# zijinxuxu/PDFNet

Hardware: AMD Instinct MI355X
Metric: train-step images/sec @256x256 RGB-D B=32 (higher is better)
Workload: dtype f32

## Files before the change

include/pdfnet_hip.h:

```cpp
#ifndef PDFNET_HIP_H
#define PDFNET_HIP_H
#ifdef __cplusplus
extern "C" {
#endif

#define PDF_E_BADARG (-1)
#define PDF_E_WORKSPACE (-2)
#define PDF_ACT_NONE 0
#define PDF_ACT_RELU 1
#define PDF_ACT_LRELU01 2


int pdf_linear_fwd(const float* x, const float* w, const float* bias, float* y,
                   int M, int N, int K, int ldx, int ldw, int ldy, int act, void* stream);
int pdf_linear_bwd_weight(const float* x, const float* dy, float* dw, float* db, float* ws, long ws_floats,
                          int M, int N, int K, int ldx, int lddy, int accumulate, void* stream);
long pdf_wgrad_workspace_floats(int M, int NI, int NJ);
int pdf_init(void);
int pdf_debug_init_device(void);
int pdf_debug_kernel_timing(int on);
int pdf_set_stats_output(float* part, long cap_floats);
long pdf_stats_result_tiles(void);
long pdf_stats_result_rows(void);
int pdf_set_bn_tile_stats(const float* part, long tiles, long rows_per_tile);
int pdf_debug_kernel_record_count(void);
int pdf_debug_kernel_record(int i, char* name, int cap, double* flops, double* bytes, float* ms);
int pdf_stream_wait(void* waiter, void* signaler);
int pdf_set_gemm_precision(int bf16);
int pdf_debug_gemm_precision(void);
int pdf_debug_last_tile(void);
int pdf_debug_igemm_launches(void);
int pdf_linear_bwd_data(const float* dy, const float* w, float* dx, int M, int N, int K, int lddy, int ldw, int lddx, void* stream);
int pdf_linear_fwd_pair(const float* x, const float* w0, const float* w1, const float* b0, const float* b1, float* y,
                        int M, int N, int K, int ldx, int ldw, int ldy, int act, void* stream);
int pdf_linear_bwd_data_pair(const float* dy, const float* w0, const float* w1, float* dx, int M, int N, int K,
                             int lddy, int ldw, int lddx, void* stream);
int pdf_linear_bwd_weight_pair(const float* x, const float* dy, float* dw0, float* dw1, float* db0, float* db1,
                               float* ws, long ws_floats, int M, int N, int K, int ldx, int lddy, int accumulate, void* stream);

int pdf_conv2d_fwd(const float* x, const float* w, const float* bias, float* y,
                   int N, int H, int W, int Cin, int ldx, int Cout, int KH, int KW,
                   int stride, int pad, int OH, int OW, int ldy, int act, void* stream);
int pdf_conv2d_bwd_data(const float* dy, const float* w, float* dx,
                        int N, int H, int W, int Cin, int lddx, int Cout, int KH, int KW,
                        int stride, int pad, int OH, int OW, int lddy, void* stream);
int pdf_conv2d_bwd_data_add(const float* dy, const float* w, float* dx,
                        int N, int H, int W, int Cin, int lddx, int Cout, int KH, int KW,
                        int stride, int pad, int OH, int OW, int lddy, void* stream);
int pdf_conv2d_bwd_weight(const float* x, const float* dy, float* dw, float* db, float* ws, long ws_floats,
                          int N, int H, int W, int Cin, int ldx, int Cout, int KH, int KW,
                          int stride, int pad, int OH, int OW, int lddy, int accumulate, void* stream);

int pdf_deconv2d_fwd(const float* x, const float* w, const float* bias, float* y,
                     int N, int H, int W, int Cin, int ldx, int Cout, int KH, int KW,
                     int stride, int pad, int OH, int OW, int ldy, void* stream);
int pdf_deconv2d_bwd_data(const float* dy, const float* w, float* dx,
                          int N, int H, int W, int Cin, int lddx, int Cout, int KH, int KW,
                          int stride, int pad, int OH, int OW, int lddy, void* stream);
int pdf_deconv2d_bwd_weight(const float* x, const float* dy, float* dw, float* ws, long ws_floats,
                            int N, int H, int W, int Cin, int ldx, int Cout, int KH, int KW,
                            int stride, int pad, int OH, int OW, int lddy, int accumulate, void* stream);
int pdf_bmm_strided(const float* A, const float* B, float* C, int batch, int M, int N, int K, int RB,
                    long sab, long sar, long sam, long sak, long sbb, long sbr, long sbk, long sbn,
                    long scb, long scm, long scn, int beta, void* stream);


int pdf_knn_ball_group(const float* pts, int ldp, int C, int Bc, int N, int S, int K, float r2,
                       int* idx, float* grouped, int ldg, void* stream);
int pdf_group_bwd(const float* dg, int ldg, const int* idx, float* dpts, int ldd, int C,
                  int Bc, int N, int S, int K, void* stream);
int pdf_gather_sub_fwd(const float* u, int ldu, const float* v, int ldv, const int* idx, int Bc, int N, int S, int K, int C,
                       float* y, int ldy, void* stream);
int pdf_gather_sub_bwd(const float* dy, int lddy, const int* idx, float* du, int ldu, float* dv, int ldv,
                       int Bc, int N, int S, int K, int C, void* stream);
int pdf_invert_index(const int* idx, int Bc, int N, int E, int* start, int* list, int* tmp, void* stream);
int pdf_gather_sub_bwd_sorted(const float* dy, int lddy, const int* start, const int* list, float* du, int ldu, float* dv, int ldv,
                              int Bc, int N, int S, int K, int C, void* stream);
int pdf_gather_rows(const float* feat, int ldf, int C, long HW, const long* ind, long ind_bstride,
                    int B, int M, int R, int shift, float* out, int ldo, void* stream);
int pdf_scatter_rows_add(const float* dout, int ldo, int C, long HW, const long* ind, long ind_bstride,
                         int B, int M, int R, int shift, float* dfeat, int ldf, void* stream);
int pdf_window_op(float* feat, int ldf, int C, int H, int W, const long* ind, long ind_bstride,
                  int B, int M, int r, float* buf, const float* src, int mode, void* stream);
int pdf_nms_top1(const float* hm, int BC, int H, int W, long* ind, float* score, void* stream);
int pdf_maxk_fwd(const float* x, int ldx, int C, long R, int K, float* y, int ldy, int* arg, void* stream);
int pdf_maxk_bwd(const float* dy, int ldy, const int* arg, int C, long R, int K, float* dx, int ldx, void* stream);
int pdf_bn_relu_maxk_fwd(const float* y, int ldy, int C, long R, int K, const float* gamma, const float* beta,
                         float* running_mean, float* running_var, float momentum, float eps, int training,
                         float* out, int ldo, int* arg, float* save_mean, float* save_rstd, float* scale, float* shift,
                         float* ws, void* stream);
int pdf_bn_relu_maxk_bwd(const float* dout, int lddo, const int* arg, const float* y, int ldy, const float* save_mean, const float* save_rstd,
                         const float* gamma, const float* scale, const float* shift, int C, long R, int K,
                         float* dy, int lddy, float* dgamma, float* dbeta, int accumulate, float* ws, void* stream);
long pdf_sa_fused_workspace_floats(int Bc, int S, int K, int C1, int C2, int C3);
int pdf_sa_fused_fwd(const float* u, const float* v, const int* idx, int Bc, int N, int S, int K, int C1, int C2, int C3,
                     const float* w2, const float* b2, const float* w3, const float* b3,
                     const float* gamma1, const float* beta1, const float* gamma2, const float* beta2, const float* gamma3, const float* beta3,
                     float* rmean1, float* rvar1, float* rmean2, float* rvar2, float* rmean3, float* rvar3, float momentum, float eps, int training,
                     float* out, int* arg, float* zsel, float* saved, float* ws, long ws_floats, void* stream);
int pdf_sa_fused_bwd(const float* dout, const float* u, const float* v, const int* idx, int Bc, int N, int S, int K, int C1, int C2, int C3,
                     const float* w2, const float* b2, const float* w3, const float* b3,
                     const float* out, const int* arg, const float* zsel, const float* saved,
                     float* dz1, float* dw2, float* db2, float* dw3, float* db3,
                     float* dgamma1, float* dbeta1, float* dgamma2, float* dbeta2, float* dgamma3, float* dbeta3,
                     float* ws, long ws_floats, void* stream);


long pdf_bn_workspace_floats(int C, long R);
int pdf_bn_train_fwd(const float* x, int ldx, int C, long R, const float* gamma, const float* beta,
                     float* running_mean, float* running_var, float momentum, float eps,
                     const float* res, int ldr, int relu, float* y, int ldy,
                     float* save_mean, float* save_rstd, float* scale, float* shift, float* ws, void* stream);
int pdf_bn_eval_fwd(const float* x, int ldx, int C, long R, const float* gamma, const float* beta,
                    const float* running_mean, const float* running_var, float eps,
                    const float* res, int ldr, int relu, float* y, int ldy, float* scale, float* shift, void* stream);
int pdf_bn_train_bwd(const float* dy, int lddy, const float* y, int ldy, int relu, const float* x, int ldx,
                     const float* save_mean, const float* save_rstd, const float* gamma,
                     const float* scale, const float* shift, int C, long R,
                     float* dx, int lddx, float* dres, int lddr, float* dgamma, float* dbeta, int accumulate,
                     float* ws, void* stream);
int pdf_bn_eval_bwd(const float* dy, int lddy, const float* y, int ldy, int relu, const float* x, int ldx,
                    const float* running_mean, const float* running_var, float eps, const float* scale, const float* shift,
                    int C, long R, float* dx, int lddx, float* dres, int lddr,
                    float* dgamma, float* dbeta, int accumulate, float* ws, void* stream);
int pdf_bn_relu_maxk_eval_bwd(const float* dout, int lddo, const int* arg, const float* y, int ldy,
                              const float* running_mean, const float* running_var, float eps, const float* scale, const float* shift,
                              int C, long R, int K, float* dy, int lddy, float* dgamma, float* dbeta, int accumulate, float* ws, void* stream);
int pdf_colsum(const float* g, int ldg, int C, long R, float* out, int accumulate, float* ws, void* stream);
int pdf_colsum_pair(const float* g, int ldg, int C, long R, float* out0, float* out1, int accumulate, float* ws, void* stream);
int pdf_layernorm_fwd(const float* x, int ldx, int F, long R, const float* gamma, const float* beta, float eps,
                      float* y, int ldy, float* mean, float* rstd, void* stream);
int pdf_layernorm_bwd(const float* dy, int lddy, const float* x, int ldx, int F, long R, const float* gamma,
                      const float* mean, const float* rstd, float* dx, int lddx, float* dgamma, float* dbeta, void* stream);
int pdf_layernorm_fused_fwd(const float* x, int ldx, const float* add, int ldadd, float p, unsigned long long seed,
                            const unsigned long long* step, int F, long R, long R_split,
                            const float* gamma0, const float* beta0, const float* gamma1, const float* beta1, float eps, int act,
                            float* z, int ldz, float* y, int ldy, float* mean, float* rstd, void* stream);
int pdf_layernorm_fused_bwd(const float* dy, int lddy, const float* y, int ldy, int act, const float* z, int ldz, int F, long R, long R_split,
                            const float* gamma0, const float* gamma1, const float* mean, const float* rstd,
                            const float* dz_in, int lddzin, float* dz, int lddz, float* dadd, int lddadd,
                            float p, unsigned long long seed, const unsigned long long* step,
                            float* dgamma0, float* dbeta0, float* dgamma1, float* dbeta1, void* stream);
int pdf_l2norm_fwd(const float* x, int ldx, int C, long R, const float* w, float eps, float* y, int ldy, float* norm, void* stream);
int pdf_l2norm_bwd(const float* dy, int lddy, const float* x, int ldx, int C, long R, const float* w, float eps,
                   const float* norm, float* dx, int lddx, float* dw, void* stream);
int pdf_l2norm_cat_fwd(int nparts, const float* const* x, const int* C, const float* const* w, float eps, long R,
                       float* y, int ldy, float* const* norm, void* stream);
int pdf_l2norm_cat_bwd(int nparts, const float* dy, int lddy, const float* const* x, const int* C, const float* const* w, float eps, long R,
                       float* const* norm, float* const* dx, float* const* dw, void* const* dx16_or_null, void* stream);

int pdf_act_fwd(const float* x, int ldx, float* y, int ldy, int C, long R, int act, void* stream);
int pdf_act_bwd(const float* dy, int lddy, const float* y, int ldy, float* dx, int lddx, int C, long R, int act, void* stream);
int pdf_sft_fwd(const float* fea, int ldf, const float* scale, int lds, const float* shift, int ldh,
                float* out, int ldo, int C, long R, void* stream);
int pdf_sft_bwd(const float* g, int ldg, const float* fea, int ldf, const float* scale, int lds,
                float* dfea, int lddf, float* dscale, int ldds, int C, long R, void* stream);
int pdf_sft3_fwd(const float* fea, int ldf, const float* cond, int ldc, const float* w_scale0, const float* b_scale0,
                 const float* w_scale1, const float* b_scale1, const float* w_shift0, const float* b_shift0,
                 const float* w_shift1, const float* b_shift1, float* out, int ldo, long R, void* stream);
int pdf_sft3_bwd(const float* g, int ldg, const float* fea, int ldf, const float* cond, int ldc,
                 const float* w_scale0, const float* b_scale0, const float* w_scale1, const float* b_scale1,
                 const float* w_shift0, const float* b_shift0, const float* w_shift1, const float* b_shift1,
                 float* dfea, int lddf, float* dcond, int lddc,
                 float* dw_scale0, float* db_scale0, float* dw_scale1, float* db_scale1,
                 float* dw_shift0, float* db_shift0, float* dw_shift1, float* db_shift1, int accumulate,
                 float* ws, long R, void* stream);
int pdf_set_bf16_operands(const void* op0_bf16, const void* op1_bf16);
int pdf_set_bf16_output(void* out_bf16);
int pdf_set_bn_input_bf16(const void* x16);
int pdf_set_input_affine_relu(const float* scale, const float* shift);
int pdf_cast_bf16(const float* src, void* dst, long n, void* stream);
int pdf_cast_bf16_transposed(const float* src, void* dst, const void* table, int nlayers, long total_tiles, void* stream);
int pdf_debug_shadow_operands(void);
int pdf_dropout(const float* x, float* y, long n, float p, unsigned long long seed, const unsigned long long* step, void* stream);
int pdf_dropout_add(const float* x, const float* res, float* y, long n, float p, unsigned long long seed,
                    const unsigned long long* step, void* stream);
int pdf_maxpool3s2_fwd(const float* x, int N, int H, int W, int C, float* y, unsigned char* arg, void* stream);
int pdf_maxpool3s2_bwd(const float* dy, const unsigned char* arg, int N, int H, int W, int C, float* dx, void* stream);
int pdf_maxpool3s2_bwd_add(const float* dy, const unsigned char* arg, int N, int H, int W, int C, float* dx, void* stream);
int pdf_upsample2x_fwd(const float* x, int N, int H, int W, int C, float* y, void* stream);
int pdf_upsample2x_bwd(const float* dy, int N, int H, int W, int C, float* dx, void* stream);
int pdf_pad2d(const float* src, int lds, long R, int C, float* dst, int ldd, long R2, int C2, void* stream);
int pdf_adam_step(float* p, const float* g, float* m, float* v, long n, float lr, float b1, float b2, float eps,
                  const float* corr, float grad_scale, void* stream);

int pdf_cheby2_fwd(const float* x, int ldx, int B, int V, int F, const int* col, const float* val, int Wd,
                   float* out, int ldo, void* stream);
int pdf_cheby2_bwd(const float* d, int ldd, int B, int V, int F, const int* colT, const float* valT, int Wd,
                   float* dx, int lddx, void* stream);
int pdf_cheby2_fwd_pair(const float* x, int ldx, int B, int V, int F, const int* col0, const float* val0,
                        const int* col1, const float* val1, int Wd, float* out, int ldo, void* stream);
int pdf_cheby2_bwd_pair(const float* d, int ldd, int B, int V, int F, const int* colT0, const float* valT0,
                        const int* colT1, const float* valT1, int Wd, float* dx, int lddx, void* stream);
int pdf_attn_fwd(const float* q, const float* k, const float* v, int ld, int B, int V, int H, int dh, int kv_shift,
                 float pdrop, unsigned long long seed, const unsigned long long* step, float* out, int ldo, float* stat, void* stream);
int pdf_attn_bwd(const float* q, const float* k, const float* v, int ld, const float* o, const float* dout, int ldo,
                 const float* stat, int B, int V, int H, int dh, int kv_shift, float pdrop, unsigned long long seed, const unsigned long long* step,
                 float* dq, float* dk, float* dv, int lddq, float* dvec, void* stream);

int pdf_fps(const float* xyz, int ld, int Bc, int N, int S, const int* start, int* idx, void* stream);

int pdf_rowloss_fwd(const float* pred, const float* tgt, long rows, long n, int mode, float* out, void* stream);
int pdf_rowloss_bwd(const float* pred, const float* tgt, const float* gout, long rows, long n, int mode, float* dpred, void* stream);
int pdf_face_loss_fwd(const float* pred, const float* gt, const long long* faces, int G, int B, int V, int Fc, float* part, void* stream);
int pdf_face_loss_bwd(const float* pred, const float* gt, const long long* faces, int G, int B, int V, int Fc,
                      const float* wn, const float* we, float* dpred, void* stream);

long pdf_dense_loss_workspace_floats(int B);
int pdf_dense_loss_fwd(const float* mask, const float* mask_gt, int mask_c, int mask_hw,
                       const float* hms, const float* hms_gt, int hms_c, int hms_hw,
                       const float* hm, const float* hm_gt, int hm_c, int hm_hw, int B, float* ws, float* out, void* stream);
int pdf_dense_loss_bwd(const float* mask, const float* mask_gt, float* dmask, int mask_c, int mask_hw,
                       const float* hms, const float* hms_gt, float* dhms, int hms_c, int hms_hw,
                       const float* hm, const float* hm_gt, float* dhm, int hm_c, int hm_hw, int B,
                       const float* g_mask, const float* g_hms, const float* g_hm, const float* stat, void* stream);
int pdf_point_dist_sum(const float* pred, const float* gt, int rows, int n, int dim, float* out, void* stream);

int pdf_procrustes_dist(const float* pred, const float* gt, int rows, int n, float* sum, float* dist, float* aligned, void* stream);
int pdf_mesh_nn_counts(const float* pred, const float* gt, int rows, int n, const float* thr, int T, int* counts, float* d_gt, float* d_pred,
                       void* stream);

int pdf_depth2pcl(const float* depth, const float* mask, const float* K, const float* valid, int B, int H, int W,
                  unsigned long long seed, long* choose, float* cloud, int* count, void* stream);

int pdf_mano_lbs_fwd(const float* root_aa, const float* pose_aa, const float* shape, const float* trans,
                     const float* v_template, const float* shapedirs, const float* posedirs, const float* J_reg,
                     const float* weights, int B, int left_side, int center_idx, float* verts, float* joints, void* stream);
int pdf_mano_lbs_bwd(const float* root_aa, const float* pose_aa, const float* shape,
                     const float* v_template, const float* shapedirs, const float* posedirs, const float* J_reg,
                     const float* weights, int B, int left_side, int center_idx, const float* dverts, const float* djoints,
                     float* droot, float* dpose, float* dshape, float* dtrans, void* stream);
int pdf_mano_split_coeff(const float* params, int ldp, long HW, const long* ind, const float* K, int B, int input_res, int down,
                         float* orient, float* pose, float* shape, float* trans, void* stream);
int pdf_mano_split_coeff_bwd(const float* params, float* dparams, int ldp, long HW, const long* ind, const float* K, int B, int input_res, int down,
                             const float* dorient, const float* dpose, const float* dtrans, void* stream);


typedef struct PdfCallOpts {
    const void* op0_bf16; const void* op1_bf16;
    void* out_bf16;
    const void* bn_x_bf16;
    float* stats_out; long stats_cap;
    long stats_tiles; long stats_rows;
    const float* tile_stats; long tile_n; long tile_rows;
    const float* in_scale; const float* in_shift;
    const void* op1_bf16_t;
    float* ws; long ws_floats;
    const float* wino_v;
} PdfCallOpts;
long pdf_conv2d_winograd_v_offset(int N, int H, int W, int Cin, int Cout, int KH, int KW, int stride, int pad);
int pdf_linear_fwd_x(const float* x, const float* w, const float* bias, float* y, int M, int N, int K, int ldx, int ldw, int ldy, int act, void* stream, PdfCallOpts* opts);
int pdf_linear_fwd_pair_x(const float* x, const float* w0, const float* w1, const float* b0, const float* b1, float* y, int M, int N, int K, int ldx, int ldw, int ldy, int act, void* stream, PdfCallOpts* opts);
int pdf_linear_bwd_data_x(const float* dy, const float* w, float* dx, int M, int N, int K, int lddy, int ldw, int lddx, void* stream, PdfCallOpts* opts);
int pdf_linear_bwd_data_pair_x(const float* dy, const float* w0, const float* w1, float* dx, int M, int N, int K, int lddy, int ldw, int lddx, void* stream, PdfCallOpts* opts);
int pdf_conv2d_fwd_x(const float* x, const float* w, const float* bias, float* y, int N, int H, int W, int Cin, int ldx, int Cout, int KH, int KW, int stride, int pad, int OH, int OW, int ldy, int act, void* stream, PdfCallOpts* opts);
int pdf_conv2d_bwd_data_x(const float* dy, const float* w, float* dx, int N, int H, int W, int Cin, int lddx, int Cout, int KH, int KW, int stride, int pad, int OH, int OW, int lddy, void* stream, PdfCallOpts* opts);
int pdf_conv2d_bwd_data_add_x(const float* dy, const float* w, float* dx, int N, int H, int W, int Cin, int lddx, int Cout, int KH, int KW, int stride, int pad, int OH, int OW, int lddy, void* stream, PdfCallOpts* opts);
int pdf_linear_bwd_weight_x(const float* x, const float* dy, float* dw, float* db, float* ws, long ws_floats, int M, int N, int K, int ldx, int lddy, int accumulate, void* stream, PdfCallOpts* opts);
int pdf_linear_bwd_weight_pair_x(const float* x, const float* dy, float* dw0, float* dw1, float* db0, float* db1, float* ws, long ws_floats, int M, int N, int K, int ldx, int lddy, int accumulate, void* stream, PdfCallOpts* opts);
int pdf_conv2d_bwd_weight_x(const float* x, const float* dy, float* dw, float* db, float* ws, long ws_floats, int N, int H, int W, int Cin, int ldx, int Cout, int KH, int KW, int stride, int pad, int OH, int OW, int lddy, int accumulate, void* stream, PdfCallOpts* opts);
int pdf_deconv2d_fwd_x(const float* x, const float* w, const float* bias, float* y, int N, int H, int W, int Cin, int ldx, int Cout, int KH, int KW, int stride, int pad, int OH, int OW, int ldy, void* stream, PdfCallOpts* opts);
int pdf_deconv2d_bwd_data_x(const float* dy, const float* w, float* dx, int N, int H, int W, int Cin, int lddx, int Cout, int KH, int KW, int stride, int pad, int OH, int OW, int lddy, void* stream, PdfCallOpts* opts);
int pdf_deconv2d_bwd_weight_x(const float* x, const float* dy, float* dw, float* ws, long ws_floats, int N, int H, int W, int Cin, int ldx, int Cout, int KH, int KW, int stride, int pad, int OH, int OW, int lddy, int accumulate, void* stream, PdfCallOpts* opts);
int pdf_bn_train_fwd_x(const float* x, int ldx, int C, long R, const float* gamma, const float* beta, float* running_mean, float* running_var, float momentum, float eps, const float* res, int ldr, int relu, float* y, int ldy, float* save_mean, float* save_rstd, float* scale, float* shift, float* ws, void* stream, PdfCallOpts* opts);
int pdf_bn_train_bwd_x(const float* dy, int lddy, const float* y, int ldy, int relu, const float* x, int ldx, const float* save_mean, const float* save_rstd, const float* gamma, const float* scale, const float* shift, int C, long R, float* dx, int lddx, float* dres, int lddr, float* dgamma, float* dbeta, int accumulate, float* ws, void* stream, PdfCallOpts* opts);
int pdf_bn_relu_maxk_fwd_x(const float* y, int ldy, int C, long R, int K, const float* gamma, const float* beta, float* running_mean, float* running_var, float momentum, float eps, int training, float* out, int ldo, int* arg, float* save_mean, float* save_rstd, float* scale, float* shift, float* ws, void* stream, PdfCallOpts* opts);
int pdf_l2norm_cat_fwd_x(int nparts, const float* const* x, const int* C, const float* const* w, float eps, long R, float* y, int ldy, float* const* norm, void* stream, PdfCallOpts* opts);
long pdf_conv2d_winograd_workspace_floats(int N, int H, int W, int Cin, int Cout, int KH, int KW, int stride, int pad, int backward);
int pdf_debug_armed_slots(void);
int pdf_debug_callopts_size(void);

int pdf_x3_split(const float* x, void* out, long n, long cs, void* stream);
long pdf_deconv2d_x3_workspace_floats(int N, int H, int W, int Cin, int Cout, int KH, int KW, int stride, int pad, int backward);
int pdf_set_x3_mode(int mode);
int pdf_stream_create(void** out, int priority, int* lo, int* hi);
int pdf_debug_x3_mode(void);
int pdf_debug_x3_stamps(unsigned long long* out);
int pdf_x3_batched_gemm_nt(const void* A3, long csA, const void* B3, long csB, float* C, int batch, long gsA, long gsB, long gsC, int M, int N, int K, int variant, int nprod, void* stream);
int pdf_batched_gemm_nt(const float* A, const float* B, float* C, int batch, long gsA, long gsB, long gsC, int M, int N, int K, void* stream);
int pdf_x3_batched_gemm_tn(const void* P3, long csP, const void* Q3, long csQ, float* slab, int batch, long gsP, long gsQ, int M, int NI, int NJ, int splits, int variant, int nprod, void* stream);
int pdf_batched_gemm_tn(const float* P, const float* Q, float* slab, int batch, long gsP, long gsQ, int M, int NI, int NJ, int splits, void* stream);

typedef struct PdfMeshLin { const float* w[2]; const float* b[2]; } PdfMeshLin;
typedef struct PdfMeshLN { const float* g[2]; const float* b[2]; } PdfMeshLN;
typedef struct PdfMeshGcn { PdfMeshLin fc1, fc2, sc; PdfMeshLN n2, n3; unsigned long long seed; } PdfMeshGcn;
typedef struct PdfMeshAttn {
    PdfMeshLN ln; PdfMeshLin q, k, v, fc; PdfMeshLN ffln; PdfMeshLin f1, f2;
    unsigned long long seed_att, seed_z, seed_t, seed_x;
} PdfMeshAttn;
typedef struct PdfMeshLinG { float* w[2]; float* b[2]; } PdfMeshLinG;
typedef struct PdfMeshLNG { float* g[2]; float* b[2]; } PdfMeshLNG;
typedef struct PdfMeshGcnG { PdfMeshLinG fc1, fc2, sc; PdfMeshLNG n2, n3; } PdfMeshGcnG;
typedef struct PdfMeshAttnG { PdfMeshLNG ln; PdfMeshLinG q, k, v, fc; PdfMeshLNG ffln; PdfMeshLinG f1, f2; } PdfMeshAttnG;
typedef struct PdfMeshLevel {
    int level, B, training, cin0;
    float p;
    const unsigned long long* step;
    const float* x;
    float* out;
    const int* ell_col[2]; const float* ell_val[2]; const int* ell_colT[2]; const float* ell_valT[2]; int ell_w;
    PdfMeshGcn gcn[4];
    PdfMeshAttn self_, cross;
    float* tape;
    float* qkv;
    const float* dout;
    float* dx;
    float* gtape;
    PdfMeshGcnG ggcn[4]; PdfMeshAttnG gself, gcross;
    float* wg_ws; long wg_ws_floats;
} PdfMeshLevel;
long pdf_mesh_tape_floats(int level, int B);
long pdf_mesh_gtape_floats(int level, int B);
int pdf_mesh_level_fwd(const PdfMeshLevel* a, void* stream);
int pdf_mesh_level_bwd(const PdfMeshLevel* a, void* stream, void* side_stream);
int pdf_mesh_level_fwd_bf16(const PdfMeshLevel* a, void* stream);
int pdf_mesh_level_bwd_bf16(const PdfMeshLevel* a, void* stream, void* side_stream);
int pdf_mesh_level_fwd_x3(const PdfMeshLevel* a, void* stream);
int pdf_mesh_level_bwd_x3(const PdfMeshLevel* a, void* stream, void* side_stream);
int pdf_debug_mesh_level_size(void);

typedef struct PdfMeshLoss {
    const float* vp; const float* v2p; const float* hd3; const float* hd2; const float* r;
    const float* vgt[2]; const float* jgt[2]; const float* v2gt[2]; const float* lmsgt[2];
    const long long* ind; const float* K; const float* valid;
    const float* reg[2]; const long long* faces; const long long* perm[2];
    int B, Fc, size, down;
    float* part;
    float* out;
    float coef[12];
    const float* gmp;
    int edge_grad;
    float* dvp; float* dv2p; float* dhd3; float* dhd2; float* dr;
} PdfMeshLoss;
int pdf_mesh_loss_fwd(const PdfMeshLoss* a, void* stream);
int pdf_mesh_loss_bwd(const PdfMeshLoss* a, void* stream);
int pdf_debug_mesh_loss_size(void);
int pdf_debug_mesh_stamps(unsigned long long* out);

#ifdef __cplusplus
}
#endif
#endif
```

pdfnet_amd/csrc/common.h:

```cpp
#pragma once
#include <hip/hip_runtime.h>
#include <stdint.h>
#include "pdfnet_hip.h"

#define PDF_API extern "C" __attribute__((visibility("default")))

#define PDF_LAUNCH_CHECK()                                  \
    do {                                                    \
        hipError_t e__ = hipGetLastError();                 \
        if (e__ != hipSuccess) return (int)e__;             \
    } while (0)

static inline int cdiv(long a, long b) { return (int)((a + b - 1) / b); }

static inline int grid_for(long n, int block = 256, int cap = 256 * 8) {
    long g = (n + block - 1) / block;
    if (g > cap) g = cap;
    if (g < 1) g = 1;
    return (int)g;
}

__device__ __forceinline__ float wave_sum(float v) {
#pragma unroll
    for (int o = 32; o > 0; o >>= 1) v += __shfl_xor(v, o, 64);
    return v;
}
__device__ __forceinline__ float wave_max(float v) {
#pragma unroll
    for (int o = 32; o > 0; o >>= 1) v = fmaxf(v, __shfl_xor(v, o, 64));
    return v;
}
__device__ __forceinline__ int wave_sum_i(int v) {
#pragma unroll
    for (int o = 32; o > 0; o >>= 1) v += __shfl_xor(v, o, 64);
    return v;
}

__device__ __forceinline__ uint32_t pdf_hash32(uint32_t x) {
    x ^= x >> 16; x *= 0x7feb352dU; x ^= x >> 15; x *= 0x846ca68bU; x ^= x >> 16;
    return x;
}
__device__ __forceinline__ float pdf_uniform(uint64_t seed, uint64_t idx) {
    uint32_t h = pdf_hash32((uint32_t)idx ^ pdf_hash32((uint32_t)(idx >> 32) + (uint32_t)seed) ^ (uint32_t)(seed >> 32) * 0x9E3779B9U);
    return (float)(h >> 8) * (1.0f / 16777216.0f);
}

__device__ __forceinline__ void pdf_store_wt(float* p, float v) { __hip_atomic_store(p, v, __ATOMIC_RELAXED, __HIP_MEMORY_SCOPE_AGENT); }
__device__ __forceinline__ bool pdf_last_block_arrives(int* counter, int expected, int* flag, bool release = true) {
    asm volatile("s_waitcnt vmcnt(0)" ::: "memory");
    __syncthreads();
    if (threadIdx.x == 0) {
        if (release) {
            __builtin_amdgcn_fence(__ATOMIC_RELEASE, "agent");
            asm volatile("s_waitcnt vmcnt(0)" ::: "memory");
        }
        const int t = __hip_atomic_fetch_add(counter, 1, __ATOMIC_RELAXED, __HIP_MEMORY_SCOPE_AGENT);
        const int last = t == expected - 1;
        if (last) {
            __builtin_amdgcn_fence(__ATOMIC_ACQUIRE, "agent");
            asm volatile("s_waitcnt vmcnt(0)" ::: "memory");
            __hip_atomic_store(counter, 0, __ATOMIC_RELAXED, __HIP_MEMORY_SCOPE_AGENT);
        }
        *flag = last;
    }
    __syncthreads();
    return *flag != 0;
}

#define PDF_COUNTER_RING (1 << 22)
int* pdf_ticket_counters(int n);
#define PDF_SCRATCH_RING (1L << 26)
#define PDF_SCRATCH_MAX (1L << 22)
float* pdf_scratch(long floats);
typedef __bf16 pdf_bf16x2 __attribute__((ext_vector_type(2)));
typedef float pdf_f32x2 __attribute__((ext_vector_type(2)));
__device__ __forceinline__ unsigned int pdf_pk_bf16(float a, float b) {
    pdf_f32x2 f = {a, b};
    pdf_bf16x2 v = __builtin_convertvector(f, pdf_bf16x2);
    return *reinterpret_cast<unsigned int*>(&v);
}
__device__ __forceinline__ void pdf_x3_split2(float a, float b, unsigned& h, unsigned& m, unsigned& l) {
    h = pdf_pk_bf16(a, b);
    float ra = a - __uint_as_float(h << 16), rb = b - __uint_as_float(h & 0xffff0000u);
    m = pdf_pk_bf16(ra, rb);
    ra -= __uint_as_float(m << 16); rb -= __uint_as_float(m & 0xffff0000u);
    l = pdf_pk_bf16(ra, rb);
}
__device__ __forceinline__ void pdf_x3_store2(unsigned short* base, long o, long cs, float a, float b) {
    unsigned h, m, l;
    pdf_x3_split2(a, b, h, m, l);
    *reinterpret_cast<unsigned*>(base + o) = h;
    *reinterpret_cast<unsigned*>(base + o + cs) = m;
    *reinterpret_cast<unsigned*>(base + o + 2 * cs) = l;
}
template <class F, class... A> static inline int pdf_call_x(PdfCallOpts* opts, F impl, A... a) {
    PdfCallOpts none = {};
    PdfCallOpts& co = opts != nullptr ? *opts : none;
    co.stats_tiles = co.stats_rows = 0;
    return impl(a..., co);
}
struct PdfPlainCall { PdfCallOpts co; PdfPlainCall(); ~PdfPlainCall(); };
template <class F, class... A> static inline int pdf_call_plain(F impl, A... a) {
    PdfPlainCall call;
    return impl(a..., call.co);
}
```

pdfnet_amd/csrc/gemm.hip:

```cpp
#include "common.h"

#include "gemm_common.h"

long pdf_internal_wino_workspace(int N, int H, int W, int Ck, int Cn, int flip);
int pdf_internal_wino_eligible(int N, int H, int W, int Ck, int Cn, int KH, int KW, int stride, int pad, int flip);
int pdf_internal_conv3x3_winograd(const float* x, int ldx, const float* w, const float* bias, float* y, int ldy, float* ws,
                                  int N, int H, int W, int Ck, int Cn, int act, int accum, int flip, const float* v_shared, hipStream_t s);
int pdf_internal_wino_wgrad_eligible(int N, int H, int W, int Cin, int Cout, int KH, int KW, int stride, int pad);
long pdf_internal_wino_wgrad_workspace(int N, int H, int W, int Cin, int Cout);
long pdf_internal_wino_v_offset(int N, int H, int W, int Ck, int Cn);
int pdf_internal_conv3x3_winograd_wgrad(const float* x, int ldx, const float* dy, int lddy, float* dw, float* db, float* ws,
                                        int N, int H, int W, int Cin, int Cout, int accumulate, const float* v_cached, hipStream_t s);
PDF_API long pdf_conv2d_winograd_v_offset(int N, int H, int W, int Cin, int Cout, int KH, int KW, int stride, int pad) {
    if (!pdf_internal_wino_eligible(N, H, W, Cin, Cout, KH, KW, stride, pad, 0) || !pdf_internal_wino_wgrad_eligible(N, H, W, Cin, Cout, KH, KW, stride, pad)) return -1;
    return pdf_internal_wino_v_offset(N, H, W, Cin, Cout);
}
PDF_API long pdf_conv2d_winograd_workspace_floats(int N, int H, int W, int Cin, int Cout, int KH, int KW, int stride, int pad, int backward) {
    if (backward == 2) return pdf_internal_wino_wgrad_eligible(N, H, W, Cin, Cout, KH, KW, stride, pad) ? pdf_internal_wino_wgrad_workspace(N, H, W, Cin, Cout) : 0;
    const int Ck = backward ? Cout : Cin, Cn = backward ? Cin : Cout;
    return pdf_internal_wino_eligible(N, H, W, Ck, Cn, KH, KW, stride, pad, backward) ? pdf_internal_wino_workspace(N, H, W, Ck, Cn, backward) : 0;
}

#ifndef PDF_FRAG_PIPE
#define PDF_FRAG_PIPE 0
// ... 239 lines not shown
            for (int j = 0; j < TN; ++j) b[set][j] = bs[brow + j * 32 * LD + kk * 2];
        };
        if (FRAG_PIPE) frag(0, 0);
#pragma unroll
        for (int kk = 0; kk < BK / 2; ++kk) {
            const int set = FRAG_PIPE ? (kk & 1) : 0;
            if (FRAG_PIPE) { if (kk + 1 < BK / 2) frag(set ^ 1, kk + 1); }
            else frag(0, kk);
#pragma unroll
            for (int i = 0; i < TM; ++i)
#pragma unroll
                for (int j = 0; j < TN; ++j)
                    acc[i][j] = __builtin_amdgcn_mfma_f32_32x32x2f32(a[set][i], b[set][j], acc[i][j], 0, 0, 0);
        }
    };
    if constexpr (FAST && BUF && IG_DEEP && BM * BN <= 64 * 64) {
        gload(kt0, ra, rb);
        gload(kt0 + 1, ra1, rb1);
        lstore(0, ra, rb);
        __syncthreads();
        for (int kt = kt0; kt < kt1; kt += 2) {
            gload(kt + 2, ra, rb);
            compute(0);
            if (kt + 1 >= kt1) break;
            lstore(1, ra1, rb1);
            __syncthreads();
            gload(kt + 3, ra1, rb1);
            compute(1);
            if (kt + 2 < kt1) lstore(0, ra, rb);
            __syncthreads();
        }
        if (g.stat != nullptr) __syncthreads();
    } else {
        gload(kt0, ra, rb);
        lstore(0, ra, rb);
        __syncthreads();
        int cur = 0;
        for (int kt = kt0; kt < kt1; ++kt) {
            if (kt + 1 < kt1) gload(kt + 1, ra, rb);
            compute(cur);
            if (kt + 1 < kt1) lstore(cur ^ 1, ra, rb);
            __syncthreads();
            cur ^= 1;
        }
    }

    if (g.ksteps > 0) {
        float* pp = g.part + (long)blockIdx.z * g.M * g.N;
        if (m0 + BM <= g.M && (long)g.M * g.N < (1L << 29)) {
            const auto rsP = __builtin_amdgcn_make_buffer_rsrc((void*)pp, 0, (unsigned)g.M * (unsigned)g.N * 4u, 0x00020000);
            const unsigned ldn4 = (unsigned)g.N * 4u;
#pragma unroll
            for (int j = 0; j < TN; ++j) {
                const int col = n0 + wn * TN * 32 + j * 32 + (lane & 31);
#pragma unroll
                for (int i = 0; i < TM; ++i) {
                    const unsigned vo = col < g.N ? (unsigned)((m0 + wm * TM * 32 + i * 32 + 4 * (lane >> 5)) * g.N + col) * 4u : 0xffffffffu;
                    float v[16];
#pragma unroll
                    for (int r = 0; r < 16; ++r) v[r] = acc[i][j][r];
#pragma unroll
                    for (int r = 0; r < 16; ++r)
                        __builtin_amdgcn_raw_buffer_store_b32(__builtin_bit_cast(unsigned, v[r]), rsP, vo, ((r & 3) + 8 * (r >> 2)) * ldn4, 0);
                }
            }
            return;
        }
#pragma unroll
        for (int j = 0; j < TN; ++j) {
            const int col = n0 + wn * TN * 32 + j * 32 + (lane & 31);
#pragma unroll
            for (int i = 0; i < TM; ++i)
#pragma unroll
                for (int r = 0; r < 16; ++r) {
                    const int row = m0 + wm * TM * 32 + i * 32 + (r & 3) + 8 * (r >> 2) + 4 * (lane >> 5);
                    if (col < g.N && row < g.M) pp[(long)row * g.N + col] = acc[i][j][r];
                }
        }
        return;
    }
    StatAcc st[TN];
#pragma unroll
    for (int j = 0; j < TN; ++j) st[j] = StatAcc{0.f, 0.f, 0.f, 0.f};
    const bool do_stat = g.stat != nullptr;
    if constexpr (FAST && BUF) {
        if (g.cbytes != 0 && m0 + BM <= g.M) {
            lean_epilogue<TM, TN, WM, WN, BN>(acc, g, Cp, biasp, m0, n0, tmi, wm, wn, lane, tid, &As[0][0]);
            return;
        }
    }
#pragma unroll
    for (int j = 0; j < TN; ++j) {
        const int col = n0 + wn * TN * 32 + j * 32 + (lane & 31);
        const bool cok = col < g.N;
        int co = col, padd_y = 0, padd_x = 0;
        if (g.ps_cout > 0) {
            int tap = col / g.ps_cout;
            co = col - tap * g.ps_cout;
            padd_y = tap / g.ps_kw;
            padd_x = tap - padd_y * g.ps_kw;
        }
        const float bv = (biasp != nullptr && cok) ? biasp[co] : 0.f;
#pragma unroll
        for (int i = 0; i < TM; ++i) {
#pragma unroll
            for (int r = 0; r < 16; ++r) {
                const int row = m0 + wm * TM * 32 + i * 32 + (r & 3) + 8 * (r >> 2) + 4 * (lane >> 5);
                if (cok && row < g.M) {
                    float v = acc[i][j][r] + bv;
                    if (g.act == 1) v = fmaxf(v, 0.f);
                    else if (g.act == 2) v = v > 0.f ? v : 0.1f * v;
                    long o;
                    if (g.plain_out) o = (long)row * g.ldc + co;
                    else {
                        int hw = g.QH * g.QW;
                        int ni = row / hw, rem = row - ni * hw;
                        int qy = rem / g.QW, qx = rem - qy * g.QW;
                        int oy = qy * g.osy + g.ooy + padd_y, ox = qx * g.osx + g.oox + padd_x;
                        o = (((long)ni * g.OH + oy) * g.OW + ox) * g.ldc + co;
                    }
                    if (g.accum) v += Cp[o];
                    Cp[o] = v;
                    if (do_stat) stat_add(st[j], v);
                }
            }
        }
    }
    if (do_stat) stat_finish<TN, WM, WN, BN>(st, &As[0][0], g.stat, tmi, n0, g.N, wm, wn, lane, tid);
}

template <int BM, int BN, int WM, int WN, bool FAST, bool KN, int BKT = 16, bool BUF = false>
__global__ __launch_bounds__(WM * WN * 64, (BM * BN >= 128 * 128 ? 3 : 1)) void igemm_nt(const IGemm g) {
    igemm_nt_body<BM, BN, WM, WN, FAST, KN, BKT, BUF, false>(g);
}
template <int BM, int BN, int WM, int WN, int BKT>
__global__ __launch_bounds__(WM * WN * 64, (BM * BN >= 128 * 128 ? 3 : 1)) void igemm_nt_aff(const IGemm g) {
    igemm_nt_body<BM, BN, WM, WN, true, false, BKT, true, true>(g);
}

#define HALO_MAX_PIX 264
template <bool KN, bool BUF = false>
__global__ __launch_bounds__(256, 3) void igemm_halo3x3(const IGemm g) {
    constexpr int BM = 128, BN = 128, WN = 2, BK = 16, LD = 17, TM = 2, TN = 2;
    constexpr int NH = (HALO_MAX_PIX * 4 + 255) / 256;
    __shared__ float As[2][HALO_MAX_PIX * LD];
    __shared__ float Bs[2][BN * LD];
    const int tid = threadIdx.x, lane = tid & 63, wave = tid >> 6;
    const int wm = wave / WN, wn = wave % WN;
    const float* __restrict__ Ap = g.A; const float* __restrict__ Bp = g.B; const float* __restrict__ biasp = g.bias;
    float* __restrict__ Cp = g.C;
    const int ntm = g.M / BM, ntn = (g.N + BN - 1) / BN;
    int tmi, tni;
    xcd_tile(blockIdx.x, ntm * ntn, ntn, tmi, tni, g.gm);
    const int m0 = tmi * BM, n0 = tni * BN;
    const int W = g.W, H = g.H, HC = W + 2, R = BM / W, HP = (R + 2) * HC;
    const int img = m0 / (H * W), y0 = (m0 - img * H * W) / W;
    long hsrc[NH]; int hdst[NH]; bool hok[NH];
#pragma unroll
    for (int i = 0; i < NH; ++i) {
        const int q = tid + i * 256, hp = q >> 2, part = q & 3;
        const int hy = hp / HC, hx = hp - hy * HC;
        const int iy = y0 - 1 + hy, ix = hx - 1;
        hok[i] = hp < HP && iy >= 0 && iy < H && ix >= 0 && ix < W;
        hsrc[i] = (((long)img * H + iy) * W + ix) * g.lda + part * 4;
        hdst[i] = hp < HP ? hp * LD + part * 4 : -1;
    }
    const int lrow = tid >> 2, kq = (tid & 3) * 4;
    const int nq4 = (tid & 31) * 4;
    long bbase[2]; bool bval[2]; int kb[2];
#pragma unroll
    for (int i = 0; i < 2; ++i) {
        if (KN) { kb[i] = (tid + i * 256) >> 5; bval[i] = n0 + nq4 < g.N; bbase[i] = (long)kb[i] * g.ldb + n0 + nq4; }
        else { const int n = n0 + lrow + i * 64; kb[i] = 0; bval[i] = n < g.N; bbase[i] = (long)n * g.ldb; }
    }
    f32x16 acc[TM][TN];
#pragma unroll
    for (int a = 0; a < TM; ++a)
#pragma unroll
        for (int b = 0; b < TN; ++b)
#pragma unroll
            for (int r = 0; r < 16; ++r) acc[a][b][r] = 0.f;

    float4 ra[NH], rb[2];
    const auto rsA = __builtin_amdgcn_make_buffer_rsrc((void*)Ap, 0, BUF ? g.abytes : 0, 0x00020000);
    const auto rsB = __builtin_amdgcn_make_buffer_rsrc((void*)Bp, 0, BUF ? g.bbytes : 0, 0x00020000);
    unsigned hoffB[NH], boffB[2];
    if constexpr (BUF) {
#pragma unroll
        for (int i = 0; i < NH; ++i) hoffB[i] = (unsigned)hsrc[i] * 4u;
#pragma unroll
        for (int i = 0; i < 2; ++i) boffB[i] = (unsigned)(bbase[i] + (KN ? 0 : kq)) * 4u;
    }
    auto hload = [&](int ci0) {
#pragma unroll
        for (int i = 0; i < NH; ++i) {
            if constexpr (BUF) ra[i] = as_f4(__builtin_amdgcn_raw_buffer_load_b128(rsA, hok[i] ? hoffB[i] + (unsigned)ci0 * 4u : 0xffffffffu, 0, 0));
            else ra[i] = *reinterpret_cast<const float4*>(hok[i] ? Ap + hsrc[i] + ci0 : g_zero16);
        }
    };
    auto hstore = [&](int buf) {
#pragma unroll
        for (int i = 0; i < NH; ++i)
            if (hdst[i] >= 0) { float* p = &As[buf][hdst[i]]; p[0] = ra[i].x; p[1] = ra[i].y; p[2] = ra[i].z; p[3] = ra[i].w; }
    };
    auto bload = [&](int ci0, int tap) {
        const int wb = g.wt[tap] * (KN ? g.btap : g.Cin);
        if constexpr (BUF) {
            const unsigned sb = KN ? (unsigned)(ci0 * g.ldb + wb) * 4u : (unsigned)(wb + ci0) * 4u;
#pragma unroll
            for (int i = 0; i < 2; ++i) rb[i] = as_f4(__builtin_amdgcn_raw_buffer_load_b128(rsB, bval[i] ? boffB[i] + sb : 0xffffffffu, 0, 0));
        } else {
            const long wofs = KN ? (long)ci0 * g.ldb + wb : (long)(wb + ci0 + kq);
#pragma unroll
            for (int i = 0; i < 2; ++i) rb[i] = *reinterpret_cast<const float4*>(bval[i] ? Bp + bbase[i] + wofs : g_zero16);
        }
    };
    auto bstore = [&](int buf) {
#pragma unroll
        for (int i = 0; i < 2; ++i) {
            if (KN) { float* p = &Bs[buf][nq4 * LD + kb[i]]; p[0] = rb[i].x; p[LD] = rb[i].y; p[2 * LD] = rb[i].z; p[3 * LD] = rb[i].w; }
            else { float* p = &Bs[buf][(lrow + i * 64) * LD + kq]; p[0] = rb[i].x; p[1] = rb[i].y; p[2] = rb[i].z; p[3] = rb[i].w; }
        }
    };
    int arow[TM];
#pragma unroll
    for (int i = 0; i < TM; ++i) {
        const int p = (wm * TM + i) * 32 + (lane & 31), r = p / W, c = p - r * W;
        arow[i] = ((r + 1) * HC + c + 1) * LD + (lane >> 5);
    }
    const int brow = (wn * TN * 32 + (lane & 31)) * LD + (lane >> 5);

    const int nchunks = g.Cin / BK, nsteps = nchunks * 9;
    hload(0); hstore(0);
    bload(0, 0); bstore(0);
    __syncthreads();
    int abuf = 0, bbuf = 0, chunk = 0, tap = 0;
    for (int st = 0; st < nsteps; ++st) {
        const bool more = st + 1 < nsteps;
        const int ntap = tap == 8 ? 0 : tap + 1, nchunk = tap == 8 ? chunk + 1 : chunk;
        if (more) bload(nchunk * BK, ntap);
        const bool stage_a = tap == 0 && chunk + 1 < nchunks;
        if (stage_a) hload((chunk + 1) * BK);
        const int toff = (g.dy[tap] * HC + g.dx[tap]) * LD;
        const float* as = As[abuf] + toff;
        const float* bs = Bs[bbuf];
        float a[2][TM], b[2][TN];
        auto frag = [&](int set, int kk) {
#pragma unroll
            for (int i = 0; i < TM; ++i) a[set][i] = as[arow[i] + kk * 2];
#pragma unroll
            for (int j = 0; j < TN; ++j) b[set][j] = bs[brow + j * 32 * LD + kk * 2];
        };
        if (FRAG_PIPE) frag(0, 0);
#pragma unroll
        for (int kk = 0; kk < BK / 2; ++kk) {
            const int set = FRAG_PIPE ? (kk & 1) : 0;
            if (FRAG_PIPE) { if (kk + 1 < BK / 2) frag(set ^ 1, kk + 1); }
            else frag(0, kk);
#pragma unroll
            for (int i = 0; i < TM; ++i)
#pragma unroll
                for (int j = 0; j < TN; ++j) acc[i][j] = __builtin_amdgcn_mfma_f32_32x32x2f32(a[set][i], b[set][j], acc[i][j], 0, 0, 0);
        }
        if (more) bstore(bbuf ^ 1);
        if (stage_a) hstore(abuf ^ 1);
        __syncthreads();
        bbuf ^= 1;
        if (tap == 8) abuf ^= 1;
        tap = ntap; chunk = nchunk;
    }
    if constexpr (BUF) {
        if (g.cbytes != 0) {
            lean_epilogue<TM, TN, 2, WN, BN>(acc, g, Cp, biasp, m0, n0, tmi, wm, wn, lane, tid, &As[0][0]);
            return;
        }
    }
    StatAcc st[TN];
#pragma unroll
    for (int j = 0; j < TN; ++j) st[j] = StatAcc{0.f, 0.f, 0.f, 0.f};
    const bool do_stat = g.stat != nullptr;
#pragma unroll
    for (int j = 0; j < TN; ++j) {
        const int col = n0 + wn * TN * 32 + j * 32 + (lane & 31);
        const bool cok = col < g.N;
        const float bv = (biasp != nullptr && cok) ? biasp[col] : 0.f;
#pragma unroll
        for (int i = 0; i < TM; ++i)
#pragma unroll
            for (int r = 0; r < 16; ++r) {
                const int row = m0 + wm * TM * 32 + i * 32 + (r & 3) + 8 * (r >> 2) + 4 * (lane >> 5);
                if (cok) {
                    float v = acc[i][j][r] + bv;
                    if (g.act == 1) v = fmaxf(v, 0.f);
                    else if (g.act == 2) v = v > 0.f ? v : 0.1f * v;
                    if (g.accum) v += Cp[(long)row * g.ldc + col];
                    Cp[(long)row * g.ldc + col] = v;
                    if (do_stat) stat_add(st[j], v);
                }
            }
    }
    if (do_stat) stat_finish<TN, 2, WN, BN>(st, &As[0][0], g.stat, tmi, n0, g.N, wm, wn, lane, tid);
}

template <int BI, int BJ, int WM, int WN, bool FAST, int BKT, bool BUF, bool AFF>
__device__ __forceinline__ void wgemm_tn_body(const WGemm& g) {
    constexpr int BK = BKT;
    constexpr int TM = BI / WM / 32, TN = BJ / WN / 32;
    constexpr int TPR_P = BI / 4, TPR_Q = BJ / 4;
    constexpr int RP = BK / (256 / TPR_P), RQ = BK / (256 / TPR_Q);
    __shared__ __attribute__((aligned(16))) float Ps[2][BK * BI];
    __shared__ __attribute__((aligned(16))) float Qs[2][BK * BJ];

    const int tid = threadIdx.x, lane = tid & 63, wave = tid >> 6;
    const float* __restrict__ Pp = g.P; const float* __restrict__ Qp = g.Q; float* slabp = g.slab; float* bslabp = g.bslab;
    if (blockIdx.z) { Pp += g.gsP; Qp += g.gsQ; slabp = g.slab1; bslabp = g.bslab1; }
    const int wm = wave / WN, wn = wave % WN;
    const int NJ = g.T * g.Cq;
    const int nti = (g.NI + BI - 1) / BI, ntj = (NJ + BJ - 1) / BJ;
    int ti, tj;
    if (g.tap_major) {
        const int nblk = nti * ntj, q = nblk >> 3, r = nblk & 7, x = blockIdx.x & 7;
        const int lin = (x < r ? x * (q + 1) : r * (q + 1) + (x - r) * q) + (blockIdx.x >> 3);
        const int nb = g.Cq / BJ;
        const int per_cb = g.T * nti;
        const int cb = lin / per_cb, rem = lin - cb * per_cb;
        const int tap = rem / nti;
        ti = rem - tap * nti;
        tj = tap * nb + cb;
    } else {
        xcd_tile(blockIdx.x, nti * ntj, ntj, ti, tj);
    }
    const int i0 = ti * BI, j0 = tj * BJ;
    const bool do_bias = bslabp != nullptr && tj == 0 && tid < BI;
    float bsum = 0.f;
    const int ms = blockIdx.y * g.rows_per_split;
    const int me = min(g.M, ms + g.rows_per_split);

    const int pr = tid / TPR_P, pc = (tid % TPR_P) * 4;
    const int qr = tid / TPR_Q, qc = (tid % TPR_Q) * 4;
    int qt[4], qch[4]; bool qok[4];
#pragma unroll
    for (int e = 0; e < 4; ++e) {
        int j = j0 + qc + e;
        qok[e] = j < NJ;
        int t = qok[e] ? j / g.Cq : 0;
        qt[e] = t; qch[e] = j - t * g.Cq;
    }

    f32x16 acc[TM][TN];
#pragma unroll
    for (int a = 0; a < TM; ++a)
#pragma unroll
        for (int b = 0; b < TN; ++b)
#pragma unroll
            for (int r = 0; r < 16; ++r) acc[a][b][r] = 0.f;

    float4 rp[RP], rq[RQ];
    int q_ni[RQ], q_y[RQ], q_x[RQ];
#pragma unroll
    for (int i = 0; i < RQ; ++i) {
        int m = ms + qr + i * (256 / TPR_Q);
        int hw = g.QH * g.QW;
        q_ni[i] = m / hw;
        int rem = m - q_ni[i] * hw;
        q_y[i] = rem / g.QW;
        q_x[i] = rem - q_y[i] * g.QW;
    }
    const auto rsP = __builtin_amdgcn_make_buffer_rsrc((void*)Pp, 0, BUF ? g.pbytes : 0, 0x00020000);
    const auto rsQ = __builtin_amdgcn_make_buffer_rsrc((void*)Qp, 0, BUF ? g.qbytes : 0, 0x00020000);
    float4 qsc = make_float4(1.f, 1.f, 1.f, 1.f), qsh = make_float4(0.f, 0.f, 0.f, 0.f);
    if (AFF && qok[0]) { qsc = *reinterpret_cast<const float4*>(g.q_scale + qch[0]); qsh = *reinterpret_cast<const float4*>(g.q_shift + qch[0]); }
    auto gload = [&](int mb) {
        if constexpr (BUF) {
#pragma unroll
            for (int i = 0; i < RP; ++i) {
                const int m = mb + pr + i * (256 / TPR_P);
                const unsigned op = (m < me && i0 + pc < g.NI) ? (unsigned)(m * g.ldp + i0 + pc) * 4u : 0xffffffffu;
                const u32x4v v = __builtin_amdgcn_raw_buffer_load_b128(rsP, op, 0, 0);
                rp[i] = *reinterpret_cast<const float4*>(&v);
            }
#pragma unroll
            for (int i = 0; i < RQ; ++i) {
                const int m = mb + qr + i * (256 / TPR_Q);
                unsigned oq;
                if (g.plain_q) oq = (m < me && qok[0]) ? (unsigned)(m * g.ldq + qch[0]) * 4u : 0xffffffffu;
                else {
                    const int iy = q_y[i] * g.sy + g.dy[qt[0]], ix = q_x[i] * g.sx + g.dx[qt[0]];
                    const bool ok = m < me && qok[0] && iy >= 0 && iy < g.H && ix >= 0 && ix < g.W;
                    oq = ok ? (unsigned)(((q_ni[i] * g.H + iy) * g.W + ix) * g.ldq + qch[0]) * 4u : 0xffffffffu;
                }
                const u32x4v v = __builtin_amdgcn_raw_buffer_load_b128(rsQ, oq, 0, 0);
                rq[i] = *reinterpret_cast<const float4*>(&v);
                if constexpr (AFF) {
                    if (mb + BK <= me && qok[0]) {
                        rq[i].x = fmaxf(fmaf(rq[i].x, qsc.x, qsh.x), 0.f); rq[i].y = fmaxf(fmaf(rq[i].y, qsc.y, qsh.y), 0.f);
                        rq[i].z = fmaxf(fmaf(rq[i].z, qsc.z, qsh.z), 0.f); rq[i].w = fmaxf(fmaf(rq[i].w, qsc.w, qsh.w), 0.f);
                    } else {
                        const bool rok = oq != 0xffffffffu;
                        rq[i].x = rok ? fmaxf(fmaf(rq[i].x, qsc.x, qsh.x), 0.f) : 0.f; rq[i].y = rok ? fmaxf(fmaf(rq[i].y, qsc.y, qsh.y), 0.f) : 0.f;
                        rq[i].z = rok ? fmaxf(fmaf(rq[i].z, qsc.z, qsh.z), 0.f) : 0.f; rq[i].w = rok ? fmaxf(fmaf(rq[i].w, qsc.w, qsh.w), 0.f) : 0.f;
                    }
                }
                q_x[i] += BK;
                while (q_x[i] >= g.QW) {
                    q_x[i] -= g.QW;
                    if (++q_y[i] == g.QH) { q_y[i] = 0; ++q_ni[i]; }
                }
            }
            return;
        }
#pragma unroll
        for (int i = 0; i < RP; ++i) {
            int m = mb + pr + i * (256 / TPR_P);
            float4 v = make_float4(0.f, 0.f, 0.f, 0.f);
            if (m < me) {
                const float* p = Pp + (long)m * g.ldp + i0 + pc;
                if (FAST) { if (i0 + pc < g.NI) v = *reinterpret_cast<const float4*>(p); }
                else {
                    if (i0 + pc + 0 < g.NI) v.x = p[0];
                    if (i0 + pc + 1 < g.NI) v.y = p[1];
                    if (i0 + pc + 2 < g.NI) v.z = p[2];
                    if (i0 + pc + 3 < g.NI) v.w = p[3];
                }
            }
            rp[i] = v;
        }
#pragma unroll
        for (int i = 0; i < RQ; ++i) {
            int m = mb + qr + i * (256 / TPR_Q);
            float4 v = make_float4(0.f, 0.f, 0.f, 0.f);
            if (m < me) {
                if (g.plain_q) {
                    const float* p = Qp + (long)m * g.ldq;
                    if (FAST) { if (qok[0]) v = *reinterpret_cast<const float4*>(p + qch[0]); }
                    else {
                        if (qok[0]) v.x = p[qch[0]];
                        if (qok[1]) v.y = p[qch[1]];
                        if (qok[2]) v.z = p[qch[2]];
                        if (qok[3]) v.w = p[qch[3]];
                    }
                } else {
                    const int qy = q_y[i], qx = q_x[i];
                    const float* img = Qp + (long)q_ni[i] * g.H * g.W * g.ldq;
                    if (FAST) {
                        int iy = qy * g.sy + g.dy[qt[0]], ix = qx * g.sx + g.dx[qt[0]];
                        if (qok[0] && iy >= 0 && iy < g.H && ix >= 0 && ix < g.W)
                            v = *reinterpret_cast<const float4*>(img + ((long)iy * g.W + ix) * g.ldq + qch[0]);
                    } else {
                        float e4[4];
#pragma unroll
                        for (int e = 0; e < 4; ++e) {
                            int iy = qy * g.sy + g.dy[qt[e]], ix = qx * g.sx + g.dx[qt[e]];
                            e4[e] = (qok[e] && iy >= 0 && iy < g.H && ix >= 0 && ix < g.W)
                                        ? img[((long)iy * g.W + ix) * g.ldq + qch[e]] : 0.f;
                        }
                        v = make_float4(e4[0], e4[1], e4[2], e4[3]);
                    }
                }
            }
            rq[i] = v;
            q_x[i] += BK;
            while (q_x[i] >= g.QW) {
                q_x[i] -= g.QW;
                if (++q_y[i] == g.QH) { q_y[i] = 0; ++q_ni[i]; }
            }
        }
    };
    auto lstore = [&](int buf) {
#pragma unroll
        for (int i = 0; i < RP; ++i)
            *reinterpret_cast<float4*>(&Ps[buf][(pr + i * (256 / TPR_P)) * BI + pc]) = rp[i];
#pragma unroll
        for (int i = 0; i < RQ; ++i)
            *reinterpret_cast<float4*>(&Qs[buf][(qr + i * (256 / TPR_Q)) * BJ + qc]) = rq[i];
    };

    if (ms < me) {
        gload(ms);
        lstore(0);
    }
    __syncthreads();
    int cur = 0;
    const int aoff = (lane >> 5) * BI + wm * TM * 32 + (lane & 31);
    const int boff = (lane >> 5) * BJ + wn * TN * 32 + (lane & 31);
    for (int mb = ms; mb < me; mb += BK) {
        const bool more = mb + BK < me;
        if (more) gload(mb + BK);
        const float* ps = Ps[cur];
        const float* qs = Qs[cur];
        if (do_bias) {
#pragma unroll
            for (int kb = 0; kb < BK; ++kb) bsum += ps[kb * BI + tid];
        }
#pragma unroll
        for (int kk = 0; kk < BK / 2; ++kk) {
            float a[TM], b[TN];
#pragma unroll
            for (int i = 0; i < TM; ++i) a[i] = ps[aoff + kk * 2 * BI + i * 32];
#pragma unroll
            for (int j = 0; j < TN; ++j) b[j] = qs[boff + kk * 2 * BJ + j * 32];
#pragma unroll
            for (int i = 0; i < TM; ++i)
#pragma unroll
                for (int j = 0; j < TN; ++j)
                    acc[i][j] = __builtin_amdgcn_mfma_f32_32x32x2f32(a[i], b[j], acc[i][j], 0, 0, 0);
        }
        if (more) lstore(cur ^ 1);
        __syncthreads();
        cur ^= 1;
    }

    wgemm_finish<TM, TN>(g, acc, i0, j0, wm, wn, lane, do_bias && i0 + tid < g.NI, bsum, ti * ntj + tj, nti * ntj, reinterpret_cast<int*>(&Ps[0][0]), i0 + BI <= g.NI);
}


template <int BI, int BJ, int WM, int WN, bool FAST, int BKT = 16, bool BUF = false>
__global__ __launch_bounds__(256) void wgemm_tn(const WGemm g) {
    wgemm_tn_body<BI, BJ, WM, WN, FAST, BKT, BUF, false>(g);
}
__global__ __launch_bounds__(256) void wgemm_tn64_aff(const WGemm g) {
    wgemm_tn_body<64, 64, 2, 2, true, 32, true, true>(g);
}


#define GLDS16(src, dst) __builtin_amdgcn_global_load_lds((const __attribute__((address_space(1))) void*)(src), \
                                                          (__attribute__((address_space(3))) void*)(dst), 16, 0, 0)

#define LDS_PTR(p) ((__attribute__((address_space(3))) void*)(p))
template <int ST, bool BUF, bool AFF>
__device__ __forceinline__ void wgemm_tn_dma_body(const WGemm& g) {
    constexpr int BI = 128, BJ = 128, BK = 16, WN = 2, TM = 2, TN = 2;
    __shared__ __attribute__((aligned(16))) float smem[ST * 2 * BK * 128];
    const int tid = threadIdx.x, lane = tid & 63, wave = tid >> 6;
    const float* __restrict__ Pp = g.P; const float* __restrict__ Qp = g.Q; float* slabp = g.slab; float* bslabp = g.bslab;
    const int wm = wave / WN, wn = wave % WN;
    const int NJ = g.T * g.Cq;
    const int nti = (g.NI + BI - 1) / BI, ntj = (NJ + BJ - 1) / BJ;
    int split = blockIdx.y, plane = blockIdx.z, lin_tile = -1;
    if (g.batch > 0 && g.bsplits > 0) {
        const int tiles = nti * ntj, slot = blockIdx.x >> 3;
        const int grp = (slot / tiles) * 8 + (blockIdx.x & 7);
        if (grp >= g.bsplits * g.batch) return;
        lin_tile = slot - (slot / tiles) * tiles;
        plane = grp / g.bsplits;
        split = grp - plane * g.bsplits;
    }
    if (g.batch > 0) { Pp += (long)plane * g.gsP; Qp += (long)plane * g.gsQ; bslabp = nullptr; }
    else if (blockIdx.z) { Pp += g.gsP; Qp += g.gsQ; slabp = g.slab1; bslabp = g.bslab1; }
    int ti, tj;
    if (lin_tile >= 0) { ti = lin_tile / ntj; tj = lin_tile - ti * ntj; }
    else if (g.tap_major) {
        const int nblk = nti * ntj, q = nblk >> 3, r = nblk & 7, x = blockIdx.x & 7;
        const int lin = (x < r ? x * (q + 1) : r * (q + 1) + (x - r) * q) + (blockIdx.x >> 3);
        const int nb = g.Cq / BJ, per_cb = g.T * nti;
        const int cb = lin / per_cb, rem = lin - cb * per_cb;
        const int tap = rem / nti;
        ti = rem - tap * nti;
        tj = tap * nb + cb;
    } else {
        xcd_tile(blockIdx.x, nti * ntj, ntj, ti, tj);
    }
    const int i0 = ti * BI, j0 = tj * BJ;
    const bool do_bias = bslabp != nullptr && tj == 0 && tid < BI;
    float bsum = 0.f;
    const int ms = split * g.rows_per_split;
    const int me = min(g.M, ms + g.rows_per_split);
    const int nt = (me - ms + BK - 1) / BK;

    const int pr = tid >> 5, pc = (tid & 31) * 4;
    const bool pcol_ok = i0 + pc < g.NI;
    const int jcol = j0 + pc;
    const bool qcol_ok = jcol < NJ;
    const int qtap = qcol_ok ? jcol / g.Cq : 0;
    const int qch = jcol - qtap * g.Cq;
    const int tdy = g.dy[qtap], tdx = g.dx[qtap];
    int q_ni[2], q_y[2], q_x[2];
#pragma unroll
    for (int i = 0; i < 2; ++i) {
        const int m = ms + pr + i * 8, hw = g.QH * g.QW;
        q_ni[i] = m / hw;
        const int rem = m - q_ni[i] * hw;
        q_y[i] = rem / g.QW;
        q_x[i] = rem - q_y[i] * g.QW;
    }
    const int wbase = __builtin_amdgcn_readfirstlane(wave) * 2 * 128;
    const auto rsP = __builtin_amdgcn_make_buffer_rsrc((void*)Pp, 0, BUF ? g.pbytes : 0, 0x00020000);
    const auto rsQ = __builtin_amdgcn_make_buffer_rsrc((void*)Qp, 0, BUF ? g.qbytes : 0, 0x00020000);

    auto issue = [&](int t, int st) {
        float* sp = smem + (st * 2 + 0) * BK * 128 + wbase;
        float* sq = smem + (st * 2 + 1) * BK * 128 + wbase;
        const int mb = ms + t * BK;
#pragma unroll
        for (int i = 0; i < 2; ++i) {
            const int m = mb + pr + i * 8;
            const bool rowok = m < me;
            if constexpr (BUF) {
                const unsigned op = (rowok && pcol_ok) ? (unsigned)(m * g.ldp + i0 + pc) * 4u : 0xffffffffu;
                unsigned oq;
                if (g.plain_q) oq = (rowok && qcol_ok) ? (unsigned)(m * g.ldq + qch) * 4u : 0xffffffffu;
                else {
                    const int iy = q_y[i] * g.sy + tdy, ix = q_x[i] * g.sx + tdx;
                    const bool ok = rowok && qcol_ok && iy >= 0 && iy < g.H && ix >= 0 && ix < g.W;
                    oq = ok ? (unsigned)(((q_ni[i] * g.H + iy) * g.W + ix) * g.ldq + qch) * 4u : 0xffffffffu;
                }
                __builtin_amdgcn_raw_ptr_buffer_load_lds(rsP, LDS_PTR(sp + i * 8 * 128), 16, op, 0, 0, 0);
                __builtin_amdgcn_raw_ptr_buffer_load_lds(rsQ, LDS_PTR(sq + i * 8 * 128), 16, oq, 0, 0, 0);
            } else {
                const float* srcp = (rowok && pcol_ok) ? Pp + (long)m * g.ldp + i0 + pc : g_zero16;
                const float* srcq;
                if (g.plain_q) srcq = (rowok && qcol_ok) ? Qp + (long)m * g.ldq + qch : g_zero16;
                else {
                    const int iy = q_y[i] * g.sy + tdy, ix = q_x[i] * g.sx + tdx;
                    const bool ok = rowok && qcol_ok && iy >= 0 && iy < g.H && ix >= 0 && ix < g.W;
                    srcq = ok ? Qp + ((long)q_ni[i] * g.H * g.W + (long)iy * g.W + ix) * g.ldq + qch : g_zero16;
                }
                GLDS16(srcp, sp + i * 8 * 128);
                GLDS16(srcq, sq + i * 8 * 128);
            }
        }
        if (g.QW * 2 >= BK) {
#pragma unroll
            for (int i = 0; i < 2; ++i) {
                q_x[i] += BK;
#pragma unroll
                for (int w = 0; w < 2; ++w) {
                    const bool wrap = q_x[i] >= g.QW;
                    q_x[i] -= wrap ? g.QW : 0;
                    q_y[i] += wrap ? 1 : 0;
                    const bool wy = q_y[i] >= g.QH;
                    q_y[i] = wy ? 0 : q_y[i];
                    q_ni[i] += wy ? 1 : 0;
                }
            }
        } else {
#pragma unroll
            for (int i = 0; i < 2; ++i) {
                const int m = mb + BK + pr + i * 8, hw = g.QH * g.QW;
                q_ni[i] = m / hw;
                const int rem = m - q_ni[i] * hw;
                q_y[i] = rem / g.QW;
                q_x[i] = rem - q_y[i] * g.QW;
            }
        }
    };

    const bool uni = BUF && g.uniform != 0;
    const int utap = __builtin_amdgcn_readfirstlane(j0 < NJ ? j0 / g.Cq : 0);
    const int udy = g.dy[utap], udx = g.dx[utap];
    int s_ni[2], s_y[2], s_x[2];
#pragma unroll
    for (int i = 0; i < 2; ++i) {
        const int m = __builtin_amdgcn_readfirstlane(ms + i * 8), hw = g.QH * g.QW;
        s_ni[i] = m / hw;
        const int rem = m - s_ni[i] * hw;
        s_y[i] = rem / g.QW;
        s_x[i] = rem - s_y[i] * g.QW;
    }
    const int cx = pr * g.sx + udx;
    const unsigned kP = (unsigned)(pr * g.ldp + i0 + pc) * 4u;
    const unsigned kQ = g.plain_q ? (unsigned)(pr * g.ldq + qch) * 4u : (unsigned)(cx * g.ldq + (jcol - utap * g.Cq)) * 4u;
    auto issue_uni = [&](int t, int st) {
        float* sp = smem + (st * 2 + 0) * BK * 128 + wbase;
        float* sq = smem + (st * 2 + 1) * BK * 128 + wbase;
        const int mb = ms + t * BK;
#pragma unroll
        for (int i = 0; i < 2; ++i) {
            const int m0 = mb + i * 8;
            const bool rowok = m0 + pr < me;
            unsigned sQ; bool yok = true, xok = true;
            if (g.plain_q) sQ = (unsigned)(m0 * g.ldq) * 4u;
            else {
                const int iy = s_y[i] * g.sy + udy, x0 = s_x[i] * g.sx;
                yok = iy >= 0 && iy < g.H;
                sQ = (unsigned)(((s_ni[i] * g.H + iy) * g.W + x0) * g.ldq) * 4u;
                xok = x0 + cx >= 0 && x0 + cx < g.W;
                s_x[i] += BK;
                while (s_x[i] >= g.QW) {
                    s_x[i] -= g.QW;
                    if (++s_y[i] == g.QH) { s_y[i] = 0; ++s_ni[i]; }
                }
            }
            const unsigned op = (rowok && pcol_ok) ? kP + (unsigned)(m0 * g.ldp) * 4u : 0xffffffffu;
            const unsigned oq = (rowok && qcol_ok && yok && xok) ? kQ + sQ : 0xffffffffu;
            __builtin_amdgcn_raw_ptr_buffer_load_lds(rsP, LDS_PTR(sp + i * 8 * 128), 16, op, 0, 0, 0);
            __builtin_amdgcn_raw_ptr_buffer_load_lds(rsQ, LDS_PTR(sq + i * 8 * 128), 16, oq, 0, 0, 0);
        }
    };

    const bool u16 = BUF && g.uniform == 2;
    const long qshift = g.plain_q ? 0 : ((long)udy * g.W + udx) * g.ldq;
    const auto rsQs = __builtin_amdgcn_make_buffer_rsrc((void*)(Qp + qshift), 0, BUF ? 0xfffffff0u : 0, 0x00020000);
    unsigned vP[2], vQ[2]; int cxl[2];
#pragma unroll
    for (int i = 0; i < 2; ++i) {
        vP[i] = pcol_ok ? (unsigned)((pr + 8 * i) * g.ldp + i0 + pc) * 4u : 0xffffffffu;
        vQ[i] = !qcol_ok ? 0xffffffffu : g.plain_q ? (unsigned)((pr + 8 * i) * g.ldq + qch) * 4u : (unsigned)((pr + 8 * i) * g.sx * g.ldq + (jcol - utap * g.Cq)) * 4u;
        cxl[i] = (pr + 8 * i) * g.sx + udx;
    }
    int u_x0 = s_x[0], u_y = s_y[0];
    unsigned u_sp = (unsigned)__builtin_amdgcn_readfirstlane(ms) * (unsigned)g.ldp * 4u;
    unsigned u_sq = g.plain_q ? (unsigned)__builtin_amdgcn_readfirstlane(ms) * (unsigned)g.ldq * 4u
                              : (unsigned)(((s_ni[0] * g.H + s_y[0] * g.sy) * g.W + s_x[0] * g.sx) * g.ldq) * 4u;
    const unsigned stepP = 16u * (unsigned)g.ldp * 4u, stepQ = (g.plain_q ? 16u : 16u * (unsigned)g.sx) * (unsigned)g.ldq * 4u;
    const unsigned wrapX = (unsigned)((g.sy * g.W - g.QW * g.sx) * g.ldq) * 4u, wrapY = (unsigned)((g.H - g.QH * g.sy) * g.W * g.ldq) * 4u;
    auto issue_u16 = [&](int t, int st) {
        float* sp = smem + (st * 2 + 0) * BK * 128 + wbase;
        float* sq = smem + (st * 2 + 1) * BK * 128 + wbase;
        const bool live = t < nt;
        const int iy = u_y * g.sy + udy;
        const bool rowq = live && (g.plain_q || (iy >= 0 && iy < g.H));
#pragma unroll
        for (int i = 0; i < 2; ++i) {
            const int ix = u_x0 * g.sx + cxl[i];
            const bool xok = g.plain_q || (ix >= 0 && ix < g.W);
            __builtin_amdgcn_raw_ptr_buffer_load_lds(rsP, LDS_PTR(sp + i * 8 * 128), 16, live ? vP[i] : 0xffffffffu, u_sp, 0, 0);
            __builtin_amdgcn_raw_ptr_buffer_load_lds(rsQs, LDS_PTR(sq + i * 8 * 128), 16, (rowq && xok) ? vQ[i] : 0xffffffffu, u_sq, 0, 0);
        }
        u_sp += stepP; u_sq += stepQ;
        if (!g.plain_q) {
            u_x0 += 16;
            if (u_x0 >= g.QW) {
                u_x0 = 0; u_sq += wrapX;
                if (++u_y == g.QH) { u_y = 0; u_sq += wrapY; }
            }
        }
    };

    f32x16 acc[TM][TN];
#pragma unroll
    for (int a = 0; a < TM; ++a)
#pragma unroll
        for (int b = 0; b < TN; ++b)
#pragma unroll
            for (int r = 0; r < 16; ++r) acc[a][b][r] = 0.f;

    const int aoff = (lane >> 5) * 128 + wm * TM * 32 + (lane & 31);
    const int boff = (lane >> 5) * 128 + wn * TN * 32 + (lane & 31);
    constexpr bool qaff = BUF && AFF;
    float fsc[TN], fsh[TN];
#pragma unroll
    for (int j = 0; j < TN; ++j) {
        const int c = j0 + wn * TN * 32 + j * 32 + (lane & 31);
        fsc[j] = (qaff && c < NJ) ? g.q_scale[c] : 1.f;
        fsh[j] = (qaff && c < NJ) ? g.q_shift[c] : 0.f;
    }
#pragma unroll
    for (int p = 0; p < ST - 1; ++p) { if (u16) issue_u16(p, p); else if (uni) issue_uni(p, p); else issue(p, p); }
    int st = 0, stn = ST - 1;
    for (int t = 0; t < nt; ++t) {
        if (ST == 3) asm volatile("s_waitcnt vmcnt(4)" ::: "memory"); else asm volatile("s_waitcnt vmcnt(8)" ::: "memory");
        __builtin_amdgcn_s_barrier();
        if (!u16) { if (uni) issue_uni(t + ST - 1, stn); else issue(t + ST - 1, stn); }
        const float* ps = smem + (st * 2 + 0) * BK * 128;
        const float* qs = smem + (st * 2 + 1) * BK * 128;
        if (do_bias) {
#pragma unroll
            for (int kb = 0; kb < BK; ++kb) bsum += ps[kb * 128 + tid];
        }
        float a[2][TM], b[2][TN];
        auto frag = [&](int set, int kk) {
#pragma unroll
            for (int i = 0; i < TM; ++i) a[set][i] = ps[aoff + kk * 2 * 128 + i * 32];
#pragma unroll
            for (int j = 0; j < TN; ++j) b[set][j] = qs[boff + kk * 2 * 128 + j * 32];
            if constexpr (qaff) {
#pragma unroll
                for (int j = 0; j < TN; ++j) b[set][j] = fmaxf(fmaf(b[set][j], fsc[j], fsh[j]), 0.f);
            }
        };
        if (FRAG_PIPE) frag(0, 0);
#pragma unroll
        for (int kk = 0; kk < BK / 2; ++kk) {
            const int set = FRAG_PIPE ? (kk & 1) : 0;
            if (FRAG_PIPE) { if (kk + 1 < BK / 2) frag(set ^ 1, kk + 1); }
            else frag(0, kk);
#pragma unroll
            for (int i = 0; i < TM; ++i)
#pragma unroll
                for (int j = 0; j < TN; ++j)
                    acc[i][j] = __builtin_amdgcn_mfma_f32_32x32x2f32(a[set][i], b[set][j], acc[i][j], 0, 0, 0);
            if (kk == PDF_WG_ISSUE_AT && u16) issue_u16(t + ST - 1, stn);
        }
        st = st == ST - 1 ? 0 : st + 1;
        stn = stn == ST - 1 ? 0 : stn + 1;
    }
    asm volatile("s_waitcnt vmcnt(0)" ::: "memory");

    wgemm_finish<TM, TN>(g, acc, i0, j0, wm, wn, lane, do_bias && i0 + tid < g.NI, bsum, ti * ntj + tj, nti * ntj, reinterpret_cast<int*>(smem), i0 + 128 <= g.NI,
                         lin_tile >= 0 ? split : -1, plane);
}

template <int ST, bool BUF>
__global__ __launch_bounds__(256) void wgemm_tn_dma(const WGemm g) {
    wgemm_tn_dma_body<ST, BUF, false>(g);
}
__global__ __launch_bounds__(256) void wgemm_tn_dma_aff(const WGemm g) {
    wgemm_tn_dma_body<3, true, true>(g);
}

struct Reduce {
    const float* slab; float* out; float* out1; long n;
    const float* bslab; float* bout; float* bout1; int nb;
    int splits, accumulate;
};
__global__ void reduce_slabs(const Reduce r, int main_blocks) {
    const bool bias = (int)blockIdx.x >= main_blocks;
    const float* slab = bias ? r.bslab : r.slab;
    float* out = bias ? (blockIdx.y ? r.bout1 : r.bout) : (blockIdx.y ? r.out1 : r.out);
    const long n = bias ? r.nb : r.n;
    if (blockIdx.y) slab += (long)r.splits * n;
    const long b0 = bias ? blockIdx.x - main_blocks : blockIdx.x, nblk = bias ? gridDim.x - main_blocks : main_blocks;
    for (long i = b0 * blockDim.x + threadIdx.x; i < n; i += nblk * blockDim.x) {
        float s = r.accumulate ? out[i] : 0.f;
        for (int z = 0; z < r.splits; ++z) s += slab[(long)z * n + i];
        out[i] = s;
    }
}

__global__ __launch_bounds__(256) void reduce_slabs_2d(const Reduce r, int main_blocks) {
    __shared__ float sm[4][64];
    const bool bias = (int)blockIdx.x >= main_blocks;
    const float* slab = bias ? r.bslab : r.slab;
    float* out = bias ? (blockIdx.y ? r.bout1 : r.bout) : (blockIdx.y ? r.out1 : r.out);
    const long n = bias ? r.nb : r.n;
    if (blockIdx.y) slab += (long)r.splits * n;
    const int tx = threadIdx.x & 63, ty = threadIdx.x >> 6;
    const long i = (bias ? blockIdx.x - main_blocks : blockIdx.x) * 64L + tx;
    float s = 0.f;
    if (i < n) for (int z = ty; z < r.splits; z += 4) s += slab[(long)z * n + i];
    sm[ty][tx] = s;
    __syncthreads();
    if (ty == 0 && i < n) out[i] = (r.accumulate ? out[i] : 0.f) + ((sm[0][tx] + sm[1][tx]) + (sm[2][tx] + sm[3][tx]));
}

static bool aligned16(const void* p) { return (reinterpret_cast<uintptr_t>(p) & 15) == 0; }

#include <cstdlib>
#include <climits>
#include <mutex>
enum { ENV_IG_T128, ENV_IG_BK32, ENV_WG_TARGET, ENV_WG_MINROWS, ENV_WG_TAPMAJOR, ENV_WG_BK32, ENV_WG_DMA, ENV_IG_HALO_MINC, ENV_IG_HALO, ENV_IG_T32, ENV_WG_INLAUNCH, ENV_WG_QUANT, ENV_IG_SPLITK, ENV_WG_LDSPAD, ENV_IG_SHORTK, ENV_WG_ATOMIC, ENV_WG_STEM, ENV_IG_SPLITK_MAXT, ENV_IG_SPLITK_TARGET, ENV_WG_SLOTS, ENV_WG_BUF, ENV_IG_BUF, ENV_WG_UNIFORM, ENV_IG_BUFSTORE, ENV_IG_BF16_STATS, ENV_IG_DMA, ENV_IG_DMA128, ENV_WG_BATCH_XCD, ENV_IG_GROUPM, ENV_COUNT };
static int env_int(int which, int dflt) {
    static const char* const names[ENV_COUNT] = {"PDF_IG_T128", "PDF_IG_BK32", "PDF_WG_TARGET", "PDF_WG_MINROWS", "PDF_WG_TAPMAJOR",
                                                 "PDF_WG_BK32", "PDF_WG_DMA", "PDF_IG_HALO_MINC", "PDF_IG_HALO", "PDF_IG_T32", "PDF_WG_INLAUNCH", "PDF_WG_QUANT", "PDF_IG_SPLITK", "PDF_WG_LDSPAD", "PDF_IG_SHORTK", "PDF_WG_ATOMIC", "PDF_WG_STEM", "PDF_IG_SPLITK_MAXT", "PDF_IG_SPLITK_TARGET", "PDF_WG_SLOTS", "PDF_WG_BUF", "PDF_IG_BUF", "PDF_WG_UNIFORM", "PDF_IG_BUFSTORE", "PDF_IG_BF16_STATS", "PDF_IG_DMA", "PDF_IG_DMA128", "PDF_WG_BATCH_XCD", "PDF_IG_GROUPM"};
    static int vals[ENV_COUNT];
    static std::once_flag once;
    std::call_once(once, [] {
        for (int i = 0; i < ENV_COUNT; ++i) {
            const char* e = getenv(names[i]);
            vals[i] = e ? atoi(e) : INT_MIN;
        }
    });
    return vals[which] == INT_MIN ? dflt : vals[which];
}

#include <string>
#include <vector>
#include <cstdio>
#include <cstring>
struct KRec { std::string name; hipEvent_t e0, e1; double flops, bytes; };
static std::vector<KRec> g_krecs;
static std::vector<hipEvent_t> g_kpool;
static size_t g_kpool_next = 0;
static std::mutex g_krec_mu;
static int g_ktiming = 0;
#define PDF_KTIMER_POOL 8192
KTimer::KTimer(const char* name, double flops, double bytes, hipStream_t s) : slot(-1), stream(s) {
    if (!g_ktiming) return;
    std::lock_guard<std::mutex> lk(g_krec_mu);
    if (g_kpool_next + 2 > g_kpool.size()) return;
    KRec r; r.name = name; r.flops = flops; r.bytes = bytes;
    r.e0 = g_kpool[g_kpool_next++]; r.e1 = g_kpool[g_kpool_next++];
    (void)hipEventRecord(r.e0, s);
    slot = (int)g_krecs.size();
    g_krecs.push_back(r);
}
KTimer::~KTimer() {
    if (slot < 0) return;
    std::lock_guard<std::mutex> lk(g_krec_mu);
    (void)hipEventRecord(g_krecs[slot].e1, stream);
}
PDF_API int pdf_debug_kernel_timing(int on) {
    std::lock_guard<std::mutex> lk(g_krec_mu);
    if (on) {
        g_krecs.clear();
        g_kpool_next = 0;
        while (g_kpool.size() < PDF_KTIMER_POOL) {
            hipEvent_t e;
            if (hipEventCreate(&e) != hipSuccess) return PDF_E_WORKSPACE;
            g_kpool.push_back(e);
        }
    }
    g_ktiming = on ? 1 : 0;
    return 0;
}
PDF_API int pdf_debug_kernel_record_count(void) { std::lock_guard<std::mutex> lk(g_krec_mu); return (int)g_krecs.size(); }
PDF_API int pdf_debug_kernel_record(int i, char* name, int cap, double* flops, double* bytes, float* ms) {
    std::lock_guard<std::mutex> lk(g_krec_mu);
    if (i < 0 || i >= (int)g_krecs.size() || cap < 2) return PDF_E_BADARG;
    const KRec& r = g_krecs[i];
    snprintf(name, cap, "%s", r.name.c_str());
    *flops = r.flops; *bytes = r.bytes;
    if (hipError_t e = hipEventElapsedTime(ms, r.e0, r.e1)) return (int)e;
    return 0;
}
static double igemm_bytes(const IGemm& g, int groups) {
    const double a = g.plain_in ? (double)g.M * g.Cin : (double)(g.M / max(1, g.QH * g.QW)) * g.H * g.W * g.Cin;
    return 4.0 * groups * (a + (double)g.N * g.K + (double)g.M * g.N * (g.accum ? 2 : 1));
}
static double wgemm_bytes(const WGemm& g, int groups) {
    const double q = g.plain_q ? (double)g.M * g.Cq : (double)(g.M / max(1, g.QH * g.QW)) * g.H * g.W * g.Cq;
    return 4.0 * groups * ((double)g.M * g.NI + q + (double)g.NI * g.T * g.Cq);
}

#define SMALLK_MAX 48
__global__ __launch_bounds__(256) void small_k_gemm(const IGemm g) {
    __shared__ float bt[SMALLK_MAX][260];
    const int n0 = blockIdx.y * 256;
    const int nn = min(256, g.N - n0);
    if (g.b_kn) {
        for (int i = threadIdx.x; i < nn * g.K; i += 256) {
            const int k = i / nn, n = i - k * nn;
            bt[k][n] = g.B[(long)k * g.ldb + n0 + n];
        }
    } else {
        for (int i = threadIdx.x; i < nn * g.K; i += 256) {
            const int n = i / g.K, k = i - n * g.K;
            bt[k][n] = g.B[(long)(n0 + n) * g.ldb + k];
        }
    }
    __syncthreads();
    const int nq = (nn + 3) / 4;
    const long total = (long)g.M * nq;
    for (long i = blockIdx.x * 256L + threadIdx.x; i < total; i += (long)gridDim.x * 256) {
        const long m = i / nq;
        const int n4 = (int)(i - m * nq) * 4;
        float a0 = 0.f, a1 = 0.f, a2 = 0.f, a3 = 0.f;
        const float* ar = g.A + m * g.lda;
        for (int k = 0; k < g.K; ++k) {
            const float a = ar[k];
            a0 += a * bt[k][n4]; a1 += a * bt[k][n4 + 1]; a2 += a * bt[k][n4 + 2]; a3 += a * bt[k][n4 + 3];
        }
        float v[4] = {a0, a1, a2, a3};
        float* o = g.C + m * g.ldc + n0 + n4;
#pragma unroll
        for (int e = 0; e < 4; ++e) {
            if (n4 + e < nn) {
                float x = v[e] + (g.bias ? g.bias[n0 + n4 + e] : 0.f);
                if (g.act == 1) x = fmaxf(x, 0.f); else if (g.act == 2) x = x > 0.f ? x : 0.1f * x;
                o[e] = x;
            }
        }
    }
}

__global__ __launch_bounds__(256) void splitk_finish(const float* __restrict__ part, int splits, int M, int N, const float* __restrict__ bias,
                                                     int act, float* __restrict__ C, int ldc) {
    const long total = (long)M * N;
    for (long i = blockIdx.x * 256L + threadIdx.x; i < total; i += (long)gridDim.x * 256) {
        const long m = i / N;
        const int n = (int)(i - m * N);
        float v = bias ? bias[n] : 0.f;
        for (int z = 0; z < splits; ++z) v += part[(long)z * total + i];
        if (act == 1) v = fmaxf(v, 0.f); else if (act == 2) v = v > 0.f ? v : 0.1f * v;
        C[m * ldc + n] = v;
    }
}

template <int BM, int BN, int WM, int WN, int BKF = 16>
static void launch_igemm_tile(const IGemm& g, bool fast, dim3 grid, hipStream_t s) {
    constexpr int NT = WM * WN * 64;
    char nm[96] = "";
    const bool buf = fast && g.abytes != 0 && env_int(ENV_IG_BUF, 1);
    if (g_ktiming && buf && !g.b_kn && g.a_scale != nullptr) snprintf(nm, sizeof nm, "igemm_nt_aff<%d, %d, %d, %d, %d>", BM, BN, WM, WN, BKF);
    else if (g_ktiming) snprintf(nm, sizeof nm, "igemm_nt<%d, %d, %d, %d, %s, %s, %d, %s>", BM, BN, WM, WN, fast ? "true" : "false", g.b_kn ? "true" : "false", fast ? BKF : 16, buf ? "true" : "false");
    KTimer kt(nm, 2.0 * g.M * g.N * g.K * grid.y, igemm_bytes(g, grid.y), s);
    if (buf && g.b_kn) hipLaunchKernelGGL((igemm_nt<BM, BN, WM, WN, true, true, BKF, true>), grid, dim3(NT), 0, s, g);
    else if (buf && g.a_scale != nullptr) hipLaunchKernelGGL((igemm_nt_aff<BM, BN, WM, WN, BKF>), grid, dim3(NT), 0, s, g);
    else if (buf) hipLaunchKernelGGL((igemm_nt<BM, BN, WM, WN, true, false, BKF, true>), grid, dim3(NT), 0, s, g);
    else if (fast && g.b_kn) hipLaunchKernelGGL((igemm_nt<BM, BN, WM, WN, true, true, BKF>), grid, dim3(NT), 0, s, g);
    else if (fast) hipLaunchKernelGGL((igemm_nt<BM, BN, WM, WN, true, false, BKF>), grid, dim3(NT), 0, s, g);
    else if (g.b_kn) hipLaunchKernelGGL((igemm_nt<BM, BN, WM, WN, false, true>), grid, dim3(NT), 0, s, g);
    else hipLaunchKernelGGL((igemm_nt<BM, BN, WM, WN, false, false>), grid, dim3(NT), 0, s, g);
}

static int g_gemm_bf16 = 0;
PDF_API int pdf_set_gemm_precision(int bf16) { g_gemm_bf16 = bf16 ? 1 : 0; return 0; }
PDF_API int pdf_debug_gemm_precision() { return g_gemm_bf16; }

static thread_local int g_last_tile = 0;
static thread_local int g_igemm_launches = 0;
static int g_shadow_operands = 0;
PDF_API int pdf_debug_shadow_operands() { return g_shadow_operands; }
PDF_API int pdf_debug_last_tile() { return g_last_tile; }
PDF_API int pdf_debug_igemm_launches() { return g_igemm_launches; }

static void stat_plan(IGemm& g, PdfCallOpts* co, int BM) {
    if (g.stat == nullptr) return;
    const long tiles = cdiv(g.M, BM);
    if (!g.plain_out || g.ps_cout > 0 || g.accum || tiles * g.N * 2 > co->stats_cap) { g.stat = nullptr; return; }
    co->stats_tiles = tiles; co->stats_rows = BM;
}

static int launch_igemm(IGemm& g, hipStream_t s, int groups = 1, PdfCallOpts* co = nullptr) {
    if (g.M <= 0 || g.N <= 0 || g.K <= 0) return 0;
    g.gm = env_int(ENV_IG_GROUPM, 4);
    ++g_igemm_launches;
    float* const stat_req = (co != nullptr && groups == 1) ? co->stats_out : nullptr;
    g.stat = nullptr;
    bool fast = (g.Cin % 16 == 0) && (g.lda % 4 == 0) && (g.ldb % 4 == 0) && aligned16(g.A) && aligned16(g.B);
    if (g.b_kn) fast = fast && (g.N % 4 == 0) && (g.btap % 4 == 0);
    if (groups > 1) fast = fast && aligned16(g.B1) && (g.gsA % 4 == 0);
    g.abytes = g.bbytes = 0;
    if (fast) {
        const double aext = 4.0 * (g.plain_in ? (double)g.M * g.lda : (double)cdiv(g.M, g.QH * g.QW) * g.H * g.W * g.lda);
        const double bext = 4.0 * (double)(g.b_kn ? g.Cin : g.N) * g.ldb;
        if (aext < 4294967000.0 && bext < 4294967000.0) { g.abytes = (unsigned)aext; g.bbytes = (unsigned)bext; }
    }
    g.cbytes = 0;
    if (fast && g.plain_out && g.ps_cout == 0 && 4.0 * g.M * g.ldc < 4294967000.0 && env_int(ENV_IG_BUFSTORE, 1)) g.cbytes = (unsigned)(4.0 * g.M * g.ldc);
    if (!fast && g.C16 == nullptr && groups == 1 && !g.accum && (!g.b_kn || (g.T == 1 && g.wt[0] == 0)) && g.plain_in && g.plain_out && g.K <= SMALLK_MAX && g.N >= 32 && g.ps_cout == 0 &&
        (long)g.M * g.N >= (1L << 20)) {
        dim3 grid(grid_for((long)g.M * ((min(g.N, 256) + 3) / 4)), cdiv(g.N, 256));
        KTimer kt("small_k_gemm", 2.0 * g.M * g.N * g.K, igemm_bytes(g, 1), s);
        hipLaunchKernelGGL(small_k_gemm, grid, dim3(256), 0, s, g);
        g_last_tile = 0;
        PDF_LAUNCH_CHECK();
        return 0;
    }
    if (!(g_gemm_bf16 && fast) || groups > 1) { g.A16 = nullptr; g.B16 = nullptr; g.B16T = nullptr; }
    if (g.B16T != nullptr && (!g.b_kn || g.ldbT % 8 != 0 || (reinterpret_cast<uintptr_t>(g.B16T) & 15))) g.B16T = nullptr;
    if (g.A16 != nullptr && (g.lda % 8 != 0 || (reinterpret_cast<uintptr_t>(g.A16) & 15))) g.A16 = nullptr;
    if (g.B16 != nullptr && ((!g.b_kn && g.ldb % 8 != 0) || (reinterpret_cast<uintptr_t>(g.B16) & 15))) g.B16 = nullptr;
    if (g.A == nullptr && g.A16 == nullptr) return PDF_E_BADARG;
    if (g.a_scale != nullptr && !(fast && !g_gemm_bf16 && groups == 1 && g.T == 1 && g.plain_in && !g.b_kn && g.abytes != 0 && g.K % 4 == 0 && env_int(ENV_IG_BUF, 1)))
        return PDF_E_BADARG;
    if (g_gemm_bf16 && fast) {
        g_shadow_operands += (g.A16 != nullptr) + (g.B16 != nullptr);
        const int bm16 = igemm_bf16_tile_rows(g, groups);
        if (g.C16 != nullptr && (groups != 1 || g.cbytes == 0 || g.M % bm16 != 0 || g.accum)) return PDF_E_BADARG;
        if (stat_req != nullptr && groups == 1 && g.cbytes != 0 && g.M % bm16 == 0 && env_int(ENV_IG_BF16_STATS, 1)) { g.stat = stat_req; stat_plan(g, co, bm16); }
        const int rc = launch_igemm_bf16(g, s, groups);
        if (rc < 0) return -rc;
        if (rc == 1) { g_last_tile = 16; return 0; }
        g.stat = nullptr;
        if (co != nullptr) co->stats_tiles = co->stats_rows = 0;
    }
    if (g.C16 != nullptr) return PDF_E_BADARG;
    if (g.A == nullptr) return PDF_E_BADARG;
    const long t64 = (long)cdiv(g.M, 64) * cdiv(g.N, 64);
    const bool sk_plain = g.T == 1 && g.plain_in, sk_taps = g.T > 1 && !g.plain_in && fast && g.Cin % 32 == 0 && g.K == g.T * g.Cin;
    if (groups == 1 && (sk_plain || sk_taps) && g.plain_out && g.ps_cout == 0 && !g.accum && t64 <= env_int(ENV_IG_SPLITK_MAXT, 256) && g.K >= 512 && env_int(ENV_IG_SPLITK, 1)) {
        const bool bk32 = fast && g.Cin % 32 == 0;
        const int bk = bk32 ? 32 : 16, nk = cdiv(g.K, bk);
        int splits = (int)min((long)cdiv(env_int(ENV_IG_SPLITK_TARGET, 512), (int)t64), (long)(g.K / 128));
        while (splits > 1 && (long)splits * g.M * g.N > PDF_SCRATCH_MAX) --splits;
        if (splits >= 2) {
            const int ksteps = cdiv(nk, splits);
            splits = cdiv(nk, ksteps);
            float* part = splits >= 2 ? pdf_scratch((long)splits * g.M * g.N) : nullptr;
            if (part != nullptr) {
                IGemm gs = g;
                gs.ksteps = ksteps; gs.part = part;
                const dim3 grid((unsigned)t64, 1, (unsigned)splits);
                const int dma = env_int(ENV_IG_DMA, 0);
                if (dma > 0 && fast && bk32 && launch_igemm_dma(gs, 64, dma - 1, 1, splits, s)) {}
                else if (bk32) launch_igemm_tile<64, 64, 2, 2, 32>(gs, fast, grid, s);
                else launch_igemm_tile<64, 64, 2, 2>(gs, fast, grid, s);
                KTimer kt("splitk_finish", 0.0, 4.0 * (splits + 1) * g.M * g.N, s);
                hipLaunchKernelGGL(splitk_finish, dim3(grid_for((long)g.M * g.N)), dim3(256), 0, s, part, splits, g.M, g.N, g.bias, g.act, g.C, g.ldc);
                g_last_tile = 64064;
                PDF_LAUNCH_CHECK();
                return 0;
            }
        }
    }
    long t128 = (long)cdiv(g.M, 128) * cdiv(g.N, 128) * groups;
    const bool short_k = g.T == 1 && g.batch == 0 && ((g.K <= 256 && g.M <= 262144) || (g.K <= 512 && g.M <= 32768)) && env_int(ENV_IG_SHORTK, 1);
    bool halo = fast && groups == 1 && g.T == 9 && !g.plain_in && g.plain_out && g.ps_cout == 0 && g.sy == 1 && g.sx == 1 && g.QW == g.W && g.QH == g.H &&
                (g.W == 64 || g.W == 32 || g.W == 16) && (g.H * g.W) % 128 == 0 && g.M % 128 == 0 && g.N > 64 && t128 >= env_int(ENV_IG_T128, 600) &&
                g.Cin >= env_int(ENV_IG_HALO_MINC, 256) &&
                env_int(ENV_IG_HALO, 1);
    for (int t = 0; halo && t < 9; ++t) halo = g.dy[t] >= -1 && g.dy[t] <= 1 && g.dx[t] >= -1 && g.dx[t] <= 1;
    g.stat = stat_req;
    if (halo) {
        stat_plan(g, co, 128);
        const dim3 grid((g.M / 128) * cdiv(g.N, 128));
        const bool buf = g.abytes != 0 && env_int(ENV_IG_BUF, 1);
        KTimer kt(g.b_kn ? (buf ? "igemm_halo3x3<true, true>" : "igemm_halo3x3<true, false>") : (buf ? "igemm_halo3x3<false, true>" : "igemm_halo3x3<false, false>"),
                  2.0 * g.M * g.N * g.K, igemm_bytes(g, 1), s);
        if (buf && g.b_kn) hipLaunchKernelGGL((igemm_halo3x3<true, true>), grid, dim3(256), 0, s, g);
        else if (buf) hipLaunchKernelGGL((igemm_halo3x3<false, true>), grid, dim3(256), 0, s, g);
        else if (g.b_kn) hipLaunchKernelGGL((igemm_halo3x3<true, false>), grid, dim3(256), 0, s, g);
        else hipLaunchKernelGGL((igemm_halo3x3<false, false>), grid, dim3(256), 0, s, g);
        g_last_tile = 128128;
    }
    else if (g.N > 64 && t128 >= env_int(ENV_IG_T128, 600) && !short_k) {
        stat_plan(g, co, 128);
        const int dma = env_int(ENV_IG_DMA128, 0);
        if (!(dma > 0 && fast && g.batch == 0 && launch_igemm_dma(g, 128, dma - 1, groups, 0, s)))
            launch_igemm_tile<128, 128, 2, 2>(g, fast, dim3(cdiv(g.M, 128) * cdiv(g.N, 128), groups), s);
        g_last_tile = 128128;
    }
    else if (g.N <= 64 && (long)cdiv(g.M, 128) * groups >= env_int(ENV_IG_T128, 600))
        stat_plan(g, co, 128), launch_igemm_tile<128, 64, 4, 1>(g, fast, dim3(cdiv(g.M, 128) * cdiv(g.N, 64), groups), s), g_last_tile = 128064;
    else if (fast && (long)cdiv(g.M, 64) * cdiv(g.N, 64) * groups < 96 && g.K >= 512 && env_int(ENV_IG_T32, 1)) {
        stat_plan(g, co, 32);
        launch_igemm_tile<32, 32, 1, 1>(g, fast, dim3(cdiv(g.M, 32) * cdiv(g.N, 32), groups), s), g_last_tile = 32032;
    }
    else
    {
        stat_plan(g, co, 64);
        const dim3 grid(cdiv(g.M, 64) * cdiv(g.N, 64), groups);
        const int dma = env_int(ENV_IG_DMA, 0);
        if (dma > 0 && fast && g.batch == 0 && launch_igemm_dma(g, 64, dma - 1, groups, 0, s)) {}
        else if (fast && g.Cin % 32 == 0 && env_int(ENV_IG_BK32, 1)) launch_igemm_tile<64, 64, 2, 2, 32>(g, fast, grid, s);
        else launch_igemm_tile<64, 64, 2, 2>(g, fast, grid, s);
        g_last_tile = 64064;
    }
    PDF_LAUNCH_CHECK();
    return 0;
}

int pdf_internal_batched_wgemm(const float* P, const float* Q, float* slab, int batch, long gsP, long gsQ, int M, int NI, int NJ, int splits, hipStream_t s) {
    if (M % 16 != 0 || NI % 4 != 0 || NJ % 4 != 0 || splits < 1) return PDF_E_BADARG;
    WGemm g = {};
    g.P = P; g.Q = Q; g.M = M; g.NI = NI; g.Cq = NJ; g.T = 1; g.ldp = NI; g.ldq = NJ; g.ldw = NJ;
    g.H = 1; g.W = M; g.QH = 1; g.QW = M; g.sy = 1; g.sx = 1; g.plain_q = 1;
    g.dy[0] = 0; g.dx[0] = 0; g.wt[0] = 0;
    const int rps = cdiv(cdiv(M, splits), 16) * 16;
    splits = cdiv(M, rps);
    g.rows_per_split = rps;
    g.slab = slab; g.batch = batch; g.gsP = gsP; g.gsQ = gsQ; g.gsW = (long)splits * NI * NJ;
    g.beta = 0; g.wbytes = (unsigned)(4.0 * NI * NJ);
    g.pbytes = (unsigned)(4.0 * M * NI); g.qbytes = (unsigned)(4.0 * M * NJ);
    g.uniform = 2;
    dim3 grid((unsigned)(cdiv(NI, 128) * cdiv(NJ, 128)), (unsigned)splits, (unsigned)batch);
    if (env_int(ENV_WG_BATCH_XCD, 1)) {
        g.bsplits = splits;
        grid = dim3((unsigned)(grid.x * 8 * cdiv(splits * batch, 8)));
    }
    KTimer kt("wgemm_tn_dma<3, true>", 2.0 * batch * M * NI * NJ, 4.0 * batch * ((double)M * (NI + NJ) + (double)splits * NI * NJ), s);
    hipLaunchKernelGGL((wgemm_tn_dma<3, true>), grid, dim3(256), 0, s, g);
    PDF_LAUNCH_CHECK();
    return splits;
}

int pdf_internal_batched_gemm(const float* A, const float* B, float* C, int batch, long gsA, long gsB, long gsC, int M, int N, int K, hipStream_t s) {
    IGemm g = {};
    g.A = A; g.B = B; g.C = C; g.bias = nullptr;
    g.M = M; g.N = N; g.K = K; g.Cin = K; g.lda = K; g.ldb = K; g.ldc = N;
    g.T = 1; g.plain_in = 1; g.plain_out = 1; g.act = 0;
    g.H = 1; g.W = M; g.QH = 1; g.QW = M; g.sy = 1; g.sx = 1;
    g.batch = batch; g.gsA = gsA; g.gsB = gsB; g.gsC = gsC;
    if (g_gemm_bf16) return PDF_E_BADARG;
    return launch_igemm(g, s, batch);
}

long pdf_internal_x3_deconv_workspace(int N, int H, int W, int Cin, int Cout, int KH, int KW, int stride, int pad, int backward);
int pdf_internal_x3_deconv_fwd(const float* x, const float* w, const float* bias, float* y, float* ws, int N, int H, int W, int Cin, int Cout,
                               int KH, int KW, int stride, int OH, int OW, int ldy, hipStream_t s);
int pdf_internal_x3_deconv_bwd_data(const float* dy, const float* w, float* dx, float* ws, int N, int H, int W, int Cin, int lddx, int Cout,
                                    int KH, int KW, int stride, int OH, int OW, int lddy, hipStream_t s);
int pdf_internal_x3_deconv_general_fwd(const float* x, const float* w, const float* bias, float* y, float* ws, int N, int H, int W, int Cin, int Cout,
                                       int K, int stride, int pad, int OH, int OW, int ldy, hipStream_t s);
int pdf_internal_x3_deconv_general_bwd_data(const float* dy, const float* w, float* dx, float* ws, int N, int H, int W, int Cin, int lddx, int Cout,
                                            int K, int stride, int pad, int OH, int OW, int lddy, hipStream_t s);
int pdf_internal_x3_deconv_general_bwd_weight(const float* x, const float* dy, float* dw, float* ws, int N, int H, int W, int Cin, int Cout,
                                              int K, int stride, int pad, int OH, int OW, int lddy, int accumulate, hipStream_t s);
int pdf_internal_x3_deconv_bwd_weight(const float* x, const float* dy, float* dw, float* ws, int N, int H, int W, int Cin, int Cout,
                                      int KH, int KW, int stride, int OH, int OW, int lddy, int accumulate, hipStream_t s);
PDF_API long pdf_deconv2d_x3_workspace_floats(int N, int H, int W, int Cin, int Cout, int KH, int KW, int stride, int pad, int backward) {
    return g_gemm_bf16 ? 0 : pdf_internal_x3_deconv_workspace(N, H, W, Cin, Cout, KH, KW, stride, pad, backward);
}
static void conv_taps(IGemm& g, int KH, int KW, int pad, int dil) {
    g.T = KH * KW;
    for (int ky = 0; ky < KH; ++ky)
        for (int kx = 0; kx < KW; ++kx) {
            int t = ky * KW + kx;
            g.dy[t] = (int)(ky * dil - pad); g.dx[t] = (int)(kx * dil - pad); g.wt[t] = t;
        }
}

static IGemm linear_desc(const float* x, const float* w, const float* bias, float* y,
                         int M, int N, int K, int ldx, int ldw, int ldy, int act) {
    IGemm g = {};
    g.A = x; g.B = w; g.C = y; g.bias = bias;
    g.M = M; g.N = N; g.K = K; g.Cin = K; g.lda = ldx; g.ldb = ldw; g.ldc = ldy;
    g.T = 1; g.plain_in = 1; g.plain_out = 1; g.act = act;
    g.H = 1; g.W = M; g.QH = 1; g.QW = M; g.sy = 1; g.sx = 1;
    return g;
}
static int pdf_linear_fwd_impl(const float* x, const float* w, const float* bias, float* y,
                           int M, int N, int K, int ldx, int ldw, int ldy, int act, void* stream, PdfCallOpts& co) {
    hipStream_t s = (hipStream_t)stream;
    IGemm g = linear_desc(x, w, bias, y, M, N, K, ldx, ldw, ldy, act);
    g.A16 = co.op0_bf16; g.B16 = co.op1_bf16;
    g.a_scale = co.in_scale; g.a_shift = co.in_shift;
    return launch_igemm(g, s, 1, &co);
}
PDF_API int pdf_linear_fwd_x(const float* x, const float* w, const float* bias, float* y,
                           int M, int N, int K, int ldx, int ldw, int ldy, int act, void* stream, PdfCallOpts* opts) {
    return pdf_call_x(opts, pdf_linear_fwd_impl, x, w, bias, y, M, N, K, ldx, ldw, ldy, act, stream);
}
PDF_API int pdf_linear_fwd(const float* x, const float* w, const float* bias, float* y,
                           int M, int N, int K, int ldx, int ldw, int ldy, int act, void* stream) {
    return pdf_call_plain(pdf_linear_fwd_impl, x, w, bias, y, M, N, K, ldx, ldw, ldy, act, stream);
}

static int pdf_linear_fwd_pair_impl(const float* x, const float* w0, const float* w1, const float* b0, const float* b1, float* y,
                                int M, int N, int K, int ldx, int ldw, int ldy, int act, void* stream, PdfCallOpts& co) {
    hipStream_t s = (hipStream_t)stream;
    IGemm g = linear_desc(x, w0, b0, y, M, N, K, ldx, ldw, ldy, act);
    g.B1 = w1; g.bias1 = b1; g.gsA = (long)M * ldx; g.gsC = (long)M * ldy;
    return launch_igemm(g, s, 2);
}
PDF_API int pdf_linear_fwd_pair_x(const float* x, const float* w0, const float* w1, const float* b0, const float* b1, float* y,
                                int M, int N, int K, int ldx, int ldw, int ldy, int act, void* stream, PdfCallOpts* opts) {
    return pdf_call_x(opts, pdf_linear_fwd_pair_impl, x, w0, w1, b0, b1, y, M, N, K, ldx, ldw, ldy, act, stream);
}
PDF_API int pdf_linear_fwd_pair(const float* x, const float* w0, const float* w1, const float* b0, const float* b1, float* y,
                                int M, int N, int K, int ldx, int ldw, int ldy, int act, void* stream) {
    return pdf_call_plain(pdf_linear_fwd_pair_impl, x, w0, w1, b0, b1, y, M, N, K, ldx, ldw, ldy, act, stream);
}

static int pdf_linear_bwd_data_impl(const float* dy, const float* w, float* dx, int M, int N, int K, int lddy, int ldw, int lddx,
                                void* stream, PdfCallOpts& co) {
    hipStream_t s = (hipStream_t)stream;
    IGemm g = linear_desc(dy, w, nullptr, dx, M, K, N, lddy, ldw, lddx, 0);
    g.b_kn = 1; g.btap = 0;
    g.A16 = co.op0_bf16; g.B16 = co.op1_bf16;
    if (ldw == K) { g.B16T = co.op1_bf16_t; g.ldbT = N; }
    return launch_igemm(g, s);
}
PDF_API int pdf_linear_bwd_data_x(const float* dy, const float* w, float* dx, int M, int N, int K, int lddy, int ldw, int lddx,
                                void* stream, PdfCallOpts* opts) {
    return pdf_call_x(opts, pdf_linear_bwd_data_impl, dy, w, dx, M, N, K, lddy, ldw, lddx, stream);
}
PDF_API int pdf_linear_bwd_data(const float* dy, const float* w, float* dx, int M, int N, int K, int lddy, int ldw, int lddx,
                                void* stream) {
    return pdf_call_plain(pdf_linear_bwd_data_impl, dy, w, dx, M, N, K, lddy, ldw, lddx, stream);
}

static int pdf_linear_bwd_data_pair_impl(const float* dy, const float* w0, const float* w1, float* dx, int M, int N, int K,
                                     int lddy, int ldw, int lddx, void* stream, PdfCallOpts& co) {
    hipStream_t s = (hipStream_t)stream;
    IGemm g = linear_desc(dy, w0, nullptr, dx, M, K, N, lddy, ldw, lddx, 0);
    g.b_kn = 1; g.btap = 0;
    g.B1 = w1; g.bias1 = nullptr; g.gsA = (long)M * lddy; g.gsC = (long)M * lddx;
    return launch_igemm(g, s, 2);
}
PDF_API int pdf_linear_bwd_data_pair_x(const float* dy, const float* w0, const float* w1, float* dx, int M, int N, int K,
                                     int lddy, int ldw, int lddx, void* stream, PdfCallOpts* opts) {
    return pdf_call_x(opts, pdf_linear_bwd_data_pair_impl, dy, w0, w1, dx, M, N, K, lddy, ldw, lddx, stream);
}
PDF_API int pdf_linear_bwd_data_pair(const float* dy, const float* w0, const float* w1, float* dx, int M, int N, int K,
                                     int lddy, int ldw, int lddx, void* stream) {
    return pdf_call_plain(pdf_linear_bwd_data_pair_impl, dy, w0, w1, dx, M, N, K, lddy, ldw, lddx, stream);
}


template <int CI, int CO, int KH, int KW>
__global__ __launch_bounds__(256) void tiny_conv_fwd_kernel(const float* __restrict__ x, const float* __restrict__ w, const float* __restrict__ bias,
                                                            float* __restrict__ y, int N, int H, int W, int ldx, int pad, int OH, int OW, int ldy, int act) {
    __shared__ float ws[CO * KH * KW * CI];
    for (int i = threadIdx.x; i < CO * KH * KW * CI; i += 256) ws[i] = w[i];
    __syncthreads();
    const long total = (long)N * OH * OW;
    for (long p = blockIdx.x * 256L + threadIdx.x; p < total; p += (long)gridDim.x * 256) {
        const int ox = (int)(p % OW), oy = (int)((p / OW) % OH);
        const long n = p / ((long)OW * OH);
        float acc[CO];
#pragma unroll
        for (int c = 0; c < CO; ++c) acc[c] = bias ? bias[c] : 0.f;
#pragma unroll
        for (int ky = 0; ky < KH; ++ky)
#pragma unroll
            for (int kx = 0; kx < KW; ++kx) {
                const int iy = oy + ky - pad, ix = ox + kx - pad;
                if (iy < 0 || iy >= H || ix < 0 || ix >= W) continue;
                const float* xp = x + ((n * H + iy) * W + ix) * ldx;
#pragma unroll
                for (int ci = 0; ci < CI; ++ci) {
                    const float v = xp[ci];
#pragma unroll
                    for (int c = 0; c < CO; ++c) acc[c] = fmaf(v, ws[((c * KH + ky) * KW + kx) * CI + ci], acc[c]);
                }
            }
        float* yp = y + p * ldy;
#pragma unroll
        for (int c = 0; c < CO; ++c) {
            float v = acc[c];
            if (act == 1) v = fmaxf(v, 0.f); else if (act == 2) v = v > 0.f ? v : 0.1f * v;
            yp[c] = v;
        }
    }
}
template <int CI, int CO, int KH, int KW>
__global__ __launch_bounds__(256) void tiny_conv_wgrad_kernel(const float* __restrict__ x, const float* __restrict__ dy, float* __restrict__ part,
                                                              int N, int H, int W, int ldx, int pad, int OH, int OW, int lddy) {
    constexpr int NW = CO * KH * KW * CI;
    __shared__ float red[4][NW];
    float acc[NW];
#pragma unroll
    for (int i = 0; i < NW; ++i) acc[i] = 0.f;
    const long total = (long)N * OH * OW;
    for (long p = blockIdx.x * 256L + threadIdx.x; p < total; p += (long)gridDim.x * 256) {
        const int ox = (int)(p % OW), oy = (int)((p / OW) % OH);
        const long n = p / ((long)OW * OH);
        float g[CO];
#pragma unroll
        for (int c = 0; c < CO; ++c) g[c] = dy[p * lddy + c];
#pragma unroll
        for (int ky = 0; ky < KH; ++ky)
#pragma unroll
            for (int kx = 0; kx < KW; ++kx) {
                const int iy = oy + ky - pad, ix = ox + kx - pad;
                const bool ok = iy >= 0 && iy < H && ix >= 0 && ix < W;
                const float* xp = x + ((n * H + (ok ? iy : 0)) * W + (ok ? ix : 0)) * ldx;
#pragma unroll
                for (int ci = 0; ci < CI; ++ci) {
                    const float v = ok ? xp[ci] : 0.f;
#pragma unroll
                    for (int c = 0; c < CO; ++c) acc[((c * KH + ky) * KW + kx) * CI + ci] = fmaf(g[c], v, acc[((c * KH + ky) * KW + kx) * CI + ci]);
                }
            }
    }
    const int lane = threadIdx.x & 63, wave = threadIdx.x >> 6;
#pragma unroll
    for (int i = 0; i < NW; ++i) {
        const float v = wave_sum(acc[i]);
        if (lane == 0) red[wave][i] = v;
    }
    __syncthreads();
    for (int i = threadIdx.x; i < NW; i += 256) part[(long)blockIdx.x * NW + i] = (red[0][i] + red[1][i]) + (red[2][i] + red[3][i]);
}

__global__ __launch_bounds__(256) void narrow_wgrad_kernel(const float* __restrict__ P, const float* __restrict__ Q, float* __restrict__ part, float* __restrict__ bpart,
                                                           int M, int NI, int NJ, int ldp, int ldq, int rows_per_block) {
    __shared__ float red[256 * 16];
    __shared__ float bred[256 * 4];
    const int cgs = NJ / 4, rl = 256 / cgs;
    const int cg = threadIdx.x % cgs, lr = threadIdx.x / cgs;
    float acc[4][4] = {}, bs[4] = {};
    const int m0 = blockIdx.x * rows_per_block, m1 = min(M, m0 + rows_per_block);
    if (lr < rl) {
        for (int m = m0 + lr; m < m1; m += rl) {
            const float4 q = *reinterpret_cast<const float4*>(Q + (long)m * ldq + cg * 4);
#pragma unroll
            for (int i = 0; i < 4; ++i) {
                if (i < NI) {
                    const float p = P[(long)m * ldp + i];
                    acc[i][0] = fmaf(p, q.x, acc[i][0]); acc[i][1] = fmaf(p, q.y, acc[i][1]);
                    acc[i][2] = fmaf(p, q.z, acc[i][2]); acc[i][3] = fmaf(p, q.w, acc[i][3]);
                    if (cg == 0) bs[i] += p;
                }
            }
        }
    }
#pragma unroll
    for (int i = 0; i < 4; ++i)
#pragma unroll
        for (int e = 0; e < 4; ++e) red[threadIdx.x * 16 + i * 4 + e] = acc[i][e];
#pragma unroll
    for (int i = 0; i < 4; ++i) bred[threadIdx.x * 4 + i] = bs[i];
    __syncthreads();
    if (lr == 0) {
        for (int i = 0; i < NI; ++i)
#pragma unroll
            for (int e = 0; e < 4; ++e) {
                float t = 0.f;
                for (int r = 0; r < rl; ++r) t += red[(r * cgs + cg) * 16 + i * 4 + e];
                part[(long)blockIdx.x * NI * NJ + (long)i * NJ + cg * 4 + e] = t;
            }
        if (cg == 0 && bpart != nullptr)
            for (int i = 0; i < NI; ++i) {
                float t = 0.f;
                for (int r = 0; r < rl; ++r) t += bred[(r * cgs) * 4 + i];
                bpart[(long)blockIdx.x * NI + i] = t;
            }
    }
}


__host__ __device__ constexpr int stem_off(int j) { return j < 147 ? ((j / 3 / 7) * 133 + (j / 3) % 7) * 3 + j % 3 : 2800; }
template <int KS>
__device__ __forceinline__ void stem_fwd_steps(const float* Xs, const float* Ws, int pxo, int hi, int bcol, f32x16& acc) {
    if constexpr (KS < 74) {
        const int off = hi ? stem_off(2 * KS + 1) : stem_off(2 * KS);
        const float a = Xs[off + pxo];
        const float b = Ws[(2 * KS) * 64 + bcol];
        acc = __builtin_amdgcn_mfma_f32_32x32x2f32(a, b, acc, 0, 0, 0);
        stem_fwd_steps<KS + 1>(Xs, Ws, pxo, hi, bcol, acc);
    }
}
__global__ __launch_bounds__(256) void stem7x7_fwd_kernel(const float* __restrict__ x, const float* __restrict__ w, float* __restrict__ y,
                                                          int N, int H, int W, int OH, int OW, int ldy, int act, int cpb, float* __restrict__ stat) {
    constexpr int CH = 64, XW = 2 * CH + 5, RW = XW * 3, XF = 7 * RW, DYB = 3200;
    __shared__ __attribute__((aligned(16))) float Xs[DYB];
    __shared__ __attribute__((aligned(16))) float Ws[148 * 64];
    const int tid = threadIdx.x, lane = tid & 63, wave = tid >> 6;
    for (int i = XF + tid; i < DYB; i += 256) Xs[i] = 0.f;
    for (int i = tid; i < 148 * 64; i += 256) {
        const int j = i >> 6, co = i & 63;
        Ws[i] = j < 147 ? w[co * 147 + j] : 0.f;
    }
    const int pt = wave >> 1, ct = wave & 1, hi = lane >> 5;
    const int pxo = (32 * pt + (lane & 31)) * 6, bcol = hi * 64 + 32 * ct + (lane & 31);
    const int cpr = OW / CH;
    const long total = (long)N * OH * cpr;
    const long c0 = (long)blockIdx.x * cpb, c1 = min(total, c0 + cpb);
    float xr[14];
    auto gload = [&](long c) {
        const int n = (int)(c / ((long)OH * cpr));
        const int rem = (int)(c - (long)n * OH * cpr);
        const int oy = rem / cpr, ox0 = (rem - oy * cpr) * CH;
        const int lin0 = (2 * ox0 - 3) * 3;
#pragma unroll
        for (int r = 0; r < 7; ++r) {
            const int iy = 2 * oy - 3 + r;
            const float* row = x + ((long)(n * H + iy) * W) * 3;
#pragma unroll
            for (int h = 0; h < 2; ++h) {
                const int e = tid + 256 * h, lin = lin0 + e;
                const bool ok = iy >= 0 && iy < H && e < RW && lin >= 0 && lin < 3 * W;
                xr[r * 2 + h] = ok ? row[lin] : 0.f;
            }
        }
    };
    StatAcc st[1] = {StatAcc{0.f, 0.f, 0.f, 0.f}};
    if (c0 < c1) gload(c0);
    for (long c = c0; c < c1; ++c) {
        const int n = (int)(c / ((long)OH * cpr));
        const int rem = (int)(c - (long)n * OH * cpr);
        const int oy = rem / cpr, ox0 = (rem - oy * cpr) * CH;
        __syncthreads();
#pragma unroll
        for (int r = 0; r < 7; ++r)
#pragma unroll
            for (int h = 0; h < 2; ++h) { const int e = tid + 256 * h; if (e < RW) Xs[r * RW + e] = xr[r * 2 + h]; }
        __syncthreads();
        if (c + 1 < c1) gload(c + 1);
        f32x16 acc;
#pragma unroll
        for (int r = 0; r < 16; ++r) acc[r] = 0.f;
        stem_fwd_steps<0>(Xs, Ws, pxo, hi, bcol, acc);
        float* yp = y + ((long)(n * OH + oy) * OW + ox0 + 32 * pt) * ldy + 32 * ct + (lane & 31);
#pragma unroll
// ... 629 lines not shown
```

pdfnet_amd/csrc/gemm_common.h:

```cpp
#pragma once
#include "common.h"

typedef float f32x16 __attribute__((ext_vector_type(16)));

#define MAX_TAPS 64

struct IGemm {
    const float* A; const float* B; float* C; const float* bias;
    int M, N, K, Cin;
    int lda, ldb;
    int H, W, QH, QW, sy, sx, T;
    int plain_in, plain_out;
    int OH, OW, osy, osx, ooy, oox, ldc;
    int ps_cout, ps_kw;
    int act;
    int b_kn, btap;
    const float* B1; const float* bias1; long gsA, gsC;
    int ksteps; float* part;
    const void* A16; const void* B16; const void* B116;
    int accum;
    float* stat;
    unsigned int abytes, bbytes;
    unsigned int cbytes;
    unsigned short* C16;
    const float* a_scale; const float* a_shift;
    const void* B16T; int ldbT;
    int batch; long gsB;
    int gm;
    int dy[MAX_TAPS], dx[MAX_TAPS], wt[MAX_TAPS];
};

static __device__ __attribute__((aligned(16))) float g_zero16[4] = {0.f, 0.f, 0.f, 0.f};

__device__ __forceinline__ void xcd_tile(int bid, int nblk, int ntn, int& tm, int& tn, int gm = 1) {
    int q = nblk >> 3, r = nblk & 7, x = bid & 7;
    int lin = (x < r ? x * (q + 1) : r * (q + 1) + (x - r) * q) + (bid >> 3);
    if (gm > 1) {
        const int ntm = nblk / ntn, per = gm * ntn, grp = lin / per, first = grp * gm, rem = lin - grp * per;
        const int gsz = min(ntm - first, gm);
        tm = first + rem % gsz;
        tn = rem / gsz;
        return;
    }
    tn = lin % ntn;
    tm = lin / ntn;
}

struct StatAcc { float n, s, a, b; };
__device__ __forceinline__ void stat_add(StatAcc& t, float v) {
    if (t.n == 0.f) t.s = v;
    const float d = v - t.s;
    t.n += 1.f; t.a += d; t.b = fmaf(d, d, t.b);
}
__device__ __forceinline__ void chan_merge(float& n, float& mean, float& m2, float n2, float mean2, float m22) {
    const float nt = n + n2;
    if (nt > 0.f) {
        const float d = mean2 - mean, f = n2 / nt;
        mean = fmaf(d, f, mean);
        m2 = m2 + m22 + d * d * n * f;
    }
    n = nt;
}
template <int TN, int WM, int WN, int BN>
__device__ __forceinline__ void stat_finish(const StatAcc (&acc)[TN], float* sm, float* __restrict__ stat, int tile_row, int n0, int N,
                                            int wm, int wn, int lane, int tid) {
#pragma unroll
    for (int j = 0; j < TN; ++j) {
        float n = acc[j].n;
        float mean = n > 0.f ? acc[j].s + acc[j].a / n : 0.f;
        float m2 = n > 0.f ? fmaxf(acc[j].b - acc[j].a * acc[j].a / n, 0.f) : 0.f;
        chan_merge(n, mean, m2, __shfl_xor(n, 32, 64), __shfl_xor(mean, 32, 64), __shfl_xor(m2, 32, 64));
        if (lane < 32) {
            float* o = sm + ((wm * BN) + wn * TN * 32 + j * 32 + lane) * 3;
            o[0] = n; o[1] = mean; o[2] = m2;
        }
    }
    __syncthreads();
    if (tid < BN && n0 + tid < N) {
        float n = sm[tid * 3], mean = sm[tid * 3 + 1], m2 = sm[tid * 3 + 2];
#pragma unroll
        for (int w = 1; w < WM; ++w) chan_merge(n, mean, m2, sm[(w * BN + tid) * 3], sm[(w * BN + tid) * 3 + 1], sm[(w * BN + tid) * 3 + 2]);
        float* o = stat + ((long)tile_row * N + n0 + tid) * 2;
        o[0] = mean; o[1] = m2;
    }
}

template <int TM, int TN, int WM, int WN, int BN>
__device__ __forceinline__ void lean_epilogue(const f32x16 (&acc)[TM][TN], const IGemm& g, float* Cp, const float* __restrict__ biasp,
                                              int m0, int n0, int tile_row, int wm, int wn, int lane, int tid, float* sm) {
    const auto rsC = __builtin_amdgcn_make_buffer_rsrc((void*)Cp, 0, g.cbytes, 0x00020000);
    const unsigned ldc4 = (unsigned)g.ldc * 4u;
    const bool do_stat = g.stat != nullptr;
    StatAcc st[TN];
#pragma unroll
    for (int j = 0; j < TN; ++j) st[j] = StatAcc{0.f, 0.f, 0.f, 0.f};
#pragma unroll
    for (int j = 0; j < TN; ++j) {
        const int col = n0 + wn * TN * 32 + j * 32 + (lane & 31);
        const bool cok = col < g.N;
        const float bv = (biasp != nullptr && cok) ? biasp[col] : 0.f;
#pragma unroll
        for (int i = 0; i < TM; ++i) {
            const unsigned vo = cok ? (unsigned)((m0 + wm * TM * 32 + i * 32 + 4 * (lane >> 5)) * g.ldc + col) * 4u : 0xffffffffu;
            float v[16];
#pragma unroll
            for (int r = 0; r < 16; ++r) v[r] = acc[i][j][r] + bv;
            if (g.act == 1) {
#pragma unroll
                for (int r = 0; r < 16; ++r) v[r] = fmaxf(v[r], 0.f);
            } else if (g.act == 2) {
#pragma unroll
                for (int r = 0; r < 16; ++r) v[r] = v[r] > 0.f ? v[r] : 0.1f * v[r];
            }
            if (g.accum) {
#pragma unroll
                for (int r = 0; r < 16; ++r)
                    v[r] += __builtin_bit_cast(float, __builtin_amdgcn_raw_buffer_load_b32(rsC, vo, ((r & 3) + 8 * (r >> 2)) * ldc4, 0));
            }
            if (g.C16 != nullptr) {
                const auto rsH = __builtin_amdgcn_make_buffer_rsrc((void*)g.C16, 0, g.cbytes >> 1, 0x00020000);
                const bool odd = lane & 1;
                const unsigned vh = cok ? ((vo >> 1) - (odd ? 2u : 0u)) : 0xffffffffu;
#pragma unroll
                for (int r = 0; r < 16; ++r) v[r] = __uint_as_float(pdf_pk_bf16(v[r], v[r]) << 16);
#pragma unroll
                for (int q = 0; q < 8; ++q) {
                    const int r0 = 2 * q, r1 = r0 + 1;
                    const float other = __shfl_xor(odd ? v[r0] : v[r1], 1, 64);
                    const unsigned pk = odd ? ((__float_as_uint(other) >> 16) | (__float_as_uint(v[r1]) & 0xffff0000u))
                                            : ((__float_as_uint(v[r0]) >> 16) | (__float_as_uint(other) & 0xffff0000u));
                    const unsigned ro = (unsigned)(((odd ? r1 : r0) & 3) + 8 * ((odd ? r1 : r0) >> 2)) * (ldc4 >> 1);
                    __builtin_amdgcn_raw_buffer_store_b32(pk, rsH, cok ? vh + ro : 0xffffffffu, 0, 0);
                }
            } else {
#pragma unroll
                for (int r = 0; r < 16; ++r)
                    __builtin_amdgcn_raw_buffer_store_b32(__builtin_bit_cast(unsigned, v[r]), rsC, vo, ((r & 3) + 8 * (r >> 2)) * ldc4, 0);
            }
            if (do_stat && cok) {
                if (i == 0) st[j].s = v[0];
#pragma unroll
                for (int r = 0; r < 16; ++r) { const float d = v[r] - st[j].s; st[j].a += d; st[j].b = fmaf(d, d, st[j].b); }
                st[j].n += 16.f;
            }
            __builtin_amdgcn_sched_barrier(0);
        }
    }
    if (do_stat) stat_finish<TN, WM, WN, BN>(st, sm, g.stat, tile_row, n0, g.N, wm, wn, lane, tid);
}

struct WGemm {
    const float* P; const float* Q; float* slab;
    int M, NI, Cq, T;
    int ldp, ldq, ldw;
    int H, W, QH, QW, sy, sx;
    int plain_q;
    int rows_per_split;
    int tap_major;
    int beta;
    long gsP, gsQ; float* slab1;
    float* bslab; float* bslab1;
    float* out; float* out1; float* bout; float* bout1; int accumulate; int* counters;
    int atomic;
    const void* P16; const void* Q16;
    const float* q_scale; const float* q_shift;
    unsigned int pbytes, qbytes;
    unsigned int wbytes;
    int uniform;
    int batch; long gsW;
    int bsplits;
    int dy[MAX_TAPS], dx[MAX_TAPS], wt[MAX_TAPS];
};


template <int TM, int TN>
__device__ __forceinline__ void wgemm_finish(const WGemm& g, const f32x16 (&acc)[TM][TN], int i0, int j0, int wm, int wn, int lane,
                                             bool bias_thread, float bval, int tile_id, int ntiles, int* lds_flag, bool rows_whole = false,
                                             int split_ = -1, int plane_ = 0) {
    const int grp = g.batch > 0 ? 0 : blockIdx.z, split = split_ >= 0 ? split_ : (int)blockIdx.y, splits = split_ >= 0 ? g.bsplits : (int)gridDim.y;
    float* slabp = g.batch > 0 ? g.slab + (long)(split_ >= 0 ? plane_ : (int)blockIdx.z) * g.gsW : (grp ? g.slab1 : g.slab);
    float* bslabp = grp ? g.bslab1 : g.bslab;
    const int NJ = g.T * g.Cq;
    if (g.atomic) {
        if (bias_thread) atomicAdd((grp ? g.bout1 : g.bout) + i0 + threadIdx.x, bval);
        float* dst = grp ? g.out1 : g.out;
#pragma unroll
        for (int j = 0; j < TN; ++j) {
            const int col = j0 + wn * TN * 32 + j * 32 + (lane & 31);
            if (col >= NJ) continue;
            const int t = col / g.Cq;
            const int wcol = g.wt[t] * g.Cq + (col - t * g.Cq);
#pragma unroll
            for (int i = 0; i < TM; ++i)
#pragma unroll
                for (int r = 0; r < 16; ++r) {
                    const int row = i0 + wm * TM * 32 + i * 32 + (r & 3) + 8 * (r >> 2) + 4 * (lane >> 5);
                    if (row < g.NI) atomicAdd(dst + (long)row * g.ldw + wcol, acc[i][j][r]);
                }
        }
        return;
    }
    if (bias_thread) {
        float* bo = bslabp + (long)split * g.NI + i0 + threadIdx.x;
        *bo = g.beta ? *bo + bval : bval;
    }
    float* out = slabp + (long)split * g.NI * g.ldw;
    if (g.wbytes != 0 && rows_whole) {
        const auto rsW = __builtin_amdgcn_make_buffer_rsrc((void*)out, 0, g.wbytes, 0x00020000);
        const unsigned ldw4 = (unsigned)g.ldw * 4u;
#pragma unroll
        for (int j = 0; j < TN; ++j) {
            const int col = j0 + wn * TN * 32 + j * 32 + (lane & 31);
            const bool cok = col < NJ;
            const int t = cok ? col / g.Cq : 0;
            const int wcol = g.wt[t] * g.Cq + (col - t * g.Cq);
#pragma unroll
            for (int i = 0; i < TM; ++i) {
                const unsigned vo = cok ? (unsigned)((i0 + wm * TM * 32 + i * 32 + 4 * (lane >> 5)) * g.ldw + wcol) * 4u : 0xffffffffu;
                float v[16];
#pragma unroll
                for (int r = 0; r < 16; ++r) v[r] = acc[i][j][r];
                if (g.beta) {
#pragma unroll
                    for (int r = 0; r < 16; ++r)
                        v[r] += __builtin_bit_cast(float, __builtin_amdgcn_raw_buffer_load_b32(rsW, vo, ((r & 3) + 8 * (r >> 2)) * ldw4, 0));
                }
#pragma unroll
                for (int r = 0; r < 16; ++r)
                    __builtin_amdgcn_raw_buffer_store_b32(__builtin_bit_cast(unsigned, v[r]), rsW, vo, ((r & 3) + 8 * (r >> 2)) * ldw4, 0);
            }
        }
    } else {
#pragma unroll
    for (int j = 0; j < TN; ++j) {
        const int col = j0 + wn * TN * 32 + j * 32 + (lane & 31);
        if (col >= NJ) continue;
        const int t = col / g.Cq;
        const int wcol = g.wt[t] * g.Cq + (col - t * g.Cq);
#pragma unroll
        for (int i = 0; i < TM; ++i)
#pragma unroll
            for (int r = 0; r < 16; ++r) {
                const int row = i0 + wm * TM * 32 + i * 32 + (r & 3) + 8 * (r >> 2) + 4 * (lane >> 5);
                if (row < g.NI) {
                    float* o = out + (long)row * g.ldw + wcol;
                    *o = g.beta ? *o + acc[i][j][r] : acc[i][j][r];
                }
            }
    }
    }
    if (g.counters == nullptr || splits == 1) return;
    if (!pdf_last_block_arrives(g.counters + grp * ntiles + tile_id, splits, lds_flag, true)) return;
    float* dst = grp ? g.out1 : g.out;
    const long per = (long)g.NI * g.ldw;
#pragma unroll
    for (int j = 0; j < TN; ++j) {
        const int col = j0 + wn * TN * 32 + j * 32 + (lane & 31);
        if (col >= NJ) continue;
        const int t = col / g.Cq;
        const int wcol = g.wt[t] * g.Cq + (col - t * g.Cq);
#pragma unroll
        for (int i = 0; i < TM; ++i)
#pragma unroll
            for (int r = 0; r < 16; ++r) {
                const int row = i0 + wm * TM * 32 + i * 32 + (r & 3) + 8 * (r >> 2) + 4 * (lane >> 5);
                if (row < g.NI) {
                    const long pos = (long)row * g.ldw + wcol;
                    float sum = g.accumulate ? dst[pos] : 0.f;
                    for (int z = 0; z < splits; ++z) sum += slabp[z * per + pos];
                    dst[pos] = sum;
                }
            }
    }
    if (bslabp != nullptr && j0 == 0 && threadIdx.x < TM * 64 && i0 + (int)threadIdx.x < g.NI) {
        float* bdst = grp ? g.bout1 : g.bout;
        float sum = g.accumulate ? bdst[i0 + threadIdx.x] : 0.f;
        for (int z = 0; z < splits; ++z) sum += bslabp[(long)z * g.NI + i0 + threadIdx.x];
        bdst[i0 + threadIdx.x] = sum;
    }
}

struct KTimer {
    KTimer(const char* name, double flops, double bytes, hipStream_t s);
    ~KTimer();
    int slot; hipStream_t stream;
};

int launch_igemm_bf16(const IGemm& g, hipStream_t s, int groups);
int igemm_bf16_tile_rows(const IGemm& g, int groups);
int launch_wgemm_bf16(const WGemm& g, int splits, int groups, int small, hipStream_t s);
int launch_igemm_dma(const IGemm& g, int tile, int variant, int groups, int splits, hipStream_t s);
int launch_igemm_bf16_dma(const IGemm& g, int tile, int variant, int groups, hipStream_t s);
```

pdfnet_amd/csrc/meshdec.hip:

```cpp
#include "common.h"
#ifndef MD_BF16
#define MD_BF16 0
#endif
#ifndef MD_X3
#define MD_X3 0
#endif
#if MD_X3
namespace md_x3_build {
#elif MD_BF16
namespace md_bf16_build {
#endif

typedef float f32x16 __attribute__((ext_vector_type(16)));
typedef float f32x4 __attribute__((ext_vector_type(4)));

#if defined(MD_WAVES) && MD_WAVES != 4 && MD_WAVES != 8
#error "meshdec.hip: MD_WAVES must be 4 or 8"
#endif
#ifndef MD_WAVES
#define MD_WAVES 8
#endif
#define MD_THREADS (64 * MD_WAVES)
#ifndef MD_BF16
#define MD_BF16 0
// ... 1117 lines not shown
                    const int qi = (mc + i) * 32 + (r & 3) + 8 * (r >> 2) + 4 * g.half;
                    const float m = sm[h * G::VP + qi], il = sm[HV + h * G::VP + qi], D = sm[2 * HV + h * G::VP + qi];
                    const float a = expf(S[i][r] - m) * il;
                    float at = a, gv = P[i][r];
                    if (p > 0.f) {
                        const bool keep = md_keep(dkey, (uint32_t)rowbase + (uint32_t)((h * G::V + qi) * G::V + key), p);
                        at = keep ? a * sc : 0.f;
                        gv = keep ? gv * sc : 0.f;
                    }
                    S[i][r] = a * (gv - D);
                    P[i][r] = at;
                }
#pragma unroll
            for (int dt = 0; dt < DT; ++dt) {
#pragma unroll
                for (int i = 0; i < MTC; ++i) {
#pragma unroll
                    for (int r = 0; r < 16; ++r) {
                        const int qi = (mc + i) * 32 + (r & 3) + 8 * (r >> 2) + 4 * g.half;
                        const float qa = XQ[qi * G::LD + h * DH + dt * 32 + g.l31];
                        const float ga = XG[qi * G::LD + h * DH + dt * 32 + g.l31];
                        OK[dt] = __builtin_amdgcn_mfma_f32_32x32x2f32(qa, S[i][r], OK[dt], 0, 0, 0);
                        OV[dt] = __builtin_amdgcn_mfma_f32_32x32x2f32(ga, P[i][r], OV[dt], 0, 0, 0);
                    }
                    __builtin_amdgcn_sched_barrier(0);
                }
            }
        }
        if (key < G::V) {
#pragma unroll
            for (int dt = 0; dt < DT; ++dt)
#pragma unroll
                for (int r4 = 0; r4 < 4; ++r4) {
                    const int d = dt * 32 + 8 * r4 + 4 * g.half;
                    if (d < DH) {
                        st4(dk + (long)key * G::C + h * DH + d, f32x4{OK[dt][4 * r4], OK[dt][4 * r4 + 1], OK[dt][4 * r4 + 2], OK[dt][4 * r4 + 3]});
                        st4(dv + (long)key * G::C + h * DH + d, f32x4{OV[dt][4 * r4], OV[dt][4 * r4 + 1], OV[dt][4 * r4 + 2], OV[dt][4 * r4 + 3]});
                    }
                }
        }
    }
}

template <int LV, bool CROSS>
__global__ __launch_bounds__(MD_THREADS, 1) void mesh_att_bwd1_kernel(const PdfMeshLevel a) {
    using G = Cfg<LV>;
    constexpr int C = G::C, A = CROSS ? 1 : 0;
    extern __shared__ float smem[];
    Ctx<LV> c;
    ctx_init<LV>(c, a, smem);
    const int hd = c.hand;
    const TapeOff to = tape_offsets(LV, a.B);
    const GTapeOff go = gtape_offsets(LV, a.B);
    const PdfMeshAttn& P = CROSS ? a.cross : a.self_;
    const PdfMeshAttnG& GP = CROSS ? a.gcross : a.gself;
    const float* tape = a.tape;
    float* gt = a.gtape;
    const long ro = c.row0 * C;
    const uint32_t i0 = (uint32_t)ro;
    const float* dX = CROSS ? a.dout + ro : gt + go.att(1, 8) + ro;
    MD_STAMP(2, 0);
    drop_rows<LV>(dX, true, c.XA, c.XB, gt + go.att(A, 0) + ro, c.p, c.sc, md_key(P.seed_x + c.stepmix), i0);
    __syncthreads();
    MD_STAMP(2, 1);
    f32x16 acc[G::WMT][G::WNT];
    acc_zero<LV>(acc);
    gemm_nn<LV>(acc, c.g, c.XB, P.f2.w[hd], C, 0, 1);
    __syncthreads();
    MD_STAMP(2, 2);
    {
        const float* t = tape + to.t(A) + ro;
        float* dtp = gt + go.att(A, 1) + ro;
        f32x16 tv[G::WMT][G::WNT];
        acc_load<LV>(tv, c.g, t, C);
#pragma unroll
        for (int j = 0; j < G::WNT; ++j) {
            const int colj = (c.g.nt0 + j) * 32 + c.g.l31;
#pragma unroll
            for (int i = 0; i < G::WMT; ++i)
#pragma unroll
                for (int r = 0; r < 16; ++r) {
                    const int row = (c.g.mt0 + i) * 32 + (r & 3) + 8 * (r >> 2) + 4 * c.g.half;
                    const float o = tv[i][j][r] != 0.f ? acc[i][j][r] * c.sc : 0.f;
                    c.XB[row * G::LD + colj] = row < G::V ? o : 0.f;
                    if (row < G::V) dtp[(long)row * C + colj] = o;
                }
        }
    }
    __syncthreads();
    MD_STAMP(2, 3);
    acc_zero<LV>(acc);
    gemm_nn<LV>(acc, c.g, c.XB, P.f1.w[hd], C, 0, 1);
    __syncthreads();
    MD_STAMP(2, 4);
    acc_to_lds<LV>(acc, c.g, c.XB, nullptr);
    __syncthreads();
    MD_STAMP(2, 5);
    ln_bwd_rows<LV>(c.XB, tape + to.az(A) + ro, tape + to.stz(A) + c.row0 * 2, P.ffln.g[hd], nullptr, false, dX, GP.ffln.g[hd], GP.ffln.b[hd],
                    gt + go.att(A, 7) + ro);
    __syncthreads();
    MD_STAMP(2, 6);
    drop_rows<LV>(c.XB, false, nullptr, c.XA, gt + go.att(A, 2) + ro, c.p, c.sc, md_key(P.seed_z + c.stepmix), i0);
    __syncthreads();
    MD_STAMP(2, 7);
    acc_zero<LV>(acc);
    gemm_nn<LV>(acc, c.g, c.XA, P.fc.w[hd], C, 0, 1);
    acc_to_global<LV>(acc, c.g, gt + go.att(A, 6) + ro, C, 0);
    MD_STAMP(2, 8);
}

template <int LV, bool CROSS, int PART>
__global__ __launch_bounds__(MD_THREADS, 1) void mesh_att_bwd2_kernel(const PdfMeshLevel a, const int parts) {
    using G = Cfg<LV>;
    constexpr int C = G::C, A = CROSS ? 1 : 0, HV = G::H * G::VP;
    extern __shared__ float smem[];
    Ctx<LV> c;
    ctx_init<LV>(c, a, smem);
    float* sm = smem + 2 * G::BUF;
    const int hd = c.hand;
    const TapeOff to = tape_offsets(LV, a.B);
    const GTapeOff go = gtape_offsets(LV, a.B);
    const PdfMeshAttn& P = CROSS ? a.cross : a.self_;
    const PdfMeshAttnG& GP = CROSS ? a.gcross : a.gself;
    const float* tape = a.tape;
    float* gt = a.gtape;
    const long R = 2L * a.B * G::V, VC = (long)G::V * C, ro = c.row0 * C;
    const float* q = CROSS ? a.qkv : tape + to.q(0);
    const float* k = CROSS ? a.qkv + R * C : tape + to.k(0);
    const float* v = CROSS ? a.qkv + 2 * R * C : tape + to.v(0);
    const int bo = CROSS ? (c.bb + a.B) % (2 * a.B) : c.bb;
    const float* att_o = tape + to.a_(A);
    const float* stat = tape + to.stat(A);
    const float* dc = gt + go.att(A, 6);
    const float inv_norm = 1.f / sqrtf((float)G::DH);
    MD_STAMP(3, 0);
    const int np = PART == 1 ? parts : 1, part = PART == 1 ? (int)blockIdx.y % np : 0;
    const bool do1 = PART == 0 || (PART == 1 && (int)blockIdx.y < np), do2 = PART == 0 || (PART == 1 && (int)blockIdx.y >= np);
    if (do1) {
    load_rows<LV>(c.XA, k + (long)bo * VC, C, 0);
    load_rows<LV>(c.XB, v + (long)bo * VC, C, 0);
    __syncthreads();
    attention_bwd_q<LV>(c.g, c.XA, c.XB, q + ro, att_o + ro, dc + ro, stat + c.row0 * 8, gt + go.att(A, 3) + ro, c.p, P.seed_att + c.stepmix,
                        (unsigned long long)c.bb * G::H * G::V * G::V, part, np);
    __syncthreads();
    MD_STAMP(3, 1);
    }
    if (do2) {
    load_rows_scaled<LV>(c.XA, q + (long)bo * VC, C, 0, inv_norm);
    load_rows<LV>(c.XB, dc + (long)bo * VC, C, 0);
    for (int i = threadIdx.x; i < HV; i += MD_THREADS) {
        const int h = i / G::VP, qi = i - h * G::VP;
        float m = 0.f, il = 0.f, D = 0.f;
        if (qi < G::V) {
            const float* st = stat + (long)bo * G::V * 8 + ((long)h * G::V + qi) * 2;
            m = st[0]; il = 1.f / st[1];
            const float* go_ = dc + (long)bo * VC + (long)qi * C + h * G::DH;
            const float* oo = att_o + (long)bo * VC + (long)qi * C + h * G::DH;
#pragma unroll
            for (int d = 0; d < G::DH; d += 4) {
                const f32x4 x = ld4(go_ + d), y = ld4(oo + d);
                D += x[0] * y[0] + x[1] * y[1] + x[2] * y[2] + x[3] * y[3];
            }
        }
        sm[i] = m; sm[HV + i] = il; sm[2 * HV + i] = D;
    }
    __syncthreads();
    MD_STAMP(3, 2);
    attention_bwd_kv<LV>(c.g, c.XA, c.XB, sm, k + ro, v + ro, gt + go.att(A, 4) + ro, gt + go.att(A, 5) + ro, c.p, P.seed_att + c.stepmix,
                         (unsigned long long)bo * G::H * G::V * G::V, part, np);
    __syncthreads();
    MD_STAMP(3, 3);
    }
    if constexpr (PART == 1) return;
    f32x16 acc[G::WMT][G::WNT];
    acc_zero<LV>(acc);
    load_rows<LV>(c.XA, gt + go.att(A, 3) + ro, C, 0);
    load_rows<LV>(c.XB, gt + go.att(A, 4) + ro, C, 0);
    __syncthreads();
    gemm_nn<LV>(acc, c.g, c.XA, P.q.w[hd], C, 0, 1);
    gemm_nn<LV>(acc, c.g, c.XB, P.k.w[hd], C, 0, 1);
    __syncthreads();
    load_rows<LV>(c.XA, gt + go.att(A, 5) + ro, C, 0);
    __syncthreads();
    gemm_nn<LV>(acc, c.g, c.XA, P.v.w[hd], C, 0, 1);
    acc_to_lds<LV>(acc, c.g, c.XB, nullptr);
    __syncthreads();
    MD_STAMP(3, 4);
    const float* xin = CROSS ? tape + to.xo(0) + ro : tape + to.out(3) + ro;
    ln_bwd_rows<LV>(c.XB, xin, tape + to.st(A) + c.row0 * 2, P.ln.g[hd], nullptr, false, gt + go.att(A, 7) + ro, GP.ln.g[hd], GP.ln.b[hd],
                    gt + go.att(A, 8) + ro);
    MD_STAMP(3, 5);
}

template <int LV>
__device__ __forceinline__ void gcn_bwd_head(Ctx<LV>& c, const PdfMeshLevel& a, int blk, const TapeOff& to, const GTapeOff& go) {
    using G = Cfg<LV>;
    constexpr int C = G::C;
    const int hd = c.hand;
    const PdfMeshGcn& P = a.gcn[blk];
    const PdfMeshGcnG& GP = a.ggcn[blk];
    const float* tape = a.tape;
    float* gt = a.gtape;
    const long ro = c.row0 * C;
    const uint32_t i0 = (uint32_t)ro;
    const int* colT = c.ec; const float* valT = c.ev;
    float* XA = c.XA; float* XB = c.XB;
    MD_STAMP(4, blk * 8);
    ln_bwd_rows<LV>(XA, tape + to.z(blk) + ro, tape + to.st3(blk) + c.row0 * 2, P.n3.g[hd], P.n3.b[hd], blk != 3, nullptr, GP.n3.g[hd], GP.n3.b[hd],
                    gt + go.dz(blk) + ro);
    __syncthreads();
    MD_STAMP(4, blk * 8 + 1);
    drop_rows<LV>(XA, false, nullptr, XB, gt + go.dy2(blk) + ro, c.p, c.sc, md_key(P.seed + c.stepmix), i0);
    __syncthreads();
    MD_STAMP(4, blk * 8 + 2);
    {
        f32x16 acc[G::WMT][G::WNT];
        acc_zero<LV>(acc);
        gemm_nn<LV>(acc, c.g, XB, P.fc2.w[hd], 2 * C, 1, 2);
        acc_to_lds<LV>(acc, c.g, XA, nullptr);
        acc_zero<LV>(acc);
        gemm_nn<LV>(acc, c.g, XB, P.fc2.w[hd], 2 * C, 0, 2);
        __syncthreads();
        acc_to_lds<LV>(acc, c.g, XB, nullptr);
    }
    __syncthreads();
    MD_STAMP(4, blk * 8 + 3);
    spmm_add<LV>(XB, XA, colT, valT, a.ell_w);
    __syncthreads();
    MD_STAMP(4, blk * 8 + 4);
    ln_bwd_rows<LV>(XB, tape + to.y(blk) + ro, tape + to.st2(blk) + c.row0 * 2, P.n2.g[hd], P.n2.b[hd], true, nullptr, GP.n2.g[hd], GP.n2.b[hd],
                    gt + go.dy(blk) + ro);
    load_rows<LV>(XA, gt + go.dz(blk) + ro, C, 0);
    __syncthreads();
    MD_STAMP(4, blk * 8 + 5);
}

template <int LV, bool BLK0>
__global__ __launch_bounds__(MD_THREADS, 1) void mesh_gcn_bwd_kernel(const PdfMeshLevel a, const int blk) {
    using G = Cfg<LV>;
    constexpr int C = G::C, CIN = 2 * C;
    extern __shared__ float smem[];
    Ctx<LV> c;
    ctx_init<LV>(c, a, smem);
    const int hd = c.hand;
    const TapeOff to = tape_offsets(LV, a.B);
    const GTapeOff go = gtape_offsets(LV, a.B);
    float* gt = a.gtape;
    const long ro = c.row0 * C;
    const int* colT = c.ec; const float* valT = c.ev;
    float* XA = c.XA; float* XB = c.XB;
    ell_stage<LV>(c.ec, c.ev, a.ell_colT[hd], a.ell_valT[hd], a.ell_w);
    load_rows<LV>(XA, gt + (blk == 3 ? go.att(0, 8) : go.dz(blk)) + ro, C, 0);
    __syncthreads();
    gcn_bwd_head<LV>(c, a, blk, to, go);
    const PdfMeshGcn& P = a.gcn[blk];
    if constexpr (!BLK0) {
        f32x16 acc[G::WMT][G::WNT];
        acc_zero<LV>(acc);
        gemm_nn<LV>(acc, c.g, XB, P.fc1.w[hd], 2 * C, 0, 2);
        gemm_nn<LV>(acc, c.g, XA, P.sc.w[hd], C, 0, 1);
        __syncthreads();
        acc_to_lds<LV>(acc, c.g, XA, nullptr);
        acc_zero<LV>(acc);
        gemm_nn<LV>(acc, c.g, XB, P.fc1.w[hd], 2 * C, 1, 2);
        __syncthreads();
        acc_to_lds<LV>(acc, c.g, XB, nullptr);
        __syncthreads();
        spmm_add<LV>(XA, XB, colT, valT, a.ell_w);
        __syncthreads();
        MD_STAMP(4, blk * 8 + 6);
        store_rows<LV>(gt + go.dz(blk - 1) + ro, C, 0, XA);
    } else {
        float* dxp = a.dx + c.row0 * CIN;
        float* T = gt + go.scr() + ro;
#pragma unroll 1
        for (int c0 = 0; c0 < CIN; c0 += C) {
            f32x16 acc[G::WMT][G::WNT];
            acc_zero<LV>(acc);
            gemm_nn<LV>(acc, c.g, XB, P.fc1.w[hd], 2 * CIN, 2 * c0, 2);
            gemm_nn<LV>(acc, c.g, XA, P.sc.w[hd], CIN, c0, 1);
            acc_to_global<LV>(acc, c.g, dxp, CIN, c0);
            acc_zero<LV>(acc);
            gemm_nn<LV>(acc, c.g, XB, P.fc1.w[hd], 2 * CIN, 2 * c0 + 1, 2);
            acc_to_global<LV>(acc, c.g, T, C, 0);
            __syncthreads();
            constexpr int C4 = C / 4;
            for (int i = threadIdx.x; i < G::V * C4; i += MD_THREADS) {
                const int v = i / C4, cc = (i - v * C4) * 4;
                int ci[MD_ELLW]; float vv[MD_ELLW];
#pragma unroll
                for (int w = 0; w < MD_ELLW; ++w) { ci[w] = colT[v * MD_ELLW + w]; vv[w] = valT[v * MD_ELLW + w]; }
                f32x4 s4 = ld4(dxp + (long)v * CIN + c0 + cc);
#pragma unroll
                for (int w = 0; w < MD_ELLW; ++w) s4 += vv[w] * ld4(T + (long)ci[w] * C + cc);
                st4(dxp + (long)v * CIN + c0 + cc, s4);
            }
            __syncthreads();
        }
        MD_STAMP(4, 6);
    }
}

template <int LV>
static int mesh_bwd_launch(const PdfMeshLevel& a, hipStream_t s, hipStream_t side) {
    using G = Cfg<LV>;
    const size_t smem = (size_t)2 * G::BUF * sizeof(float), smem2 = smem + (size_t)3 * G::H * G::VP * sizeof(float);
    const size_t smem_g = smem + (size_t)2 * G::V * MD_ELLW * sizeof(float);
    static bool attr_done = false;
    if (!attr_done) {
        if (hipError_t e = hipFuncSetAttribute(reinterpret_cast<const void*>(mesh_att_bwd1_kernel<LV, false>), hipFuncAttributeMaxDynamicSharedMemorySize, (int)smem)) return (int)e;
        if (hipError_t e = hipFuncSetAttribute(reinterpret_cast<const void*>(mesh_att_bwd1_kernel<LV, true>), hipFuncAttributeMaxDynamicSharedMemorySize, (int)smem)) return (int)e;
        if (hipError_t e = hipFuncSetAttribute(reinterpret_cast<const void*>(mesh_att_bwd2_kernel<LV, false, 0>), hipFuncAttributeMaxDynamicSharedMemorySize, (int)smem2)) return (int)e;
        if (hipError_t e = hipFuncSetAttribute(reinterpret_cast<const void*>(mesh_att_bwd2_kernel<LV, true, 0>), hipFuncAttributeMaxDynamicSharedMemorySize, (int)smem2)) return (int)e;
        if (hipError_t e = hipFuncSetAttribute(reinterpret_cast<const void*>(mesh_att_bwd2_kernel<LV, false, 1>), hipFuncAttributeMaxDynamicSharedMemorySize, (int)smem2)) return (int)e;
        if (hipError_t e = hipFuncSetAttribute(reinterpret_cast<const void*>(mesh_att_bwd2_kernel<LV, true, 1>), hipFuncAttributeMaxDynamicSharedMemorySize, (int)smem2)) return (int)e;
        if (hipError_t e = hipFuncSetAttribute(reinterpret_cast<const void*>(mesh_att_bwd2_kernel<LV, false, 2>), hipFuncAttributeMaxDynamicSharedMemorySize, (int)smem2)) return (int)e;
        if (hipError_t e = hipFuncSetAttribute(reinterpret_cast<const void*>(mesh_att_bwd2_kernel<LV, true, 2>), hipFuncAttributeMaxDynamicSharedMemorySize, (int)smem2)) return (int)e;
        if (hipError_t e = hipFuncSetAttribute(reinterpret_cast<const void*>(mesh_gcn_bwd_kernel<LV, false>), hipFuncAttributeMaxDynamicSharedMemorySize, (int)smem_g)) return (int)e;
        if (hipError_t e = hipFuncSetAttribute(reinterpret_cast<const void*>(mesh_gcn_bwd_kernel<LV, true>), hipFuncAttributeMaxDynamicSharedMemorySize, (int)smem_g)) return (int)e;
        attr_done = true;
    }
    const dim3 grid(2 * a.B), blk(MD_THREADS);
    hipLaunchKernelGGL((mesh_att_bwd1_kernel<LV, true>), grid, blk, smem, s, a);
    PDF_LAUNCH_CHECK();
    static const int att_split = getenv("PDF_MESH_ATT_SPLIT") ? atoi(getenv("PDF_MESH_ATT_SPLIT")) : 7;
    const bool split = (att_split >> LV) & 1;
    static const int att_parts_env = getenv("PDF_MESH_ATT_PARTS") ? atoi(getenv("PDF_MESH_ATT_PARTS")) : 0;
    const int parts_default[3] = {2, 2, 4};
    int parts = att_parts_env > 0 ? (LV == 0 ? att_parts_env / 100 : LV == 1 ? (att_parts_env / 10) % 10 : att_parts_env % 10) : parts_default[LV];
    parts = max(1, min(parts, G::H * G::MT / 4));
    if (split) {
        hipLaunchKernelGGL((mesh_att_bwd2_kernel<LV, true, 1>), dim3(2 * a.B, 2 * parts), blk, smem2, s, a, parts);
        hipLaunchKernelGGL((mesh_att_bwd2_kernel<LV, true, 2>), grid, blk, smem2, s, a, 1);
    } else hipLaunchKernelGGL((mesh_att_bwd2_kernel<LV, true, 0>), grid, blk, smem2, s, a, 1);
    PDF_LAUNCH_CHECK();
    hipLaunchKernelGGL((mesh_att_bwd1_kernel<LV, false>), grid, blk, smem, s, a);
    PDF_LAUNCH_CHECK();
    if (split) {
        hipLaunchKernelGGL((mesh_att_bwd2_kernel<LV, false, 1>), dim3(2 * a.B, 2 * parts), blk, smem2, s, a, parts);
        hipLaunchKernelGGL((mesh_att_bwd2_kernel<LV, false, 2>), grid, blk, smem2, s, a, 1);
    } else hipLaunchKernelGGL((mesh_att_bwd2_kernel<LV, false, 0>), grid, blk, smem2, s, a, 1);
    PDF_LAUNCH_CHECK();
    for (int b = 3; b >= 1; --b) {
        hipLaunchKernelGGL((mesh_gcn_bwd_kernel<LV, false>), grid, blk, smem_g, s, a, b);
        PDF_LAUNCH_CHECK();
    }
    hipLaunchKernelGGL((mesh_gcn_bwd_kernel<LV, true>), grid, blk, smem_g, s, a, 0);
    PDF_LAUNCH_CHECK();
    if (side != s) { if (int rc = pdf_stream_wait(side, s)) return rc; }
    constexpr int C = G::C;
    const int M = a.B * G::V;
    const TapeOff to = tape_offsets(LV, a.B);
    const GTapeOff go = gtape_offsets(LV, a.B);
    const float* tape = a.tape;
    const float* gt = a.gtape;
#define MD_WG_PAIR(X, LDX, DY, GL, K_)                                                                                                     \
    if ((GL).w[0] != nullptr) {                                                                                                            \
        if (int rc = pdf_linear_bwd_weight_pair((X), (DY), (GL).w[0], (GL).w[1], (GL).b[0], (GL).b[1], a.wg_ws, a.wg_ws_floats, M, C, (K_), (LDX), C, 1, side)) \
            return rc;                                                                                                                     \
    }
    for (int i = 0; i < 4; ++i) {
        const int cin = i == 0 ? a.cin0 : C;
        const float* xi = i == 0 ? a.x : tape + to.out(i - 1);
        MD_WG_PAIR(tape + to.cat1(i), 2 * cin, gt + go.dy(i), a.ggcn[i].fc1, 2 * cin)
        MD_WG_PAIR(tape + to.cat2(i), 2 * C, gt + go.dy2(i), a.ggcn[i].fc2, 2 * C)
        MD_WG_PAIR(xi, cin, gt + go.dz(i), a.ggcn[i].sc, cin)
    }
    for (int A = 0; A < 2; ++A) {
        const PdfMeshAttnG& GP = A ? a.gcross : a.gself;
        const float* hn = tape + to.h(A);
        if (A == 0) {
            MD_WG_PAIR(hn, C, gt + go.att(A, 3), GP.q, C)
            MD_WG_PAIR(hn, C, gt + go.att(A, 4), GP.k, C)
            MD_WG_PAIR(hn, C, gt + go.att(A, 5), GP.v, C)
            MD_WG_PAIR(tape + to.a_(A), C, gt + go.att(A, 2), GP.fc, C)
        } else {
            const PdfMeshLinG* gl[4] = {&GP.q, &GP.k, &GP.v, &GP.fc};
            const float* xs[4] = {hn, hn, hn, tape + to.a_(A)};
            const int slot[4] = {3, 4, 5, 2};
            for (int t = 0; t < 4; ++t)
                if (gl[t]->w[0] != nullptr)
                    if (int rc = pdf_linear_bwd_weight(xs[t], gt + go.att(A, slot[t]), gl[t]->w[0], gl[t]->b[0], a.wg_ws, a.wg_ws_floats, 2 * M, C, C, C, C, 1, side)) return rc;
        }
        MD_WG_PAIR(tape + to.hn(A), C, gt + go.att(A, 1), GP.f1, C)
        MD_WG_PAIR(tape + to.t(A), C, gt + go.att(A, 0), GP.f2, C)
    }
#undef MD_WG_PAIR
    return 0;
}

PDF_API int pdf_mesh_level_bwd(const PdfMeshLevel* a, void* stream, void* side_stream) {
    hipStream_t s = (hipStream_t)stream, side = (hipStream_t)side_stream;
    if (int rc = mesh_check(a)) return rc;
    if (a->dout == nullptr || a->dx == nullptr || a->gtape == nullptr || a->wg_ws == nullptr || !a->training) return PDF_E_BADARG;
    switch (a->level) {
        case 0: return mesh_bwd_launch<0>(*a, s, side);
        case 1: return mesh_bwd_launch<1>(*a, s, side);
        default: return mesh_bwd_launch<2>(*a, s, side);
    }
}

#if !MD_BF16
PDF_API int pdf_debug_mesh_stamps(unsigned long long* out) {
#if MD_STAMPS
    if (hipMemcpyFromSymbol(out, HIP_SYMBOL(g_md_stamps), sizeof(unsigned long long) * 8 * 3 * 64) != hipSuccess) return 0;
    return 1;
#else
    (void)out;
    return 0;
#endif
}
#else
}
#endif
```

pdfnet_amd/functional.py:

```python
import ctypes
import torch
from torch.autograd import Function

from . import hip
from .hip import ptr, ptr_at, stream

ACT_NONE, ACT_RELU, ACT_LRELU = 0, 1, 2
import os as _os

_byref = ctypes.byref
_CallOpts = hip.CallOpts
USE_SIDE_STREAMS = _os.environ.get("PDFNET_SIDE_STREAMS", "1") != "0"
_side = {}


def _record(obj, stream_):
    if torch.is_tensor(obj):
        obj.record_stream(stream_)
        s16 = getattr(obj, '_pdf_bf16', None)
        if s16 is not None:
            s16.record_stream(stream_)
    elif isinstance(obj, (list, tuple)):
        for o in obj:
            _record(o, stream_)
# ... 2011 lines not shown
        G = pts.numel() // (B * n * 3)
        for h in range(G):
            _L().pdf_bmm_strided(ptr_at(pts, h * B * n * 3), ptr(K), ptr_at(out, h * B * n * 3), B, n, 3, 3, 1,
                                 n * 3, 0, 3, 1, 9, 0, 1, 3, n * 3, 3, 1, 0, stream())
        ctx.save_for_backward(K)
        ctx.cfg = (G, B, n)
        return out

    @staticmethod
    def backward(ctx, g):
        (K,) = ctx.saved_tensors
        G, B, n = ctx.cfg
        g = g.contiguous()
        d = torch.empty_like(g)
        for h in range(G):
            _L().pdf_bmm_strided(ptr_at(g, h * B * n * 3), ptr(K), ptr_at(d, h * B * n * 3), B, n, 3, 3, 1,
                                 n * 3, 0, 3, 1, 9, 0, 3, 1, n * 3, 3, 1, 0, stream())
        return d, None


def project_points(pts, K):
    return _ProjectPoints.apply(pts, K)


class _RowLoss(Function):

    @staticmethod
    def forward(ctx, pred, tgt, row_dims, mode):
        hip.require_gpu(pred, tgt)
        pred, tgt = pred.contiguous(), tgt.contiguous()
        if pred.shape != tgt.shape:
            raise ValueError("pdfnet_amd: rowloss wants equal shapes, got %s vs %s" % (tuple(pred.shape), tuple(tgt.shape)))
        rows = 1
        for d in pred.shape[:row_dims]:
            rows *= d
        n = pred.numel() // max(rows, 1)
        out = torch.empty(pred.shape[:row_dims], dtype=torch.float32, device=pred.device)
        _L().pdf_rowloss_fwd(ptr(pred), ptr(tgt), rows, n, mode, ptr(out), stream())
        ctx.save_for_backward(pred, tgt)
        ctx.cfg = (rows, n, mode)
        return out

    @staticmethod
    def backward(ctx, g):
        pred, tgt = ctx.saved_tensors
        rows, n, mode = ctx.cfg
        dp = torch.empty_like(pred)
        _L().pdf_rowloss_bwd(ptr(pred), ptr(tgt), ptr(g.contiguous()), rows, n, mode, ptr(dp), stream())
        return dp, None, None, None


def rowloss(pred, tgt, row_dims, mode):
    return _RowLoss.apply(pred, tgt.detach(), row_dims, 0 if mode == 'l1' else 1)


class _FaceLoss(Function):

    @staticmethod
    def forward(ctx, pred, gt, faces, edge_grad):
        hip.require_gpu(pred, gt, faces)
        pred, gt, faces = pred.contiguous(), gt.contiguous(), faces.contiguous()
        G, B, V, _ = pred.shape
        Fc = faces.shape[1]
        part = torch.empty((G, B, 2), dtype=torch.float32, device=pred.device)
        _L().pdf_face_loss_fwd(ptr(pred), ptr(gt), ptr(faces), G, B, V, Fc, ptr(part), stream())
        ctx.save_for_backward(pred, gt, faces)
        ctx.edge_grad = edge_grad
        ctx.set_materialize_grads(False)
        m = part.sum(1) / float(B * 3 * Fc)
        return m[:, 0], m[:, 1]

    @staticmethod
    def backward(ctx, gn, ge):
        pred, gt, faces = ctx.saved_tensors
        G, B, V, _ = pred.shape
        Fc = faces.shape[1]
        k = 1.0 / float(B * 3 * Fc)
        wn = (gn * k).contiguous() if gn is not None else torch.zeros(G, device=pred.device)
        we = (ge * k).contiguous() if (ge is not None and ctx.edge_grad) else None
        dp = torch.empty_like(pred)
        _L().pdf_face_loss_bwd(ptr(pred), ptr(gt), ptr(faces), G, B, V, Fc, ptr(wn), ptr(we), ptr(dp), stream())
        return dp, None, None, None


def face_loss(pred, gt, faces, edge_grad=True):
    return _FaceLoss.apply(pred, gt.detach(), faces, edge_grad)


class _DenseLoss(Function):

    @staticmethod
    def forward(ctx, mask, mask_gt, hms, hms_gt, hm, hm_gt):
        hip.require_gpu(mask, hms, hm)
        mask, hms, hm = cl(mask), cl(hms), cl(hm)
        mask_gt, hms_gt, hm_gt = (t.detach().float().contiguous() for t in (mask_gt, hms_gt, hm_gt))
        for a, b in ((mask, mask_gt), (hms, hms_gt), (hm, hm_gt)):
            if a.shape != b.shape:
                raise ValueError("pdfnet_amd: dense_loss wants equal shapes, got %s vs %s" % (tuple(a.shape), tuple(b.shape)))
        B = mask.shape[0]
        L = _L()
        ws = _ws(L.pdf_dense_loss_workspace_floats(B), mask.device)
        out = torch.empty(3 + 2 * B, dtype=torch.float32, device=mask.device)
        dims = lambda t: (t.shape[1], t.shape[2] * t.shape[3])
        L.pdf_dense_loss_fwd(ptr(mask), ptr(mask_gt), *dims(mask), ptr(hms), ptr(hms_gt), *dims(hms), ptr(hm), ptr(hm_gt), *dims(hm),
                             B, ptr(ws), ptr(out), stream())
        ctx.save_for_backward(mask, mask_gt, hms, hms_gt, hm, hm_gt, out)
        ctx.set_materialize_grads(False)
        return out[0], out[1], out[2:2 + B]

    @staticmethod
    def backward(ctx, g_mask, g_hms, g_hm):
        mask, mask_gt, hms, hms_gt, hm, hm_gt, out = ctx.saved_tensors
        B = mask.shape[0]
        g_mask, g_hms, g_hm = (t.contiguous() if t is not None else None for t in (g_mask, g_hms, g_hm))
        need = ctx.needs_input_grad
        dmask = torch.empty_like(mask) if need[0] and g_mask is not None else None
        dhms = torch.empty_like(hms) if need[2] and g_hms is not None else None
        dhm = torch.empty_like(hm) if need[4] and g_hm is not None else None
        dims = lambda t: (t.shape[1], t.shape[2] * t.shape[3])
        _L().pdf_dense_loss_bwd(ptr(mask), ptr(mask_gt), ptr(dmask), *dims(mask), ptr(hms), ptr(hms_gt), ptr(dhms), *dims(hms),
                                ptr(hm), ptr(hm_gt), ptr(dhm), *dims(hm), B, ptr(g_mask), ptr(g_hms), ptr(g_hm), ptr(out), stream())
        return dmask, None, dhms, None, dhm, None


def dense_loss(mask, mask_gt, hms, hms_gt, hm, hm_gt):
    return _DenseLoss.apply(mask, mask_gt, hms, hms_gt, hm, hm_gt)


def point_dist_sum(pred, gt):
    hip.require_gpu(pred, gt)
    p, q = pred.detach().float().contiguous(), gt.detach().float().contiguous()
    if p.shape != q.shape:
        raise ValueError("pdfnet_amd: point_dist_sum wants equal shapes, got %s vs %s" % (tuple(p.shape), tuple(q.shape)))
    n, dim = p.shape[-2], p.shape[-1]
    out = torch.empty(p.shape[:-2], dtype=torch.float32, device=p.device)
    _L().pdf_point_dist_sum(ptr(p), ptr(q), out.numel(), n, dim, ptr(out), stream())
    return out


def _point_sets(name, pred, gt):
    hip.require_gpu(pred, gt)
    p, q = pred.detach().float().contiguous(), gt.detach().float().contiguous()
    if p.shape != q.shape or p.dim() < 2 or p.shape[-1] != 3:
        raise ValueError("pdfnet_amd: %s wants equal shapes [..., n, 3], got %s vs %s" % (name, tuple(p.shape), tuple(q.shape)))
    if p.shape[-2] > 1024:
        raise ValueError("pdfnet_amd: %s takes at most 1024 points per set, got %d" % (name, p.shape[-2]))
    return p, q, p.shape[-2]


def procrustes_dist(pred, gt, return_aligned=False):
    p, q, n = _point_sets("procrustes_dist", pred, gt)
    total = torch.empty(p.shape[:-2], dtype=torch.float32, device=p.device)
    dist = torch.empty(p.shape[:-1], dtype=torch.float32, device=p.device)
    aligned = torch.empty_like(p) if return_aligned else None
    _L().pdf_procrustes_dist(ptr(p), ptr(q), total.numel(), n, ptr(total), ptr(dist), ptr(aligned), stream())
    return (total, dist, aligned) if return_aligned else (total, dist)


def mesh_nn_counts(pred, gt, thresholds, return_dist=False):
    p, q, n = _point_sets("mesh_nn_counts", pred, gt)
    thr = [float(t) for t in thresholds]
    if not 1 <= len(thr) <= 4:
        raise ValueError("pdfnet_amd: mesh_nn_counts takes 1 to 4 thresholds, got %d" % len(thr))
    counts = torch.empty(p.shape[:-2] + (len(thr), 2), dtype=torch.int32, device=p.device)
    d_gt, d_pred = (torch.empty(p.shape[:-1], dtype=torch.float32, device=p.device) for _ in range(2)) if return_dist else (None, None)
    _L().pdf_mesh_nn_counts(ptr(p), ptr(q), counts.numel() // (2 * len(thr)), n, (ctypes.c_float * len(thr))(*thr), len(thr),
                            ptr(counts), ptr(d_gt), ptr(d_pred), stream())
    return (counts, d_gt, d_pred) if return_dist else counts


MESH_FUSED = _os.environ.get("PDFNET_MESH_FUSED", "1") != "0"
MESH_FUSED_BF16 = _os.environ.get("PDFNET_MESH_FUSED_BF16", "1") != "0"
MESH_BF16_MFMA = _os.environ.get("PDFNET_MESH_BF16_MFMA", "1") != "0"


def mesh_bf16_mfma():
    return _GEMM_BF16 and MESH_BF16_MFMA


def mesh_x3():
    return (not _GEMM_BF16) and (_L().pdf_debug_x3_mode() & 4) != 0


def _mesh_entry(L, which):
    if mesh_bf16_mfma():
        return getattr(L, 'pdf_mesh_level_%s_bf16' % which)
    if mesh_x3():
        return getattr(L, 'pdf_mesh_level_%s_x3' % which)
    return getattr(L, 'pdf_mesh_level_%s' % which)


def _pair(dst, l, r):
    dst[0], dst[1] = ptr(l), ptr(r)


def _mesh_lin(dst, wf, l, r):
    _pair(getattr(dst, wf), l.weight, r.weight)
    _pair(dst.b, l.bias, r.bias)


def mesh_level_params(layer):
    gl, gr = layer.graph_left.GCN_blocks, layer.graph_right.GCN_blocks
    at = layer.attn
    sl, sr = at.L_self_attn_layer, at.R_self_attn_layer
    gcn = [dict(fc1=(bl.fc1, br.fc1), fc2=(bl.fc2, br.fc2), sc=(bl.shortcut, br.shortcut), n2=(bl.norm2, br.norm2), n3=(bl.norm3, br.norm3))
           for bl, br in zip(gl, gr)]
    self_ = dict(ln=(sl.layer_norm, sr.layer_norm), q=(sl.w_qs, sr.w_qs), k=(sl.w_ks, sr.w_ks), v=(sl.w_vs, sr.w_vs), fc=(sl.fc, sr.fc),
                 ffln=(sl.ff.layer_norm, sr.ff.layer_norm), f1=(sl.ff.fc1, sr.ff.fc1), f2=(sl.ff.fc2, sr.ff.fc2))
    cross = dict(ln=(at.layer_norm1, at.layer_norm2), q=(at.w_qs, at.w_qs), k=(at.w_ks, at.w_ks), v=(at.w_vs, at.w_vs), fc=(at.fc, at.fc),
                 ffln=(at.ffL.layer_norm, at.ffR.layer_norm), f1=(at.ffL.fc1, at.ffR.fc1), f2=(at.ffL.fc2, at.ffR.fc2))
    return gcn, self_, cross


_MESH_GCN_KEYS = (('fc1', 'w'), ('fc2', 'w'), ('sc', 'w'), ('n2', 'g'), ('n3', 'g'))
_MESH_ATT_KEYS = (('ln', 'g'), ('q', 'w'), ('k', 'w'), ('v', 'w'), ('fc', 'w'), ('ffln', 'g'), ('f1', 'w'), ('f2', 'w'))


def _mesh_args(layer, x, save, p, out, tape, qkv):
    a = hip.MeshLevel()
    _, B, V, cin = x.shape
    level = {63: 0, 126: 1, 252: 2}.get(V)
    bl, br = layer.graph_left.GCN_blocks[0], layer.graph_right.GCN_blocks[0]
    if level is None or cin != 2 * (256 >> level) or bl.fc1.weight.shape[0] != (256 >> level) or len(layer.graph_left.GCN_blocks) != 4 or layer.attn.n_heads != 4:
        raise ValueError("pdfnet_amd: the fused mesh decoder covers the reference's levels (V = 63 / 126 / 252, C = 256 / 128 / 64, 4 blocks, 4 heads)")
    a.level, a.B, a.training, a.cin0, a.p = level, B, 1 if (save or p > 0) else 0, cin, p
    a.step = ptr(step_counter(x.device)) if p > 0 else None
    a.x, a.out, a.tape, a.qkv = ptr(x), ptr(out), ptr(tape), ptr(qkv)
    for k, (tl, tr) in zip(('ell_col', 'ell_val', 'ell_colT', 'ell_valT'), zip(bl.ell, br.ell)):
        _pair(getattr(a, k), tl, tr)
    a.ell_w = bl.ell_col.shape[1]
    gcn, self_, cross = mesh_level_params(layer)
    for i, blk in enumerate(gcn):
        for k, wf in _MESH_GCN_KEYS:
            _mesh_lin(getattr(a.gcn[i], k), wf, *blk[k])
        a.gcn[i].seed = next_seed() if p > 0 else 0
    for dst, src in ((a.self_, self_), (a.cross, cross)):
        for k, wf in _MESH_ATT_KEYS:
            _mesh_lin(getattr(dst, k), wf, *src[k])
        for k in ('seed_att', 'seed_z', 'seed_t', 'seed_x'):
            setattr(dst, k, next_seed() if p > 0 else 0)
    return a


def mesh_level_forward(layer, x, training=False, save=False):
    hip.require_gpu(x)
    x = x.contiguous()
    _, B, V, cin = x.shape
    C = cin // 2
    level = {63: 0, 126: 1, 252: 2}[V]
    out = torch.empty((2, B, V, C), dtype=torch.float32, device=x.device)
    tape = torch.empty(_L().pdf_mesh_tape_floats(level, B), dtype=torch.float32, device=x.device)
    qkv = torch.empty((3, 2, B, V, C), dtype=torch.float32, device=x.device)
    a = _mesh_args(layer, x, save or training, float(layer.attn.p) if training else 0.0, out, tape, qkv)
    _mesh_entry(_L(), 'fwd')(_byref(a), stream())
    return out, a, tape, qkv


def _mesh_param_list(layer):
    gcn, self_, cross = mesh_level_params(layer)
    seen, tensors, slots = {}, [], []

    def add(t, where):
        if id(t) not in seen:
            seen[id(t)] = len(tensors)
            tensors.append(t)
            slots.append([])
        slots[seen[id(t)]].append(where)
    for i, blk in enumerate(gcn):
        for k, wf in _MESH_GCN_KEYS:
            for hnd, m in enumerate(blk[k]):
                add(m.weight, ('ggcn', i, k, hnd, wf))
                add(m.bias, ('ggcn', i, k, hnd, 'b'))
    for grp, src in (('gself', self_), ('gcross', cross)):
        for k, wf in _MESH_ATT_KEYS:
            for hnd, m in enumerate(src[k]):
                add(m.weight, (grp, None, k, hnd, wf))
                add(m.bias, (grp, None, k, hnd, 'b'))
    return tensors, slots


class _MeshLevel(Function):

    @staticmethod
    def forward(ctx, x, layer, training, *params):
        need = any(ctx.needs_input_grad)
        x = x.contiguous()
        out, a, tape, qkv = mesh_level_forward(layer, x, training, save=need)
        if need:
            ctx.layer, ctx.args, ctx.keep = layer, a, (x, tape, qkv, out)
        return out

    @staticmethod
    def backward(ctx, dout):
        x, tape, qkv, out = ctx.keep
        a, layer = ctx.args, ctx.layer
        L = _L()
        dout = dout.contiguous()
        _, B, V, cin = x.shape
        C = cin // 2
        dx = torch.empty_like(x)
        gtape = torch.empty(L.pdf_mesh_gtape_floats(a.level, B), dtype=torch.float32, device=x.device)
        M = B * V
        nws = max(2 * L.pdf_wgrad_workspace_floats(M, C, 4 * C), 2 * L.pdf_wgrad_workspace_floats(M, C, 2 * C), 2 * L.pdf_wgrad_workspace_floats(M, C, C),
                  L.pdf_wgrad_workspace_floats(2 * M, C, C))
        ws = _ws(nws, x.device)
        a.dout, a.dx, a.gtape, a.wg_ws, a.wg_ws_floats = ptr(dout), ptr(dx), ptr(gtape), ptr(ws), nws
        tensors, slots = _mesh_param_list(layer)
        grads = []
        for t, where in zip(tensors, slots):
            g = _main_grad(t, t)
            ret = None
            if g is None:
                g = ret = torch.zeros_like(t)
            grads.append(ret)
            for grp, i, k, hnd, wb in where:
                dst = getattr(a, grp)
                if i is not None:
                    dst = dst[i]
                getattr(getattr(dst, k), wb)[hnd] = ptr(g)
        cur = stream()
        direct = all(g is None for g in grads)
        with wgrad_stream(direct, x, tape, qkv, gtape, ws, dout, params=tensors):
            _mesh_entry(L, 'bwd')(_byref(a), cur, stream())
        ctx.keep = ctx.args = None
        return (dx, None, None) + tuple(grads)


def mesh_level(layer, x):
    tensors, _ = _mesh_param_list(layer)
    return _MeshLevel.apply(x, layer, layer.training, *tensors)


def mesh_level_ok(layer, x):
    if not (MESH_FUSED and x.is_cuda and (MESH_FUSED_BF16 or not _GEMM_BF16) and x.dim() == 4 and x.shape[0] == 2 and x.dtype == torch.float32):
        return False
    level = {63: 0, 126: 1, 252: 2}.get(x.shape[2])
    return (level is not None and x.shape[3] == 2 * (256 >> level) and len(layer.graph_left.GCN_blocks) == 4 and layer.attn.n_heads == 4
            and layer.graph_left.GCN_blocks[0].fc1.weight.shape[0] == (256 >> level) and x.shape[1] <= 2048)


MESH_LOSS_FUSED = _os.environ.get("PDFNET_MESH_LOSS_FUSED", "1") != "0"
MESH_LOSS_TERMS = ('verts2d_loss', 'norm_loss', 'edge_loss', 'gcn_2d_loss', 'root_loss', 'verts_loss', 'abs_verts_loss', 'gcn_loss',
                   'abs_joints_loss', 'joints2d_loss', 'joints_loss', 'bone_direc_loss')


class _MeshLoss(Function):

    @staticmethod
    def forward(ctx, vp, v2p, hd3, hd2, r, gt, consts, size, down, edge_grad, coefs):
        hip.require_gpu(vp)
        vp, v2p, hd3, hd2, r = (t.contiguous() for t in (vp, v2p, hd3, hd2, r))
        B = vp.shape[1]
        if vp.shape[2:] != (778, 3) or hd3.shape[2:] != (252, 3):
            raise ValueError("pdfnet_amd: mesh_loss wants the decoder's 778- and 252-vertex meshes")
        a = hip.MeshLoss()
        keep = [vp, v2p, hd3, hd2, r]
        for k, t in (('vp', vp), ('v2p', v2p), ('hd3', hd3), ('hd2', hd2), ('r', r)):
            setattr(a, k, ptr(t))
        for k in ('vgt', 'jgt', 'v2gt', 'lmsgt'):
            for i in (0, 1):
                t = gt[k][i].contiguous()
                keep.append(t)
                getattr(a, k)[i] = ptr(t)
        for k in ('ind', 'K', 'valid'):
            t = gt[k].contiguous()
            keep.append(t)
            setattr(a, k, ptr(t))
        regs, faces, perms = consts
        a.reg[0], a.reg[1] = ptr(regs[0]), ptr(regs[1])
        a.faces = ptr(faces)
        a.perm[0], a.perm[1] = ptr(perms[0]), ptr(perms[1])
        a.B, a.Fc, a.size, a.down, a.edge_grad = B, faces.shape[1], int(size), int(down), 1 if edge_grad else 0
        for i, c in enumerate(coefs):
            a.coef[i] = float(c)
        part = torch.empty((2, B, 12), dtype=torch.float32, device=vp.device)
        out = torch.empty(4 + 9 * B, dtype=torch.float32, device=vp.device)
        a.part, a.out = ptr(part), ptr(out)
        _L().pdf_mesh_loss_fwd(_byref(a), stream())
        ctx.args, ctx.keep = a, keep + [regs, faces, perms, part]
        terms = out[:4 + 8 * B]
        ctx.mark_non_differentiable(terms)
        return out[4 + 8 * B:], terms

    @staticmethod
    def backward(ctx, g, _):
        a = ctx.args
        vp, v2p, hd3, hd2, r = ctx.keep[:5]
        g = g.contiguous()
        dvp, dv2p, dhd3, dhd2, dr = (torch.empty_like(t) for t in (vp, v2p, hd3, hd2, r))
        a.gmp = ptr(g)
        a.dvp, a.dv2p, a.dhd3, a.dhd2, a.dr = ptr(dvp), ptr(dv2p), ptr(dhd3), ptr(dhd2), ptr(dr)
        _L().pdf_mesh_loss_bwd(_byref(a), stream())
        return dvp, dv2p, dhd3, dhd2, dr, None, None, None, None, None, None


def mesh_loss(vp, v2p, hd3, hd2, r, gt, consts, size, down, edge_grad, coefs):
    mp, terms = _MeshLoss.apply(vp, v2p, hd3, hd2, r, gt, consts, size, down, edge_grad, tuple(coefs))
    B = vp.shape[1]
    d = {k: terms[i] for i, k in enumerate(MESH_LOSS_TERMS[:4])}
    d.update({k: terms[4 + i * B:4 + (i + 1) * B] for i, k in enumerate(MESH_LOSS_TERMS[4:])})
    return mp, d
```

Before: 727.1.

## Group mesh-decoder weight-gradient GEMMs into single grouped kernel launches

Replaces the many per-linear weight-gradient GEMM launches in the mesh-level backward with a grouped kernel that takes a table of problems as kernel arguments, plus one grouped split-reduction kernel. The attention-group wgrads are started early on the side stream, right after the attention backward, so they can overlap the GCN backward kernels. This is meant to cut launch overhead and small-grid underutilisation for the many tiny GEMMs. In exchange it needs a larger workspace, because the two groups can share it concurrently, and the grouped path uses a single fixed 64x64 tile configuration.

```diff
diff --git a/include/pdfnet_hip.h b/include/pdfnet_hip.h
--- a/include/pdfnet_hip.h
+++ b/include/pdfnet_hip.h
@@ -313,6 +313,9 @@
 long pdf_mesh_gtape_floats(int level, int B);
 int pdf_mesh_level_fwd(const PdfMeshLevel* a, void* stream);
 int pdf_mesh_level_bwd(const PdfMeshLevel* a, void* stream, void* side_stream);
+long pdf_mesh_wgrad_workspace_floats(int level, int B);
+int pdf_set_mesh_wgrad_grouped(int on);
+int pdf_debug_mesh_wgrad_plan(int level, int B, int* problems, int* blocks, int* splits, long* ws_floats);
 int pdf_mesh_level_fwd_bf16(const PdfMeshLevel* a, void* stream);
 int pdf_mesh_level_bwd_bf16(const PdfMeshLevel* a, void* stream, void* side_stream);
 int pdf_mesh_level_fwd_x3(const PdfMeshLevel* a, void* stream);
diff --git a/pdfnet_amd/csrc/common.h b/pdfnet_amd/csrc/common.h
--- a/pdfnet_amd/csrc/common.h
+++ b/pdfnet_amd/csrc/common.h
@@ -104,3 +104,9 @@
     PdfPlainCall call;
     return impl(a..., call.co);
 }
+
+#define PDF_WG_GROUP_MAX 48
+struct PdfWGProb { const float* dy; const float* x; float* dw; float* db; int lddy, ldx, M, NI, NJ, rps, accumulate; };
+long pdf_internal_grouped_wgemm_ws(const PdfWGProb* pr, int n);
+int pdf_internal_grouped_wgemm(const PdfWGProb* pr, int n, float* ws, long ws_floats, hipStream_t s);
+int pdf_internal_mesh_wgrad_grouped();
diff --git a/pdfnet_amd/csrc/gemm.hip b/pdfnet_amd/csrc/gemm.hip
--- a/pdfnet_amd/csrc/gemm.hip
+++ b/pdfnet_amd/csrc/gemm.hip
@@ -565,8 +565,9 @@
     if (do_stat) stat_finish<TN, 2, WN, BN>(st, &As[0][0], g.stat, tmi, n0, g.N, wm, wn, lane, tid);
 }
 
-template <int BI, int BJ, int WM, int WN, bool FAST, int BKT, bool BUF, bool AFF>
-__device__ __forceinline__ void wgemm_tn_body(const WGemm& g) {
+template <int BI, int BJ, int WM, int WN, bool FAST, int BKT, bool BUF, bool AFF, bool PLAIN = false>
+__device__ __forceinline__ void wgemm_tn_tile(const WGemm& g, const float* __restrict__ Pp, const float* __restrict__ Qp, float* bslabp,
+                                              const int ti, const int tj, const int nti, const int ntj, const int split, const int split_) {
     constexpr int BK = BKT;
     constexpr int TM = BI / WM / 32, TN = BJ / WN / 32;
     constexpr int TPR_P = BI / 4, TPR_Q = BJ / 4;
@@ -575,28 +576,12 @@
     __shared__ __attribute__((aligned(16))) float Qs[2][BK * BJ];
 
     const int tid = threadIdx.x, lane = tid & 63, wave = tid >> 6;
-    const float* __restrict__ Pp = g.P; const float* __restrict__ Qp = g.Q; float* slabp = g.slab; float* bslabp = g.bslab;
-    if (blockIdx.z) { Pp += g.gsP; Qp += g.gsQ; slabp = g.slab1; bslabp = g.bslab1; }
     const int wm = wave / WN, wn = wave % WN;
     const int NJ = g.T * g.Cq;
-    const int nti = (g.NI + BI - 1) / BI, ntj = (NJ + BJ - 1) / BJ;
-    int ti, tj;
-    if (g.tap_major) {
-        const int nblk = nti * ntj, q = nblk >> 3, r = nblk & 7, x = blockIdx.x & 7;
-        const int lin = (x < r ? x * (q + 1) : r * (q + 1) + (x - r) * q) + (blockIdx.x >> 3);
-        const int nb = g.Cq / BJ;
-        const int per_cb = g.T * nti;
-        const int cb = lin / per_cb, rem = lin - cb * per_cb;
-        const int tap = rem / nti;
-        ti = rem - tap * nti;
-        tj = tap * nb + cb;
-    } else {
-        xcd_tile(blockIdx.x, nti * ntj, ntj, ti, tj);
-    }
     const int i0 = ti * BI, j0 = tj * BJ;
     const bool do_bias = bslabp != nullptr && tj == 0 && tid < BI;
     float bsum = 0.f;
-    const int ms = blockIdx.y * g.rows_per_split;
+    const int ms = split * g.rows_per_split;
     const int me = min(g.M, ms + g.rows_per_split);
 
     const int pr = tid / TPR_P, pc = (tid % TPR_P) * 4;
@@ -606,7 +591,7 @@
     for (int e = 0; e < 4; ++e) {
         int j = j0 + qc + e;
         qok[e] = j < NJ;
-        int t = qok[e] ? j / g.Cq : 0;
+        int t = (qok[e] && !PLAIN) ? j / g.Cq : 0;
         qt[e] = t; qch[e] = j - t * g.Cq;
     }
 
@@ -622,6 +607,7 @@
     int q_ni[RQ], q_y[RQ], q_x[RQ];
 #pragma unroll
     for (int i = 0; i < RQ; ++i) {
+        if constexpr (PLAIN) { q_ni[i] = 0; q_y[i] = 0; q_x[i] = 0; continue; }
         int m = ms + qr + i * (256 / TPR_Q);
         int hw = g.QH * g.QW;
         q_ni[i] = m / hw;
@@ -646,7 +632,7 @@
             for (int i = 0; i < RQ; ++i) {
                 const int m = mb + qr + i * (256 / TPR_Q);
                 unsigned oq;
-                if (g.plain_q) oq = (m < me && qok[0]) ? (unsigned)(m * g.ldq + qch[0]) * 4u : 0xffffffffu;
+                if (PLAIN || g.plain_q) oq = (m < me && qok[0]) ? (unsigned)(m * g.ldq + qch[0]) * 4u : 0xffffffffu;
                 else {
                     const int iy = q_y[i] * g.sy + g.dy[qt[0]], ix = q_x[i] * g.sx + g.dx[qt[0]];
                     const bool ok = m < me && qok[0] && iy >= 0 && iy < g.H && ix >= 0 && ix < g.W;
@@ -664,10 +650,12 @@
                         rq[i].z = rok ? fmaxf(fmaf(rq[i].z, qsc.z, qsh.z), 0.f) : 0.f; rq[i].w = rok ? fmaxf(fmaf(rq[i].w, qsc.w, qsh.w), 0.f) : 0.f;
                     }
                 }
-                q_x[i] += BK;
-                while (q_x[i] >= g.QW) {
-                    q_x[i] -= g.QW;
-                    if (++q_y[i] == g.QH) { q_y[i] = 0; ++q_ni[i]; }
+                if constexpr (!PLAIN) {
+                    q_x[i] += BK;
+                    while (q_x[i] >= g.QW) {
+                        q_x[i] -= g.QW;
+                        if (++q_y[i] == g.QH) { q_y[i] = 0; ++q_ni[i]; }
+                    }
                 }
             }
             return;
@@ -773,7 +761,29 @@
         cur ^= 1;
     }
 
-    wgemm_finish<TM, TN>(g, acc, i0, j0, wm, wn, lane, do_bias && i0 + tid < g.NI, bsum, ti * ntj + tj, nti * ntj, reinterpret_cast<int*>(&Ps[0][0]), i0 + BI <= g.NI);
+    wgemm_finish<TM, TN, PLAIN>(g, acc, i0, j0, wm, wn, lane, do_bias && i0 + tid < g.NI, bsum, ti * ntj + tj, nti * ntj, reinterpret_cast<int*>(&Ps[0][0]), i0 + BI <= g.NI, split_);
+}
+
+template <int BI, int BJ, int WM, int WN, bool FAST, int BKT, bool BUF, bool AFF>
+__device__ __forceinline__ void wgemm_tn_body(const WGemm& g) {
+    const float* __restrict__ Pp = g.P; const float* __restrict__ Qp = g.Q; float* bslabp = g.bslab;
+    if (blockIdx.z) { Pp += g.gsP; Qp += g.gsQ; bslabp = g.bslab1; }
+    const int NJ = g.T * g.Cq;
+    const int nti = (g.NI + BI - 1) / BI, ntj = (NJ + BJ - 1) / BJ;
+    int ti, tj;
+    if (g.tap_major) {
+        const int nblk = nti * ntj, q = nblk >> 3, r = nblk & 7, x = blockIdx.x & 7;
+        const int lin = (x < r ? x * (q + 1) : r * (q + 1) + (x - r) * q) + (blockIdx.x >> 3);
+        const int nb = g.Cq / BJ;
+        const int per_cb = g.T * nti;
+        const int cb = lin / per_cb, rem = lin - cb * per_cb;
+        const int tap = rem / nti;
+        ti = rem - tap * nti;
+        tj = tap * nb + cb;
+    } else {
+        xcd_tile(blockIdx.x, nti * ntj, ntj, ti, tj);
+    }
+    wgemm_tn_tile<BI, BJ, WM, WN, FAST, BKT, BUF, AFF>(g, Pp, Qp, bslabp, ti, tj, nti, ntj, blockIdx.y, -1);
 }
 
 
@@ -783,6 +793,36 @@
 }
 __global__ __launch_bounds__(256) void wgemm_tn64_aff(const WGemm g) {
     wgemm_tn_body<64, 64, 2, 2, true, 32, true, true>(g);
+}
+
+struct WGroupProb {
+    const float* P; const float* Q;
+    float* out; float* bout;
+    int M, blk0;
+    int ni_nj, ldp_ldq, splits_beta;
+    int rps;
+};
+struct WGroup { int n, nblk; WGroupProb p[PDF_WG_GROUP_MAX]; };
+static_assert(sizeof(WGroup) <= 3072, "wgemm_tn_grouped: the problem table is passed as kernel arguments");
+__global__ __launch_bounds__(256) void wgemm_tn_grouped(const WGroup t) {
+    const int q = t.nblk >> 3, r = t.nblk & 7, x = blockIdx.x & 7;
+    const int lin = (x < r ? x * (q + 1) : r * (q + 1) + (x - r) * q) + (blockIdx.x >> 3);
+    int pi = 0;
+    while (pi + 1 < t.n && lin >= t.p[pi + 1].blk0) ++pi;
+    const WGroupProb& p = t.p[pi];
+    WGemm g = {};
+    g.M = p.M; g.NI = p.ni_nj & 0xffff; g.Cq = p.ni_nj >> 16; g.T = 1;
+    g.ldp = p.ldp_ldq & 0xffff; g.ldq = p.ldp_ldq >> 16; g.ldw = g.Cq;
+    g.plain_q = 1; g.rows_per_split = p.rps;
+    g.bsplits = p.splits_beta & 0xffff; g.beta = p.splits_beta >> 16;
+    g.slab = p.out; g.bslab = p.bout;
+    g.pbytes = (unsigned)g.M * (unsigned)g.ldp * 4u; g.qbytes = (unsigned)g.M * (unsigned)g.ldq * 4u;
+    g.wbytes = (unsigned)(g.NI * g.ldw) * 4u;
+    const int nti = (g.NI + 63) >> 6, ntj = (g.Cq + 63) >> 6;
+    const int local = lin - p.blk0, tiles = nti * ntj;
+    const int split = local / tiles, tile = local - split * tiles;
+    const int ti = tile / ntj, tj = tile - ti * ntj;
+    wgemm_tn_tile<64, 64, 2, 2, true, 32, true, false, true>(g, p.P, p.Q, p.bout, ti, tj, nti, ntj, split, split);
 }
 
 
@@ -1097,11 +1137,49 @@
     if (ty == 0 && i < n) out[i] = (r.accumulate ? out[i] : 0.f) + ((sm[0][tx] + sm[1][tx]) + (sm[2][tx] + sm[3][tx]));
 }
 
+struct RGroupProb {
+    const float* slab; float* dw; float* db;
+    int n, nb, splits, accumulate, blk0, pad_;
+};
+struct RGroup { int n, nblk; RGroupProb p[PDF_WG_GROUP_MAX]; };
+static_assert(sizeof(RGroup) <= 3072, "reduce_slabs_grouped: the problem table is passed as kernel arguments");
+__global__ __launch_bounds__(256) void reduce_slabs_grouped(const RGroup t) {
+    const int bid = blockIdx.x;
+    int pi = 0;
+    while (pi + 1 < t.n && bid >= t.p[pi + 1].blk0) ++pi;
+    const RGroupProb& p = t.p[pi];
+    const int local = bid - p.blk0, wblocks = (p.n + 1023) >> 10, splits = p.splits;
+    const bool bias = local >= wblocks;
+    const float* slab = bias ? p.slab + (long)splits * p.n : p.slab;
+    float* out = bias ? p.db : p.dw;
+    const int n = bias ? p.nb : p.n;
+    const int base = bias ? 0 : local << 10;
+    float s[4];
+#pragma unroll
+    for (int e = 0; e < 4; ++e) {
+        const int i = base + e * 256 + (int)threadIdx.x;
+        s[e] = (p.accumulate && i < n) ? out[i] : 0.f;
+    }
+    for (int z = 0; z < splits; ++z) {
+#pragma unroll
+        for (int e = 0; e < 4; ++e) {
+            const int i = base + e * 256 + (int)threadIdx.x;
+            if (i < n) s[e] += slab[(long)z * n + i];
+        }
+    }
+#pragma unroll
+    for (int e = 0; e < 4; ++e) {
+        const int i = base + e * 256 + (int)threadIdx.x;
+        if (i < n) out[i] = s[e];
+    }
+}
+
 static bool aligned16(const void* p) { return (reinterpret_cast<uintptr_t>(p) & 15) == 0; }
 
 #include <cstdlib>
 #include <climits>
 #include <mutex>
+#include <algorithm>
 enum { ENV_IG_T128, ENV_IG_BK32, ENV_WG_TARGET, ENV_WG_MINROWS, ENV_WG_TAPMAJOR, ENV_WG_BK32, ENV_WG_DMA, ENV_IG_HALO_MINC, ENV_IG_HALO, ENV_IG_T32, ENV_WG_INLAUNCH, ENV_WG_QUANT, ENV_IG_SPLITK, ENV_WG_LDSPAD, ENV_IG_SHORTK, ENV_WG_ATOMIC, ENV_WG_STEM, ENV_IG_SPLITK_MAXT, ENV_IG_SPLITK_TARGET, ENV_WG_SLOTS, ENV_WG_BUF, ENV_IG_BUF, ENV_WG_UNIFORM, ENV_IG_BUFSTORE, ENV_IG_BF16_STATS, ENV_IG_DMA, ENV_IG_DMA128, ENV_WG_BATCH_XCD, ENV_IG_GROUPM, ENV_COUNT };
 static int env_int(int which, int dflt) {
     static const char* const names[ENV_COUNT] = {"PDF_IG_T128", "PDF_IG_BK32", "PDF_WG_TARGET", "PDF_WG_MINROWS", "PDF_WG_TAPMAJOR",
@@ -1407,6 +1485,70 @@
     hipLaunchKernelGGL((wgemm_tn_dma<3, true>), grid, dim3(256), 0, s, g);
     PDF_LAUNCH_CHECK();
     return splits;
+}
+
+long pdf_internal_grouped_wgemm_ws(const PdfWGProb* pr, int n) {
+    if (pr == nullptr || n < 1 || n > PDF_WG_GROUP_MAX || g_gemm_bf16) return -1;
+    long need = 0;
+    for (int i = 0; i < n; ++i) {
+        const PdfWGProb& q = pr[i];
+        if (q.dy == nullptr || q.x == nullptr || q.dw == nullptr || q.M < 1 || q.NI < 4 || q.NJ < 4 || q.rps < 1) return -1;
+        if (q.NI % 4 || q.NJ % 4 || q.lddy % 4 || q.ldx % 4 || q.lddy < q.NI || q.ldx < q.NJ || !aligned16(q.dy) || !aligned16(q.x)) return -1;
+        if (q.NI > 32764 || q.NJ > 32764 || q.lddy > 32764 || q.ldx > 32764) return -1;
+        if (4.0 * q.M * q.lddy >= 4294967000.0 || 4.0 * q.M * q.ldx >= 4294967000.0) return -1;
+        const int splits = cdiv(q.M, q.rps);
+        if (splits > 1 && q.rps % 16) return -1;
+        if (splits > 32767 || (long)splits * q.NI * q.NJ >= (1L << 31)) return -1;
+        if (splits > 1) need += (long)splits * ((long)q.NI * q.NJ + (q.db ? q.NI : 0));
+    }
+    return need;
+}
+
+int pdf_internal_grouped_wgemm(const PdfWGProb* pr, int n, float* ws, long ws_floats, hipStream_t s) {
+    const long need = pdf_internal_grouped_wgemm_ws(pr, n);
+    if (need < 0 || need > ws_floats || (need > 0 && ws == nullptr)) return PDF_E_BADARG;
+    int order[PDF_WG_GROUP_MAX];
+    for (int i = 0; i < n; ++i) order[i] = i;
+    std::stable_sort(order, order + n, [&](int a, int b) { return min(pr[a].rps, pr[a].M) > min(pr[b].rps, pr[b].M); });
+    WGroup t = {};
+    RGroup r = {};
+    long off = 0;
+    int blk = 0, rblk = 0;
+    double flops = 0.0, bytes = 0.0, rbytes = 0.0;
+    for (int k = 0; k < n; ++k) {
+        const PdfWGProb& q = pr[order[k]];
+        const int splits = cdiv(q.M, q.rps);
+        const long per = (long)q.NI * q.NJ, perb = q.db ? q.NI : 0;
+        WGroupProb& w = t.p[k];
+        w.P = q.dy; w.Q = q.x; w.M = q.M; w.blk0 = blk; w.rps = q.rps;
+        w.ni_nj = q.NI | (q.NJ << 16); w.ldp_ldq = q.lddy | (q.ldx << 16);
+        if (splits == 1) {
+            w.out = q.dw; w.bout = q.db; w.splits_beta = 1 | ((q.accumulate ? 1 : 0) << 16);
+        } else {
+            w.out = ws + off; w.bout = q.db ? ws + off + splits * per : nullptr; w.splits_beta = splits;
+            RGroupProb& rp = r.p[r.n++];
+            rp.slab = ws + off; rp.dw = q.dw; rp.db = q.db; rp.n = (int)per; rp.nb = (int)perb; rp.splits = splits;
+            rp.accumulate = q.accumulate ? 1 : 0; rp.blk0 = rblk;
+            rblk += cdiv(per, 1024) + (perb ? 1 : 0);
+            off += splits * (per + perb);
+            rbytes += 4.0 * (splits + 1 + (q.accumulate ? 1 : 0)) * (per + perb);
+        }
+        blk += cdiv(q.NI, 64) * cdiv(q.NJ, 64) * splits;
+        flops += 2.0 * q.M * q.NI * q.NJ;
+        bytes += 4.0 * ((double)q.M * (q.NI + q.NJ) + (double)splits * (per + perb));
+    }
+    t.n = n; t.nblk = blk; r.nblk = rblk;
+    {
+        KTimer kt("wgemm_tn_grouped<64, 64>", flops, bytes, s);
+        hipLaunchKernelGGL(wgemm_tn_grouped, dim3((unsigned)blk), dim3(256), 0, s, t);
+    }
+    PDF_LAUNCH_CHECK();
+    if (r.n > 0) {
+        KTimer kt("reduce_slabs_grouped", 0.0, rbytes, s);
+        hipLaunchKernelGGL(reduce_slabs_grouped, dim3((unsigned)rblk), dim3(256), 0, s, r);
+        PDF_LAUNCH_CHECK();
+    }
+    return 0;
 }
 
 int pdf_internal_batched_gemm(const float* A, const float* B, float* C, int batch, long gsA, long gsB, long gsC, int M, int N, int K, hipStream_t s) {
diff --git a/pdfnet_amd/csrc/gemm_common.h b/pdfnet_amd/csrc/gemm_common.h
--- a/pdfnet_amd/csrc/gemm_common.h
+++ b/pdfnet_amd/csrc/gemm_common.h
@@ -173,7 +173,7 @@
 };
 
 
-template <int TM, int TN>
+template <int TM, int TN, bool PLAIN = false>
 __device__ __forceinline__ void wgemm_finish(const WGemm& g, const f32x16 (&acc)[TM][TN], int i0, int j0, int wm, int wn, int lane,
                                              bool bias_thread, float bval, int tile_id, int ntiles, int* lds_flag, bool rows_whole = false,
                                              int split_ = -1, int plane_ = 0) {
@@ -188,8 +188,8 @@
         for (int j = 0; j < TN; ++j) {
             const int col = j0 + wn * TN * 32 + j * 32 + (lane & 31);
             if (col >= NJ) continue;
-            const int t = col / g.Cq;
-            const int wcol = g.wt[t] * g.Cq + (col - t * g.Cq);
+            const int t = PLAIN ? 0 : col / g.Cq;
+            const int wcol = PLAIN ? col : g.wt[t] * g.Cq + (col - t * g.Cq);
 #pragma unroll
             for (int i = 0; i < TM; ++i)
 #pragma unroll
@@ -212,8 +212,8 @@
         for (int j = 0; j < TN; ++j) {
             const int col = j0 + wn * TN * 32 + j * 32 + (lane & 31);
             const bool cok = col < NJ;
-            const int t = cok ? col / g.Cq : 0;
-            const int wcol = g.wt[t] * g.Cq + (col - t * g.Cq);
+            const int t = (cok && !PLAIN) ? col / g.Cq : 0;
+            const int wcol = PLAIN ? col : g.wt[t] * g.Cq + (col - t * g.Cq);
 #pragma unroll
             for (int i = 0; i < TM; ++i) {
                 const unsigned vo = cok ? (unsigned)((i0 + wm * TM * 32 + i * 32 + 4 * (lane >> 5)) * g.ldw + wcol) * 4u : 0xffffffffu;
@@ -235,8 +235,8 @@
     for (int j = 0; j < TN; ++j) {
         const int col = j0 + wn * TN * 32 + j * 32 + (lane & 31);
         if (col >= NJ) continue;
-        const int t = col / g.Cq;
-        const int wcol = g.wt[t] * g.Cq + (col - t * g.Cq);
+        const int t = PLAIN ? 0 : col / g.Cq;
+        const int wcol = PLAIN ? col : g.wt[t] * g.Cq + (col - t * g.Cq);
 #pragma unroll
         for (int i = 0; i < TM; ++i)
 #pragma unroll
@@ -257,8 +257,8 @@
     for (int j = 0; j < TN; ++j) {
         const int col = j0 + wn * TN * 32 + j * 32 + (lane & 31);
         if (col >= NJ) continue;
-        const int t = col / g.Cq;
-        const int wcol = g.wt[t] * g.Cq + (col - t * g.Cq);
+        const int t = PLAIN ? 0 : col / g.Cq;
+        const int wcol = PLAIN ? col : g.wt[t] * g.Cq + (col - t * g.Cq);
 #pragma unroll
         for (int i = 0; i < TM; ++i)
 #pragma unroll
diff --git a/pdfnet_amd/csrc/meshdec.hip b/pdfnet_amd/csrc/meshdec.hip
--- a/pdfnet_amd/csrc/meshdec.hip
+++ b/pdfnet_amd/csrc/meshdec.hip
@@ -1443,6 +1443,158 @@
 }
 
 template <int LV>
+static int mesh_wg_per_linear(const PdfMeshLevel& a, hipStream_t side) {
+    using G = Cfg<LV>;
+    constexpr int C = G::C;
+    const int M = a.B * G::V;
+    const TapeOff to = tape_offsets(LV, a.B);
+    const GTapeOff go = gtape_offsets(LV, a.B);
+    const float* tape = a.tape;
+    const float* gt = a.gtape;
+#define MD_WG_PAIR(X, LDX, DY, GL, K_)                                                                                                     \
+    if ((GL).w[0] != nullptr) {                                                                                                            \
+        if (int rc = pdf_linear_bwd_weight_pair((X), (DY), (GL).w[0], (GL).w[1], (GL).b[0], (GL).b[1], a.wg_ws, a.wg_ws_floats, M, C, (K_), (LDX), C, 1, side)) \
+            return rc;                                                                                                                     \
+    }
+    for (int i = 0; i < 4; ++i) {
+        const int cin = i == 0 ? a.cin0 : C;
+        const float* xi = i == 0 ? a.x : tape + to.out(i - 1);
+        MD_WG_PAIR(tape + to.cat1(i), 2 * cin, gt + go.dy(i), a.ggcn[i].fc1, 2 * cin)
+        MD_WG_PAIR(tape + to.cat2(i), 2 * C, gt + go.dy2(i), a.ggcn[i].fc2, 2 * C)
+        MD_WG_PAIR(xi, cin, gt + go.dz(i), a.ggcn[i].sc, cin)
+    }
+    for (int A = 0; A < 2; ++A) {
+        const PdfMeshAttnG& GP = A ? a.gcross : a.gself;
+        const float* hn = tape + to.h(A);
+        if (A == 0) {
+            MD_WG_PAIR(hn, C, gt + go.att(A, 3), GP.q, C)
+            MD_WG_PAIR(hn, C, gt + go.att(A, 4), GP.k, C)
+            MD_WG_PAIR(hn, C, gt + go.att(A, 5), GP.v, C)
+            MD_WG_PAIR(tape + to.a_(A), C, gt + go.att(A, 2), GP.fc, C)
+        } else {
+            const PdfMeshLinG* gl[4] = {&GP.q, &GP.k, &GP.v, &GP.fc};
+            const float* xs[4] = {hn, hn, hn, tape + to.a_(A)};
+            const int slot[4] = {3, 4, 5, 2};
+            for (int t = 0; t < 4; ++t)
+                if (gl[t]->w[0] != nullptr)
+                    if (int rc = pdf_linear_bwd_weight(xs[t], gt + go.att(A, slot[t]), gl[t]->w[0], gl[t]->b[0], a.wg_ws, a.wg_ws_floats, 2 * M, C, C, C, C, 1, side)) return rc;
+        }
+        MD_WG_PAIR(tape + to.hn(A), C, gt + go.att(A, 1), GP.f1, C)
+        MD_WG_PAIR(tape + to.t(A), C, gt + go.att(A, 0), GP.f2, C)
+    }
+#undef MD_WG_PAIR
+    return 0;
+}
+
+static inline int mesh_wg_rows_per_split(int M, int want) {
+    for (int sp = want; sp > 1; --sp) {
+        const int rps = cdiv(cdiv(M, sp), 16) * 16, n = cdiv(M, rps);
+        if (n == sp && rps >= 128 && M - (n - 1) * rps >= 128) return rps;
+    }
+    return M;
+}
+static inline int mesh_wg_want_splits(int level) {
+    const int tiles = 1056 >> (2 * level);
+    return max(1, (1024 + tiles / 2) / tiles);
+}
+template <int LV>
+static void mesh_wg_tables(const PdfMeshLevel& a, PdfWGProb (*tab)[PDF_WG_GROUP_MAX], int* ntab) {
+    using G = Cfg<LV>;
+    constexpr int C = G::C;
+    const int M = a.B * G::V;
+    const TapeOff to = tape_offsets(LV, a.B);
+    const GTapeOff go = gtape_offsets(LV, a.B);
+    const float* tape = a.tape;
+    const float* gt = a.gtape;
+    const int want = mesh_wg_want_splits(LV);
+    const int rps = mesh_wg_rows_per_split(M, want), rps2 = mesh_wg_rows_per_split(2 * M, 2 * want);
+    ntab[0] = ntab[1] = 0;
+    auto pair = [&](int grp, const float* x, int ldx, const float* dy, const PdfMeshLinG& gl, int K) {
+        for (int h = 0; h < 2; ++h)
+            if (gl.w[h] != nullptr)
+                tab[grp][ntab[grp]++] = PdfWGProb{dy + (long)h * M * C, x + (long)h * M * ldx, gl.w[h], gl.b[h], C, ldx, M, C, K, rps, 1};
+    };
+    auto shared = [&](const float* x, const float* dy, const PdfMeshLinG& gl) {
+        if (gl.w[0] != nullptr) tab[0][ntab[0]++] = PdfWGProb{dy, x, gl.w[0], gl.b[0], C, C, 2 * M, C, C, rps2, 1};
+    };
+    for (int i = 0; i < 4; ++i) {
+        const int cin = i == 0 ? a.cin0 : C;
+        const float* xi = i == 0 ? a.x : tape + to.out(i - 1);
+        pair(1, tape + to.cat1(i), 2 * cin, gt + go.dy(i), a.ggcn[i].fc1, 2 * cin);
+        pair(1, tape + to.cat2(i), 2 * C, gt + go.dy2(i), a.ggcn[i].fc2, 2 * C);
+        pair(1, xi, cin, gt + go.dz(i), a.ggcn[i].sc, cin);
+    }
+    for (int A = 0; A < 2; ++A) {
+        const PdfMeshAttnG& GP = A ? a.gcross : a.gself;
+        const float* hn = tape + to.h(A);
+        const float* ao = tape + to.a_(A);
+        if (A == 0) {
+            pair(0, hn, C, gt + go.att(A, 3), GP.q, C);
+            pair(0, hn, C, gt + go.att(A, 4), GP.k, C);
+            pair(0, hn, C, gt + go.att(A, 5), GP.v, C);
+            pair(0, ao, C, gt + go.att(A, 2), GP.fc, C);
+        } else {
+            shared(hn, gt + go.att(A, 3), GP.q);
+            shared(hn, gt + go.att(A, 4), GP.k);
+            shared(hn, gt + go.att(A, 5), GP.v);
+            shared(ao, gt + go.att(A, 2), GP.fc);
+        }
+        pair(0, tape + to.hn(A), C, gt + go.att(A, 1), GP.f1, C);
+        pair(0, tape + to.t(A), C, gt + go.att(A, 0), GP.f2, C);
+    }
+}
+template <int LV>
+static bool mesh_wg_grouped_ok(const PdfMeshLevel& a, PdfWGProb (*tab)[PDF_WG_GROUP_MAX], int* ntab) {
+    ntab[0] = ntab[1] = 0;
+    if (!pdf_internal_mesh_wgrad_grouped() || pdf_debug_gemm_precision()) return false;
+    mesh_wg_tables<LV>(a, tab, ntab);
+    for (int grp = 0; grp < 2; ++grp) {
+        if (ntab[grp] == 0) continue;
+        const long need = pdf_internal_grouped_wgemm_ws(tab[grp], ntab[grp]);
+        if (need < 0 || need > a.wg_ws_floats) return false;
+    }
+    return true;
+}
+
+#if !MD_BF16
+static int g_mesh_wg_grouped = -1;
+int pdf_internal_mesh_wgrad_grouped() {
+    if (g_mesh_wg_grouped < 0) { const char* e = getenv("PDF_MESH_WG_GROUPED"); g_mesh_wg_grouped = (e == nullptr || atoi(e) != 0) ? 1 : 0; }
+    return g_mesh_wg_grouped;
+}
+PDF_API int pdf_set_mesh_wgrad_grouped(int on) {
+    const int before = pdf_internal_mesh_wgrad_grouped();
+    g_mesh_wg_grouped = on ? 1 : 0;
+    return before;
+}
+PDF_API int pdf_debug_mesh_wgrad_plan(int level, int B, int* problems, int* blocks, int* splits, long* ws_floats) {
+    if (level < 0 || level > 2 || B < 1 || B > 2048) return 0;
+    const int C = 256 >> level, M = B * (63 << level), want = mesh_wg_want_splits(level);
+    const int rps = mesh_wg_rows_per_split(M, want), rps2 = mesh_wg_rows_per_split(2 * M, 2 * want);
+    const int sp = cdiv(M, rps), sp2 = cdiv(2 * M, rps2), nti = C / 64;
+    int nblk = 0, nprob = 0;
+    long ws[2] = {0, 0};
+    auto add = [&](int grp, int K, int count, int s_) {
+        nprob += count;
+        nblk += count * nti * (K / 64) * s_;
+        if (s_ > 1) ws[grp] += (long)count * s_ * ((long)C * K + C);
+    };
+    add(1, 4 * C, 2, sp); add(1, 2 * C, 4, sp);
+    add(1, 2 * C, 12, sp); add(1, C, 6, sp);
+    add(0, C, 16, sp); add(0, C, 4, sp2);
+    if (problems) *problems = nprob;
+    if (blocks) *blocks = nblk;
+    if (splits) *splits = sp;
+    if (ws_floats) *ws_floats = max(ws[0], ws[1]);
+    return 1;
+}
+PDF_API long pdf_mesh_wgrad_workspace_floats(int level, int B) {
+    long ws = 0;
+    return pdf_debug_mesh_wgrad_plan(level, B, nullptr, nullptr, nullptr, &ws) ? ws : 0;
+}
+#endif
+
+template <int LV>
 static int mesh_bwd_launch(const PdfMeshLevel& a, hipStream_t s, hipStream_t side) {
     using G = Cfg<LV>;
     const size_t smem = (size_t)2 * G::BUF * sizeof(float), smem2 = smem + (size_t)3 * G::H * G::VP * sizeof(float);
@@ -1482,6 +1634,14 @@
         hipLaunchKernelGGL((mesh_att_bwd2_kernel<LV, false, 2>), grid, blk, smem2, s, a, 1);
     } else hipLaunchKernelGGL((mesh_att_bwd2_kernel<LV, false, 0>), grid, blk, smem2, s, a, 1);
     PDF_LAUNCH_CHECK();
+    PdfWGProb tab[2][PDF_WG_GROUP_MAX];
+    int ntab[2] = {0, 0};
+    const bool grouped = mesh_wg_grouped_ok<LV>(a, tab, ntab);
+    if (grouped && side != s && ntab[0] > 0) {
+        if (int rc = pdf_stream_wait(side, s)) return rc;
+        if (int rc = pdf_internal_grouped_wgemm(tab[0], ntab[0], a.wg_ws, a.wg_ws_floats, side)) return rc;
+        ntab[0] = 0;
+    }
     for (int b = 3; b >= 1; --b) {
         hipLaunchKernelGGL((mesh_gcn_bwd_kernel<LV, false>), grid, blk, smem_g, s, a, b);
         PDF_LAUNCH_CHECK();
@@ -1489,44 +1649,10 @@
     hipLaunchKernelGGL((mesh_gcn_bwd_kernel<LV, true>), grid, blk, smem_g, s, a, 0);
     PDF_LAUNCH_CHECK();
     if (side != s) { if (int rc = pdf_stream_wait(side, s)) return rc; }
-    constexpr int C = G::C;
-    const int M = a.B * G::V;
-    const TapeOff to = tape_offsets(LV, a.B);
-    const GTapeOff go = gtape_offsets(LV, a.B);
-    const float* tape = a.tape;
-    const float* gt = a.gtape;
-#define MD_WG_PAIR(X, LDX, DY, GL, K_)                                                                                                     \
-    if ((GL).w[0] != nullptr) {                                                                                                            \
-        if (int rc = pdf_linear_bwd_weight_pair((X), (DY), (GL).w[0], (GL).w[1], (GL).b[0], (GL).b[1], a.wg_ws, a.wg_ws_floats, M, C, (K_), (LDX), C, 1, side)) \
-            return rc;                                                                                                                     \
-    }
-    for (int i = 0; i < 4; ++i) {
-        const int cin = i == 0 ? a.cin0 : C;
-        const float* xi = i == 0 ? a.x : tape + to.out(i - 1);
-        MD_WG_PAIR(tape + to.cat1(i), 2 * cin, gt + go.dy(i), a.ggcn[i].fc1, 2 * cin)
-        MD_WG_PAIR(tape + to.cat2(i), 2 * C, gt + go.dy2(i), a.ggcn[i].fc2, 2 * C)
-        MD_WG_PAIR(xi, cin, gt + go.dz(i), a.ggcn[i].sc, cin)
-    }
-    for (int A = 0; A < 2; ++A) {
-        const PdfMeshAttnG& GP = A ? a.gcross : a.gself;
-        const float* hn = tape + to.h(A);
-        if (A == 0) {
-            MD_WG_PAIR(hn, C, gt + go.att(A, 3), GP.q, C)
-            MD_WG_PAIR(hn, C, gt + go.att(A, 4), GP.k, C)
-            MD_WG_PAIR(hn, C, gt + go.att(A, 5), GP.v, C)
-            MD_WG_PAIR(tape + to.a_(A), C, gt + go.att(A, 2), GP.fc, C)
-        } else {
-            const PdfMeshLinG* gl[4] = {&GP.q, &GP.k, &GP.v, &GP.fc};
-            const float* xs[4] = {hn, hn, hn, tape + to.a_(A)};
-            const int slot[4] = {3, 4, 5, 2};
-            for (int t = 0; t < 4; ++t)
-                if (gl[t]->w[0] != nullptr)
-                    if (int rc = pdf_linear_bwd_weight(xs[t], gt + go.att(A, slot[t]), gl[t]->w[0], gl[t]->b[0], a.wg_ws, a.wg_ws_floats, 2 * M, C, C, C, C, 1, side)) return rc;
-        }
-        MD_WG_PAIR(tape + to.hn(A), C, gt + go.att(A, 1), GP.f1, C)
-        MD_WG_PAIR(tape + to.t(A), C, gt + go.att(A, 0), GP.f2, C)
-    }
-#undef MD_WG_PAIR
+    if (!grouped) return mesh_wg_per_linear<LV>(a, side);
+    for (int grp = 0; grp < 2; ++grp)
+        if (ntab[grp] > 0)
+            if (int rc = pdf_internal_grouped_wgemm(tab[grp], ntab[grp], a.wg_ws, a.wg_ws_floats, side)) return rc;
     return 0;
 }
 
diff --git a/pdfnet_amd/functional.py b/pdfnet_amd/functional.py
--- a/pdfnet_amd/functional.py
+++ b/pdfnet_amd/functional.py
@@ -2337,7 +2337,7 @@
         gtape = torch.empty(L.pdf_mesh_gtape_floats(a.level, B), dtype=torch.float32, device=x.device)
         M = B * V
         nws = max(2 * L.pdf_wgrad_workspace_floats(M, C, 4 * C), 2 * L.pdf_wgrad_workspace_floats(M, C, 2 * C), 2 * L.pdf_wgrad_workspace_floats(M, C, C),
-                  L.pdf_wgrad_workspace_floats(2 * M, C, C))
+                  L.pdf_wgrad_workspace_floats(2 * M, C, C), L.pdf_mesh_wgrad_workspace_floats(a.level, B))
         ws = _ws(nws, x.device)
         a.dout, a.dx, a.gtape, a.wg_ws, a.wg_ws_floats = ptr(dout), ptr(dx), ptr(gtape), ptr(ws), nws
         tensors, slots = _mesh_param_list(layer)
```

Result: no change. 725.8 (-0.2%).
